# wdykas/LDDL

Hardware: AMD Instinct MI355X
Metric: WordPiece+MLM tokens/sec (1/2/4/8 MI355X) and % of HBM roofline (higher is better)
Workload: dtype uint16

## Files before the change

### include/lddl_amd.h

```cpp
#ifndef LDDL_AMD_H_
#define LDDL_AMD_H_

#include <stddef.h>
#include <stdint.h>

#ifdef __cplusplus
extern "C" {
#endif

typedef struct lddl_ctx lddl_ctx;

const char* lddl_last_error(void);
int lddl_version(void);
const char* lddl_build_id(void);

int64_t lddl_synth_corpus(uint64_t seed, int64_t doc_begin, int64_t target_bytes,
                          double nonascii_frac, uint8_t* text, int64_t text_cap,
                          int64_t* sent_off, int64_t sent_cap, int64_t* doc_sent_off,
                          int64_t doc_cap, int64_t* n_sent_out, int64_t* n_doc_out,
                          int n_threads);
int64_t lddl_synth_doc_text(uint64_t seed, int64_t doc_begin, int64_t target_bytes,
                            double nonascii_frac, uint8_t* text, int64_t text_cap, int64_t* doc_off,
                            int64_t doc_cap, int64_t* n_doc_out, int n_threads);

typedef struct lddl_reader lddl_reader;
int lddl_read_groups(int64_t n_blocks, const char* const* paths, const int64_t* starts,
                     const int64_t* ends, const uint32_t* mt_states, double ratio, int64_t n_groups,
                     const int64_t* group_off, const uint64_t* group_seed_abs, int n_threads,
                     lddl_reader** out, int64_t* n_docs, int64_t* n_text, int64_t* bad);
int lddl_read_fill(lddl_reader* reader, uint8_t* text, int64_t* doc_off, int64_t* block_ndocs);
int lddl_read_counts(const lddl_reader* reader, int64_t* block_ndocs, int64_t* doc_len);
int lddl_read_fill_range(lddl_reader* reader, int64_t d0, int64_t d1, uint8_t* text,
                         int64_t* doc_off);
int lddl_read_free(lddl_reader* reader);
int lddl_random_state_data(int64_t n, uint64_t seed_abs, uint32_t* out);

int lddl_ctx_create(int device, const uint8_t* norm_table, int64_t table_len, const char* vocab,
                    int64_t vocab_len, lddl_ctx** out);
int lddl_ctx_destroy(lddl_ctx* ctx);
int lddl_ctx_info(const lddl_ctx* ctx, int32_t* vocab_size, int32_t* special_ids,
                  int32_t* max_piece_bytes);
int lddl_ctx_id_bytes(const lddl_ctx* ctx);
int lddl_ctx_render_table(const lddl_ctx* ctx, const uint8_t** d_bytes, const int64_t** d_off);

typedef void* (*lddl_alloc_fn)(size_t bytes, void* stream, void* user);
typedef void (*lddl_free_fn)(void* p, void* stream, void* user);
int lddl_ctx_set_allocator(lddl_ctx* ctx, lddl_alloc_fn alloc_fn, lddl_free_fn free_fn,
                           void* user);

int lddl_tokenize(lddl_ctx* ctx, void* stream, const uint8_t* d_text, int64_t n_bytes,
                  const int64_t* d_sent_off, int64_t n_sent, int32_t max_pieces, int32_t* d_ids,
                  int32_t* d_sent_len);

int lddl_utf8_check(void* stream, const uint8_t* d_text, int64_t n_bytes, int64_t* d_first_bad);

int lddl_punkt_set_params(lddl_ctx* ctx, const uint8_t* table, int64_t table_bytes,
                          const uint8_t* records, int64_t records_bytes);
int lddl_segment_count(lddl_ctx* ctx, void* stream, const uint8_t* d_text, int64_t n_bytes,
                       const int64_t* d_doc_off, int64_t n_doc, int64_t* n_sent);
int lddl_segment_fill(lddl_ctx* ctx, void* stream, int64_t* d_sent_off, int64_t* d_doc_sent_off);

int lddl_bart_count(lddl_ctx* ctx, void* stream, const uint8_t* d_text, int64_t n_bytes,
                    const int64_t* d_sent_off, int64_t n_sent, const int64_t* d_doc_sent_off,
                    int64_t n_doc, int32_t target_words, int64_t* n_chunks, int64_t* n_out_bytes);
int lddl_bart_fill(lddl_ctx* ctx, void* stream, uint8_t* d_out, int64_t* d_chunk_off,
                   int32_t* d_num_tokens, int64_t* d_doc_chunk_off);

typedef struct lddl_pairs lddl_pairs;
enum { LDDL_RNG_REPLAY = 0, LDDL_RNG_NATIVE = 1 };
typedef struct {
  int32_t seq;
  int32_t dup;
  int32_t masking;
  int32_t rng;
  double short_seq_prob;
  double masked_lm_ratio;
  uint64_t native_seed;
} lddl_pair_params;
int lddl_pairs_plan(lddl_ctx* ctx, void* stream, const lddl_pair_params* params,
                    const int64_t* d_sent_off, const int32_t* d_ids, const int32_t* d_sent_len,
                    int64_t n_sent, const int64_t* d_doc_sent_off, int64_t n_doc,
                    const int64_t* d_part_doc_off, const int64_t* d_part_seed, int64_t n_part,
                    lddl_pairs** out, int64_t* counts);
int lddl_pairs_emit(lddl_pairs* plan, void* stream, void* d_tokens, int64_t* d_tok_off,
                    int32_t* d_len_a, uint8_t* d_is_rn, uint16_t* d_pos, void* d_lab,
                    int64_t* d_pos_off);
int lddl_pairs_destroy(lddl_pairs* plan, void* stream);
int lddl_pairs_part_offsets(lddl_pairs* plan, void* stream, int64_t* d_part_pair_off);
int lddl_pairs_plan_ms(const lddl_pairs* plan, float* ms);

int lddl_bin_partitions(lddl_ctx* ctx, void* stream, const int32_t* d_num_tokens,
                        const int64_t* d_tok_off, int64_t n_rows, const int64_t* d_part_off,
                        int64_t n_part, int32_t bin_size, int32_t nbins, int64_t* d_perm,
                        int64_t* d_bin_id, int64_t* d_counts);

int lddl_bin_stable(lddl_ctx* ctx, void* stream, const int32_t* d_num_tokens,
                    const int64_t* d_tok_off, int64_t n_rows, int32_t bin_size, int32_t nbins,
                    int64_t* d_perm, int64_t* d_bin_id, int64_t* d_counts);

int lddl_render_lengths(lddl_ctx* ctx, void* stream, const void* d_tokens,
                        const int64_t* d_tok_off, const int32_t* d_len_a, const void* d_lab,
                        const int64_t* d_pos_off, const int64_t* d_rows, int64_t n_rows,
                        int64_t* d_a_len, int64_t* d_b_len, int64_t* d_l_len, int64_t* d_npy_len,
                        const uint8_t* d_is_rn, uint16_t* d_num_tokens_out, uint8_t* d_is_rn_out);
int lddl_render_write(lddl_ctx* ctx, void* stream, const void* d_tokens,
                      const int64_t* d_tok_off, const int32_t* d_len_a, const uint16_t* d_pos,
                      const void* d_lab, const int64_t* d_pos_off, const int64_t* d_rows,
                      int64_t n_rows, const int64_t* d_a_off, const int64_t* d_b_off,
                      const int64_t* d_l_off, const int64_t* d_npy_off, uint8_t* d_a_bytes,
                      uint8_t* d_b_bytes, uint8_t* d_l_bytes, uint8_t* d_npy_bytes);

int lddl_gather_ragged(void* stream, const void* d_src_a, const int64_t* d_off_a, int64_t n_a,
                       const void* d_src_b, const int64_t* d_off_b, int32_t elem_bytes,
                       const int64_t* d_rows, int64_t n_rows, const int64_t* d_dst_off, void* d_dst);
int lddl_take(void* stream, const void* d_a, int64_t n_a, const void* d_b, int32_t elem_bytes,
              const int64_t* d_rows, int64_t n_rows, void* d_dst);
int lddl_ragged_offsets(lddl_ctx* ctx, void* stream, const int64_t* d_off_a, int64_t n_a,
                        const int64_t* d_off_b, const int64_t* d_rows, int64_t n_rows,
                        int64_t* d_out);
int lddl_expand_segments(void* stream, const int64_t* d_src, const int64_t* d_seg,
                         const int64_t* d_seg_off, int64_t n_seg, int64_t total, int64_t* d_out);
int lddl_pairs_meta_pack(void* stream, const int64_t* d_tok_off, const int32_t* d_len_a,
                         const uint8_t* d_is_rn, const int64_t* d_pos_off, const int64_t* d_rows,
                         int64_t n, int32_t* d_meta);
int lddl_pairs_meta_unpack(void* stream, const int32_t* d_meta, int64_t n, int64_t* d_ntok,
                           int32_t* d_len_a, uint8_t* d_is_rn, int64_t* d_nmask);

int lddl_scan_i64(lddl_ctx* ctx, void* stream, const int64_t* d_in, int64_t n, int64_t* d_out);

int lddl_collate_encode(lddl_ctx* ctx, void* stream, const uint8_t* d_bytes, const int64_t* d_a_off,
                        const int64_t* d_b_off, const int32_t* d_na, const int32_t* d_nb,
                        int32_t batch, int32_t seq_len, int64_t* d_input_ids,
                        int64_t* d_token_type_ids, int64_t* d_attention_mask,
                        int64_t* d_special_tokens_mask, const uint8_t* d_lab_bytes,
                        const int64_t* d_lab_off, const uint16_t* d_pos, const int64_t* d_pos_off,
                        int64_t* d_labels, int64_t ignore_index);

int lddl_collate_encode_mp(lddl_ctx* ctx, void* stream, const uint8_t* d_bytes,
                           const int64_t* d_a_off, const int64_t* d_b_off, const int32_t* d_na,
                           const int32_t* d_nb, int32_t batch, int32_t seq_len,
                           int64_t* d_input_ids, int64_t* d_token_type_ids,
                           int64_t* d_attention_mask, int64_t* d_special_tokens_mask,
                           const uint8_t* d_lab_bytes, const int64_t* d_lab_off,
                           const uint16_t* d_pos, const int64_t* d_pos_off, int64_t* d_labels,
                           int64_t ignore_index, int64_t* d_loss_mask);

int lddl_collate_encode_masked(lddl_ctx* ctx, void* stream, const uint8_t* d_bytes,
                               const int64_t* d_a_off, const int64_t* d_b_off, const int32_t* d_na,
                               const int32_t* d_nb, int32_t batch, int32_t seq_len,
                               int64_t* d_input_ids, int64_t* d_token_type_ids,
                               int64_t* d_attention_mask, int64_t* d_labels, float mlm_probability,
                               int64_t ignore_index, int64_t vocab_len, uint64_t seed,
                               uint64_t counter);

int lddl_mask_dynamic(lddl_ctx* ctx, void* stream, int64_t* d_input_ids, int64_t* d_labels,
                      const int64_t* d_special_tokens_mask, const int32_t* d_na, const int32_t* d_nb,
                      int64_t batch, int64_t seq_len, float mlm_probability, int64_t ignore_index,
                      int64_t vocab_len, uint64_t seed, uint64_t counter,
                      const uint8_t* d_r_masked, const uint8_t* d_r_replaced,
                      const uint8_t* d_r_random, const int64_t* d_r_words);

int lddl_mask_dynamic_ww(lddl_ctx* ctx, void* stream, int64_t* d_input_ids, int64_t* d_labels,
                         const int64_t* d_special_tokens_mask, const int32_t* d_na,
                         const int32_t* d_nb, int64_t batch, int64_t seq_len,
                         float mlm_probability, int64_t ignore_index, int64_t vocab_len,
                         uint64_t seed, uint64_t counter);

int lddl_collate_encode_masked_ww(lddl_ctx* ctx, void* stream, const uint8_t* d_bytes,
                                  const int64_t* d_a_off, const int64_t* d_b_off,
                                  const int32_t* d_na, const int32_t* d_nb, int32_t batch,
                                  int32_t seq_len, int64_t* d_input_ids, int64_t* d_token_type_ids,
                                  int64_t* d_attention_mask, int64_t* d_labels,
                                  float mlm_probability, int64_t ignore_index, int64_t vocab_len,
                                  uint64_t seed, uint64_t counter);

#ifdef __cplusplus
}
#endif

#endif
```

### lddl_amd/_native.py

```python
import ctypes
import os

import torch

_HERE = os.path.dirname(os.path.abspath(__file__))
LIB_PATH = os.environ.get('LDDL_AMD_LIB') or os.path.join(_HERE, '_lib', 'liblddl_amd.so')

c_i64, c_u64, c_i32, c_u32, c_dbl, c_vp = (ctypes.c_int64, ctypes.c_uint64, ctypes.c_int32,
                                           ctypes.c_uint32, ctypes.c_double, ctypes.c_void_p)
c_i64p = ctypes.POINTER(ctypes.c_int64)

SIGNATURES = {
    'lddl_last_error': (ctypes.c_char_p, []),
    'lddl_build_id': (ctypes.c_char_p, []),
    'lddl_version': (ctypes.c_int, []),
    'lddl_synth_corpus': (c_i64, [c_u64, c_i64, c_i64, c_dbl, c_vp, c_i64, c_vp, c_i64, c_vp, c_i64,
                                  c_i64p, c_i64p, ctypes.c_int]),
    'lddl_read_groups': (ctypes.c_int, [c_i64, c_vp, c_vp, c_vp, c_vp, c_dbl, c_i64, c_vp, c_vp,
                                        ctypes.c_int, ctypes.POINTER(c_vp), c_i64p, c_i64p, c_vp]),
    'lddl_read_fill': (ctypes.c_int, [c_vp, c_vp, c_vp, c_vp]),
    'lddl_read_free': (ctypes.c_int, [c_vp]),
    'lddl_read_counts': (ctypes.c_int, [c_vp, c_vp, c_vp]),
    'lddl_read_fill_range': (ctypes.c_int, [c_vp, c_i64, c_i64, c_vp, c_vp]),
    'lddl_random_state_data': (ctypes.c_int, [c_i64, c_u64, c_vp]),
    'lddl_ctx_create': (ctypes.c_int, [ctypes.c_int, c_vp, c_i64, c_vp, c_i64,
                                       ctypes.POINTER(c_vp)]),
    'lddl_ctx_destroy': (ctypes.c_int, [c_vp]),
    'lddl_ctx_info': (ctypes.c_int, [c_vp, c_vp, c_vp, c_vp]),
    'lddl_ctx_id_bytes': (ctypes.c_int, [c_vp]),
    'lddl_ctx_render_table': (ctypes.c_int, [c_vp, ctypes.POINTER(c_vp), ctypes.POINTER(c_vp)]),
    'lddl_synth_doc_text': (c_i64, [c_u64, c_i64, c_i64, c_dbl, c_vp, c_i64, c_vp, c_i64, c_vp,
                                    ctypes.c_int]),
    'lddl_punkt_set_params': (ctypes.c_int, [c_vp, c_vp, c_i64, c_vp, c_i64]),
    'lddl_segment_count': (ctypes.c_int, [c_vp, c_vp, c_vp, c_i64, c_vp, c_i64,
                                          ctypes.POINTER(c_i64)]),
    'lddl_segment_fill': (ctypes.c_int, [c_vp, c_vp, c_vp, c_vp]),
    'lddl_bart_count': (ctypes.c_int, [c_vp, c_vp, c_vp, c_i64, c_vp, c_i64, c_vp, c_i64, c_i32,
                                       ctypes.POINTER(c_i64), ctypes.POINTER(c_i64)]),
    'lddl_bart_fill': (ctypes.c_int, [c_vp, c_vp, c_vp, c_vp, c_vp, c_vp]),
    'lddl_tokenize': (ctypes.c_int, [c_vp, c_vp, c_vp, c_i64, c_vp, c_i64, c_i32, c_vp, c_vp]),
    'lddl_pairs_plan': (ctypes.c_int, [c_vp, c_vp, c_vp, c_vp, c_vp, c_vp, c_i64, c_vp, c_i64, c_vp,
                                       c_vp, c_i64, ctypes.POINTER(c_vp), c_vp]),
    'lddl_pairs_emit': (ctypes.c_int, [c_vp, c_vp, c_vp, c_vp, c_vp, c_vp, c_vp, c_vp, c_vp]),
    'lddl_pairs_destroy': (ctypes.c_int, [c_vp, c_vp]),
    'lddl_pairs_part_offsets': (ctypes.c_int, [c_vp, c_vp, c_vp]),
    'lddl_pairs_plan_ms': (ctypes.c_int, [c_vp, ctypes.POINTER(ctypes.c_float)]),
    'lddl_bin_partitions': (ctypes.c_int, [c_vp, c_vp, c_vp, c_vp, c_i64, c_vp, c_i64, c_i32, c_i32,
                                           c_vp, c_vp, c_vp]),
    'lddl_bin_stable': (ctypes.c_int, [c_vp, c_vp, c_vp, c_vp, c_i64, c_i32, c_i32, c_vp, c_vp,
                                       c_vp]),
    'lddl_render_lengths': (ctypes.c_int, [c_vp, c_vp, c_vp, c_vp, c_vp, c_vp, c_vp, c_vp, c_i64,
                                           c_vp, c_vp, c_vp, c_vp, c_vp, c_vp, c_vp]),
    'lddl_render_write': (ctypes.c_int, [c_vp, c_vp, c_vp, c_vp, c_vp, c_vp, c_vp, c_vp, c_vp,
                                         c_i64, c_vp, c_vp, c_vp, c_vp, c_vp, c_vp, c_vp, c_vp]),
    'lddl_scan_i64': (ctypes.c_int, [c_vp, c_vp, c_vp, c_i64, c_vp]),
    'lddl_gather_ragged': (ctypes.c_int, [c_vp, c_vp, c_vp, c_i64, c_vp, c_vp, c_i32, c_vp, c_i64,
                                          c_vp, c_vp]),
    'lddl_take': (ctypes.c_int, [c_vp, c_vp, c_i64, c_vp, c_i32, c_vp, c_i64, c_vp]),
    'lddl_ragged_offsets': (ctypes.c_int, [c_vp, c_vp, c_vp, c_i64, c_vp, c_vp, c_i64, c_vp]),
    'lddl_expand_segments': (ctypes.c_int, [c_vp, c_vp, c_vp, c_vp, c_i64, c_i64, c_vp]),
    'lddl_pairs_meta_pack': (ctypes.c_int, [c_vp, c_vp, c_vp, c_vp, c_vp, c_vp, c_i64, c_vp]),
    'lddl_pairs_meta_unpack': (ctypes.c_int, [c_vp, c_vp, c_i64, c_vp, c_vp, c_vp, c_vp]),
    'lddl_ctx_set_allocator': (ctypes.c_int, [c_vp, c_vp, c_vp, c_vp]),
    'lddl_collate_encode': (ctypes.c_int, [c_vp, c_vp, c_vp, c_vp, c_vp, c_vp, c_vp, c_i32, c_i32,
                                           c_vp, c_vp, c_vp, c_vp, c_vp, c_vp, c_vp, c_vp, c_vp,
                                           c_i64]),
    'lddl_collate_encode_mp': (ctypes.c_int, [c_vp, c_vp, c_vp, c_vp, c_vp, c_vp, c_vp, c_i32,
                                              c_i32, c_vp, c_vp, c_vp, c_vp, c_vp, c_vp, c_vp, c_vp,
                                              c_vp, c_i64, c_vp]),
    'lddl_utf8_check': (ctypes.c_int, [c_vp, c_vp, c_i64, c_vp]),
    'lddl_collate_encode_masked': (ctypes.c_int, [c_vp, c_vp, c_vp, c_vp, c_vp, c_vp, c_vp, c_i32,
                                                  c_i32, c_vp, c_vp, c_vp, c_vp, ctypes.c_float,
                                                  c_i64, c_i64, c_u64, c_u64]),
    'lddl_mask_dynamic': (ctypes.c_int, [c_vp, c_vp, c_vp, c_vp, c_vp, c_vp, c_vp, c_i64, c_i64,
                                         ctypes.c_float, c_i64, c_i64, c_u64, c_u64, c_vp, c_vp,
                                         c_vp, c_vp]),
    'lddl_mask_dynamic_ww': (ctypes.c_int, [c_vp, c_vp, c_vp, c_vp, c_vp, c_vp, c_vp, c_i64, c_i64,
                                            ctypes.c_float, c_i64, c_i64, c_u64, c_u64]),
    'lddl_collate_encode_masked_ww': (ctypes.c_int, [c_vp, c_vp, c_vp, c_vp, c_vp, c_vp, c_vp,
                                                     c_i32, c_i32, c_vp, c_vp, c_vp, c_vp,
                                                     ctypes.c_float, c_i64, c_i64, c_u64, c_u64]),
}


class PairParams(ctypes.Structure):
    _fields_ = [('seq', ctypes.c_int32), ('dup', ctypes.c_int32), ('masking', ctypes.c_int32),
                ('rng', ctypes.c_int32), ('short_seq_prob', ctypes.c_double),
                ('masked_lm_ratio', ctypes.c_double), ('native_seed', ctypes.c_uint64)]


RNG_REPLAY, RNG_NATIVE = 0, 1


class NativeError(RuntimeError):
    pass


def _load():
    if not os.path.exists(LIB_PATH):
        raise ImportError('lddl_amd native library not built: {} is missing (run `python -m '
                          'lddl_amd.build`). There is no CPU fallback.'.format(LIB_PATH))
    lib = ctypes.CDLL(LIB_PATH)
    for name, (res, args) in SIGNATURES.items():
        fn = getattr(lib, name)
        fn.restype = res
        fn.argtypes = args
    return lib


lib = _load()


def check(status):
    if status < 0:
        msg = lib.lddl_last_error()
        raise NativeError((msg or b'unknown error').decode())
    return status
```

### lddl_amd/csrc/ctx.h

```cpp
#pragma once
#include <hip/hip_runtime.h>
#include <cstdio>
#include <cstdlib>
#include <string>
#include <vector>

#include "arena.h"
#include "device.h"
struct lddl_ctx {
  int device = 0;
  lddl::Tables tab{};
  uint16_t* d_l1 = nullptr;
  uint32_t* d_pages = nullptr;
  uint8_t* d_pool = nullptr;
  lddl::VEnt* d_vhash = nullptr;
  uint8_t* d_vbytes = nullptr;
  int64_t* d_voff = nullptr;
  uint8_t* d_render = nullptr;
  int64_t* d_render_off = nullptr;
  uint32_t* d_bloom = nullptr;
  uint64_t* d_vlong = nullptr;
  uint32_t* d_cont_bits = nullptr;
  int32_t vocab_size = 0;
  int32_t id_bytes() const { return vocab_size <= 65534 ? 2 : 4; }
  size_t lds_per_block = 0;
  std::vector<std::string> tokens;
  lddl::DevArena arena;
  void* punkt = nullptr;
  void* bart = nullptr;
};
extern "C" void lddl_punkt_release(lddl_ctx* c);
extern "C" void lddl_bart_release(lddl_ctx* c);
extern "C" int lddl_punkt_tables(lddl_ctx* c, const uint16_t** l1, const uint8_t** pages);

namespace lddl {
inline hipStream_t as_stream(void* s) { return reinterpret_cast<hipStream_t>(s); }
}
```

### lddl_amd/csrc/ctx.hip

```cpp
#include <cstring>

#include "common.h"
#include "ctx.h"
#include "lddl_amd.h"

using namespace lddl;

namespace {

template <typename T>
int upload(T** dst, const void* src, size_t bytes) {
  LDDL_HIP(hipMalloc((void**)dst, bytes ? bytes : 16));
  if (bytes) LDDL_HIP(hipMemcpy(*dst, src, bytes, hipMemcpyHostToDevice));
  return 0;
}

uint64_t pack8(const uint8_t* p, int len) {
  uint64_t v = 0;
  for (int i = 0; i < len && i < 8; ++i) v |= (uint64_t)p[i] << (8 * i);
  return v;
}

}

extern "C" int lddl_ctx_create(int device, const uint8_t* norm_table, int64_t table_len,
                               const char* vocab, int64_t vocab_len, lddl_ctx** out) {
  *out = nullptr;
  if (table_len < 20 || memcmp(norm_table, "LDNT", 4) != 0)
    LDDL_FAIL(-1, "bad normaliser table blob");
  uint32_t n_pages, pool_len;
  memcpy(&n_pages, norm_table + 12, 4);
  memcpy(&pool_len, norm_table + 16, 4);
  const int64_t need = 20 + 2 * 4352 + 4 * 256 * (int64_t)n_pages + pool_len;
  if (table_len < need) LDDL_FAIL(-1, "truncated normaliser table (%lld < %lld)",
                                  (long long)table_len, (long long)need);
  LDDL_HIP(hipSetDevice(device));
  {
    hipMemPool_t pool;
    if (hipDeviceGetDefaultMemPool(&pool, device) == hipSuccess) {
      uint64_t thr = UINT64_MAX;
      (void)hipMemPoolSetAttribute(pool, hipMemPoolAttrReleaseThreshold, &thr);
    }
  }
  auto* c = new lddl_ctx();
  c->device = device;
  {
    int lds = 0;
    if (hipDeviceGetAttribute(&lds, hipDeviceAttributeMaxSharedMemoryPerBlock, device) == hipSuccess)
      c->lds_per_block = (size_t)lds;
  }

  std::string cur;
  for (int64_t i = 0; i < vocab_len; ++i) {
    char ch = vocab[i];
    if (ch == '\n') {
      if (!cur.empty() && cur.back() == '\r') cur.pop_back();
      c->tokens.push_back(cur);
      cur.clear();
    } else {
      cur.push_back(ch);
    }
  }
  if (!cur.empty()) c->tokens.push_back(cur);
  const int32_t V = (int32_t)c->tokens.size();
  if (V == 0 || V >= (1 << 21)) { delete c; LDDL_FAIL(-1, "vocab size %d unsupported", V); }
  c->vocab_size = V;

  std::vector<uint8_t> vbytes, render;
  std::vector<int64_t> voff(V + 1), roff(V + 1);
  std::vector<uint8_t> cont(V);
  int max_piece = 1;
  for (int32_t i = 0; i < V; ++i) {
    const std::string& t = c->tokens[i];
    roff[i] = (int64_t)render.size();
    render.insert(render.end(), t.begin(), t.end());
    voff[i] = (int64_t)vbytes.size();
    size_t b = 0;
    if (t.size() > 2 && t[0] == '#' && t[1] == '#') { cont[i] = 1; b = 2; }
    vbytes.insert(vbytes.end(), t.begin() + b, t.end());
    max_piece = std::max(max_piece, (int)(t.size() - b));
  }
  voff[V] = (int64_t)vbytes.size();
  roff[V] = (int64_t)render.size();
  if (max_piece > 255) { delete c; LDDL_FAIL(-1, "vocab piece longer than 255 bytes"); }

  uint32_t cap = 1;
  while (cap < 4u * (uint32_t)V + 64) cap <<= 1;
  std::vector<VEnt> tab(cap);
  memset(tab.data(), 0, sizeof(VEnt) * cap);
  for (int32_t i = 0; i < V; ++i) {
    const uint8_t* p = vbytes.data() + voff[i];
    const int len = (int)(voff[i + 1] - voff[i]);
    const uint64_t k0 = pack8(p, len);
    const uint32_t k1 = (uint32_t)pack8(p + 8, len > 8 ? std::min(len - 8, 4) : 0);
    const uint32_t meta = kMetaValid | (cont[i] ? kMetaCont : 0) | (len > 12 ? kMetaLong : 0) |
                          ((uint32_t)len << 21) | (uint32_t)i;
    uint64_t h = vhash(k0, k1, len, cont[i]);
    bool dup = false;
    uint32_t s = (uint32_t)h & (cap - 1);
    for (;; s = (s + 1) & (cap - 1)) {
      const VEnt& e = tab[s];
      if (!(e.meta & kMetaValid)) break;
      if (e.k0 == k0 && e.k1 == k1 && ((e.meta ^ meta) & ~0x1FFFFFu) == 0) {
        const int32_t j = meta_id(e.meta);
        if (len <= 12 || memcmp(vbytes.data() + voff[j], p, len) == 0) {
          tab[s].meta = meta;
          dup = true;
          break;
        }
      }
    }
    if (!dup) tab[s] = VEnt{k0, k1, meta};
  }

  std::vector<uint32_t> bloom(kBloomWords, 0u);
  for (int32_t i = 0; i < V; ++i) {
    const uint8_t* p = vbytes.data() + voff[i];
    const int len = (int)(voff[i + 1] - voff[i]);
    uint32_t h = 0;
    for (int k = 0; k < len; ++k) h = h * kBloomP + (uint32_t)p[k] + 1u;
    const uint32_t x = bloom_mix(h, (uint32_t)len, cont[i]);
    bloom[bloom_word(x)] |= bloom_bits(x);
  }
  std::vector<uint64_t> vlong(4 * (size_t)V, 0ull);
  for (int32_t i = 0; i < V; ++i) {
    const int len = (int)(voff[i + 1] - voff[i]);
    memcpy(reinterpret_cast<uint8_t*>(vlong.data() + 4 * (size_t)i), vbytes.data() + voff[i], std::min(len, 32));
  }
  std::vector<uint32_t> cont_bits(((size_t)V + 31) / 32, 0u);
  for (int32_t i = 0; i < V; ++i)
    if (cont[i]) cont_bits[i >> 5] |= 1u << (i & 31);
  const uint8_t* l1 = norm_table + 20;
  const uint8_t* pages = l1 + 2 * 4352;
  const uint8_t* pool = pages + 4 * 256 * (int64_t)n_pages;
  int rc = 0;
  if ((rc = upload(&c->d_l1, l1, 2 * 4352)) || (rc = upload(&c->d_pages, pages, 4 * 256 * (size_t)n_pages)) ||
      (rc = upload(&c->d_pool, pool, pool_len)) || (rc = upload(&c->d_vhash, tab.data(), sizeof(VEnt) * cap)) ||
      (rc = upload(&c->d_vbytes, vbytes.data(), vbytes.size())) ||
      (rc = upload(&c->d_voff, voff.data(), sizeof(int64_t) * voff.size())) ||
      (rc = upload(&c->d_render, render.data(), render.size())) ||
      (rc = upload(&c->d_render_off, roff.data(), sizeof(int64_t) * roff.size())) ||
      (rc = upload(&c->d_bloom, bloom.data(), sizeof(uint32_t) * bloom.size())) ||
      (rc = upload(&c->d_vlong, vlong.data(), sizeof(uint64_t) * vlong.size())) ||
      (rc = upload(&c->d_cont_bits, cont_bits.data(), sizeof(uint32_t) * cont_bits.size()))) {
    lddl_ctx_destroy(c);
    return rc;
  }
  Tables& T = c->tab;
  T.l1 = c->d_l1;
  T.pages = c->d_pages;
  T.pool = c->d_pool;
  T.vhash = c->d_vhash;
  T.vbytes = c->d_vbytes;
  T.voff = c->d_voff;
  T.vmask = cap - 1;
  T.bloom = c->d_bloom;
  T.vlong = c->d_vlong;
  T.max_piece_bytes = max_piece;
  static const char* kSpecial[kNumSpecial] = {"[PAD]", "[UNK]", "[CLS]", "[SEP]", "[MASK]"};
  for (int k = 0; k < kNumSpecial; ++k) {
    T.special_id[k] = -1;
    for (int32_t i = 0; i < V; ++i)
      if (c->tokens[i] == kSpecial[k]) { T.special_id[k] = i; break; }
  }
  {
    const uint16_t* l1p = reinterpret_cast<const uint16_t*>(l1);
    const uint32_t* pg = reinterpret_cast<const uint32_t*>(pages) + 256 * (size_t)l1p[0];
    bool lower_ok = true, ident_ok = true;
    for (uint32_t cp = 0; cp < 128; ++cp) {
      const uint32_t e = pg[cp];
      if ((e >> 30) != kWord && (e >> 30) != kIso) continue;
      const uint32_t outc = (e & kIdent) ? cp : (e & kMulti) ? 0xFFFFFFFFu : (e & 0x1FFFFFu);
      const uint32_t want_lower = (cp >= 'A' && cp <= 'Z') ? cp + 32 : cp;
      lower_ok &= outc == want_lower;
      ident_ok &= outc == cp;
    }
    T.ascii_mode = ident_ok ? 2 : lower_ok ? 1 : 0;
  }
  if (T.special_id[kUnk] < 0) { lddl_ctx_destroy(c); LDDL_FAIL(-1, "vocab has no [UNK]"); }
  *out = c;
  return 0;
}

extern "C" int lddl_ctx_destroy(lddl_ctx* c) {
  if (!c) return 0;
  (void)hipSetDevice(c->device);
  lddl_bart_release(c);
  lddl_punkt_release(c);
  for (void* p : {(void*)c->d_l1, (void*)c->d_pages, (void*)c->d_pool, (void*)c->d_vhash,
                  (void*)c->d_vbytes, (void*)c->d_voff, (void*)c->d_render, (void*)c->d_render_off,
                  (void*)c->d_bloom, (void*)c->d_vlong, (void*)c->d_cont_bits})
    if (p) (void)hipFree(p);
  delete c;
  return 0;
}

extern "C" int lddl_ctx_info(const lddl_ctx* c, int32_t* vocab_size, int32_t* special_ids,
                             int32_t* max_piece_bytes) {
  if (!c) LDDL_FAIL(-1, "null ctx");
  if (vocab_size) *vocab_size = c->vocab_size;
  if (special_ids)
    for (int k = 0; k < kNumSpecial; ++k) special_ids[k] = c->tab.special_id[k];
  if (max_piece_bytes) *max_piece_bytes = c->tab.max_piece_bytes;
  return 0;
}

extern "C" int lddl_ctx_id_bytes(const lddl_ctx* c) {
  if (!c) LDDL_FAIL(-1, "null ctx");
  return c->id_bytes();
}

extern "C" int lddl_ctx_render_table(const lddl_ctx* c, const uint8_t** d_bytes,
                                     const int64_t** d_off) {
  if (!c) LDDL_FAIL(-1, "null ctx");
  *d_bytes = c->d_render;
  *d_off = c->d_render_off;
  return 0;
}

extern "C" int lddl_ctx_set_allocator(lddl_ctx* c, lddl_alloc_fn alloc_fn, lddl_free_fn free_fn,
                                      void* user) {
  if (!c) LDDL_FAIL(-1, "null ctx");
  if ((alloc_fn == nullptr) != (free_fn == nullptr))
    LDDL_FAIL(-1, "set both allocator callbacks or neither");
  c->arena.set_external(alloc_fn, free_fn, user);
  return 0;
}
```

### lddl_amd/csrc/pairs.hip

```cpp
#include <algorithm>
#include <cstdio>
#include <memory>
#include <vector>

#include <cstdlib>
#include <cstring>

#include "common.h"
#include "ctx.h"
#include "device.h"
#include "lddl_amd.h"
#include "scan.h"

namespace lddl {
namespace {

struct alignas(16) PairDesc {
  int64_t a_ks;
  int64_t b_ks;
  int32_t a_front;
  int32_t na;
  int32_t b_front;
  int32_t nb_rn;
};

struct alignas(16) SlotPool {
  uint32_t moff8;
  uint32_t joff16;
  int32_t nmask;
  int32_t ncand;
};

constexpr int32_t kKeep = -1;

#ifdef LDDL_STAMPS
constexpr int kStampRegions = 8;
#define STAMP_T() __builtin_amdgcn_s_memtime()
#define STAMP_ADD(r, t0)                   \
  do {                                     \
    const uint64_t t1_ = STAMP_T();        \
    st_acc[r] += t1_ - (t0);               \
    t0 = t1_;                              \
  } while (0)
#else
#define STAMP_T() 0ull
#define STAMP_ADD(r, t0) ((void)0)
#endif

struct KeepSent {
  const int32_t* len;
  __device__ int64_t operator()(int64_t s) const { return (len[s] & kLenMask) > 0; }
};
struct SentCounts {
  const int32_t* len;
  __device__ Sum2 operator()(int64_t s) const {
    const int32_t l = len[s] & kLenMask;
    return Sum2{l > 0 ? 1 : 0, l};
  }
};
struct KeepDoc {
  const int64_t* ks_pos;
  const int64_t* doc_sent_off;
  __device__ int64_t operator()(int64_t d) const {
    return ks_pos[doc_sent_off[d + 1]] > ks_pos[doc_sent_off[d]];
  }
};

__global__ void scatter_sentences_kernel(const int64_t* sent_off, const int32_t* sent_len,
                                         int64_t n_sent, const int64_t* ks_pos, const int64_t* tok_pos,
                                         int64_t* ks_start, int32_t* ks_len, int64_t* kscan) {
  const int64_t s = (int64_t)blockIdx.x * blockDim.x + threadIdx.x;
  if (s > n_sent) return;
  if (s == n_sent) {
    kscan[ks_pos[n_sent]] = tok_pos[n_sent];
    return;
  }
  const int32_t l = sent_len[s];
  if ((l & kLenMask) == 0) return;
  const int64_t k = ks_pos[s];
  ks_start[k] = sent_off[s];
  ks_len[k] = l;
  kscan[k] = tok_pos[s];
}

__global__ void scatter_docs_kernel(const int64_t* doc_sent_off, int64_t n_doc, const int64_t* ks_pos,
                                    const int64_t* kd_pos, int64_t* kd_off) {
  const int64_t d = (int64_t)blockIdx.x * blockDim.x + threadIdx.x;
  if (d > n_doc) return;
  if (d == n_doc) { kd_off[kd_pos[n_doc]] = ks_pos[doc_sent_off[n_doc]]; return; }
  if (kd_pos[d + 1] > kd_pos[d]) kd_off[kd_pos[d]] = ks_pos[doc_sent_off[d]];
}

__global__ void part_offsets_kernel(const int64_t* part_doc_off, int64_t n_part, const int64_t* kd_pos,
                                    int64_t* kp_off, unsigned long long* max_docs) {
  const int64_t p = (int64_t)blockIdx.x * blockDim.x + threadIdx.x;
  if (p <= n_part) kp_off[p] = kd_pos[part_doc_off[p]];
  if (p < n_part)
    atomicMax(max_docs, (unsigned long long)(kd_pos[part_doc_off[p + 1]] - kd_pos[part_doc_off[p]]));
}

constexpr int kN = 624, kM = 397;
constexpr int kLook = 64;
constexpr int64_t kPoolChunk = 4096;

__device__ inline int uni(int x) { return __builtin_amdgcn_readfirstlane(x); }
__device__ inline uint32_t rdlane(uint32_t v, int idx) {
  return (uint32_t)__builtin_amdgcn_readlane((int)v, uni(idx));
}
__device__ inline uint32_t temper(uint32_t y) {
  y ^= (y >> 11);
  y ^= (y << 7) & 0x9d2c5680u;
  y ^= (y << 15) & 0xefc60000u;
  y ^= (y >> 18);
  return y;
}

struct WaveRng {
  uint32_t* mt;
  int mti;
  int wbase;
  int wend;
  uint32_t win;
#ifdef LDDL_STAMPS
  uint64_t n_pass = 0, n_win = 0;
#endif

  __device__ static uint32_t twist1(uint32_t a, uint32_t b, uint32_t c) {
    const uint32_t y = (a & 0x80000000u) | (b & 0x7fffffffu);
    return c ^ (y >> 1) ^ ((y & 1u) ? 0x9908b0dfu : 0u);
  }

  __device__ void twist() {
    const int l = threadIdx.x;
#pragma unroll
    for (int r = 0; r < 10; ++r) {
      const int i = 64 * r + l;
      const int ci = r < 3 ? i + kM : r > 3 ? i - (kN - kM) : (l < kN - kM - 192 ? i + kM : i - (kN - kM));
      const uint32_t v = twist1(mt[i], mt[i + 1], mt[ci]);
      mt[i] = v;
      __asm__ volatile("" ::: "memory");
    }
    mt[kN + l] = twist1(mt[l], mt[l + 1], mt[l + kM]);
    __asm__ volatile("" ::: "memory");
    mti -= kN;
    wbase = -1024;
    wend = 0;
  }
  __device__ void ensure() {
    if (mti >= kN) twist();
  }

  __device__ void seed_i64(int64_t seed) {
    if (threadIdx.x == 0) {
      const uint64_t a = seed < 0 ? (uint64_t)(-(seed + 1)) + 1 : (uint64_t)seed;
      const uint32_t key[2] = {(uint32_t)a, (uint32_t)(a >> 32)};
      const int klen = key[1] ? 2 : 1;
      uint32_t prev = 19650218u;
      mt[0] = prev;
      for (int i = 1; i < kN; ++i) {
        prev = 1812433253u * (prev ^ (prev >> 30)) + (uint32_t)i;
        mt[i] = prev;
      }
      int i = 1, j = 0;
      prev = mt[0];
      for (int k = kN; k; --k) {
        const uint32_t v = (mt[i] ^ ((prev ^ (prev >> 30)) * 1664525u)) + key[j] + (uint32_t)j;
        mt[i] = v;
        prev = v;
        ++i;
        ++j;
        if (i >= kN) { mt[0] = mt[kN - 1]; prev = mt[0]; i = 1; }
        if (j >= klen) j = 0;
      }
      for (int k = kN - 1; k; --k) {
        const uint32_t v = (mt[i] ^ ((prev ^ (prev >> 30)) * 1566083941u)) - (uint32_t)i;
        mt[i] = v;
        prev = v;
        ++i;
        if (i >= kN) { mt[0] = mt[kN - 1]; prev = mt[0]; i = 1; }
      }
      mt[0] = 0x80000000u;
      mt[kN] = twist1(mt[0], mt[1], mt[kM]);
    }
    __syncthreads();
    mti = kN;
    wbase = -1024;
    wend = 0;
  }

  __device__ void refill() {
    ensure();
    wbase = mti;
    wend = mti + 64;
    win = temper(mt[mti + (int)threadIdx.x]);
  }
  __device__ uint32_t u32() {
    if (mti >= wend) refill();
    const uint32_t v = rdlane(win, mti - wbase);
    mti = uni(mti + 1);
    return v;
  }
  template <typename Sink>
  __device__ void fy_draws(int32_t n, Sink sink) {
    const int lane = threadIdx.x;
    int32_t s0 = n - 1;
    while (s0 >= 1) {
      ensure();
      const uint32_t w = temper(mt[mti + lane]);
      const int32_t u1 = s0 + 1 - lane;
      int32_t R = (lane * 77) >> 8;
      uint32_t x;
      uint64_t rej;
      if (s0 >= 64) {
        auto pass = [&]() {
          const int32_t u = u1 + R;
          x = w >> __clz((uint32_t)u);
#ifdef LDDL_STAMPS
          ++n_pass;
#endif
          return ballot(x >= (uint32_t)u);
        };
        uint64_t prev = pass();
        R = (int32_t)popc_below(prev);
        rej = pass();
        while (rej != prev) {
          prev = rej;
          R = (int32_t)popc_below(rej);
          rej = pass();
        }
      } else {
        auto pass = [&]() {
          const int32_t u = u1 + R;
          x = w >> (__clz((uint32_t)u) & 31);
#ifdef LDDL_STAMPS
          ++n_pass;
#endif
          return ballot(x >= (uint32_t)u) & ballot(u > 1);
        };
        uint64_t prev = pass();
        R = (int32_t)popc_below(prev);
        rej = pass();
        while (rej != prev) {
          prev = rej;
          R = (int32_t)popc_below(rej);
          rej = pass();
        }
      }
#ifdef LDDL_STAMPS
      ++n_win;
#endif
      const int32_t i = u1 + R - 1;
      sink(x > (uint32_t)i ? 0 : max(i, 0), x);
      const uint64_t fin = ballot(i < 1);
      mti = uni(mti + (fin ? (int)__ffsll((unsigned long long)fin) - 1 : 64));
      s0 -= 64 - (int32_t)__popcll(rej);
    }
    wbase = -1024;
    wend = 0;
  }
  __device__ void trunc_draws(int32_t& na, int32_t& nb, int32_t max_num, int32_t& a_front,
                              int32_t& b_front) {
    const int32_t T = na + nb - max_num;
    if (T <= 0) return;
    const int32_t d = na - nb, ad = d < 0 ? -d : d;
    const int lane = threadIdx.x;
    for (int32_t done = 0; done < T;) {
      ensure();
      const int32_t cnt = min(T - done, 32);
      const int32_t t = done + lane;
      const uint32_t par = __popc(mt[mti + 2 * lane] & 0x89010000u) & 1u;
      const uint64_t F = ballot(par == 0) & ((1ull << cnt) - 1);
      const int32_t x = t - ad;
      const uint64_t S = ballot(t < d) | (ballot(x >= 0) & ballot((x & 1) != 0));
      a_front += __popcll(F & S);
      b_front += __popcll(F & ~S);
      mti = uni(mti + 2 * cnt);
      done += cnt;
    }
    wbase = -1024;
    wend = 0;
    const int32_t nA = (d > 0 ? min(d, T) : 0) + (T > ad ? (T - ad) / 2 : 0);
    na -= nA;
    nb -= T - nA;
  }

  __device__ int32_t mask_decisions(int cnt, uint64_t lt08, int32_t V, int32_t mask_id) {
    const int lane = threadIdx.x;
    const int kV = 32 - __clz((uint32_t)V);
    int32_t res = 0;
    int c = 0;
    while (c < cnt) {
      ensure();
      const uint32_t* wp = mt + mti + lane;
      const uint32_t w0 = temper(wp[0]);
      const uint32_t w1 = (uint32_t)wave_next((int)w0), w2 = (uint32_t)wave_next((int)w1),
                     w3 = (uint32_t)wave_next((int)w2), w4 = (uint32_t)wave_next((int)w3);
      (void)w3;
      const uint64_t N64 = ((uint64_t)(w0 >> 5) << 32) | w1;
      const bool mk = N64 < (lt08 << 6);
      const uint32_t top = w2 >> 31;
      const uint32_t r4 = w4 >> (32 - kV);
      const bool r4ok = r4 < (uint32_t)V;
      const int need = mk ? 2 : 4 + (int)top;
      int len = lane + need > kLook ? 0 : mk ? 2 : top ? (r4ok ? 5 : 0) : 4;
      int32_t tok = mk ? mask_id : top ? (int32_t)r4 : kKeep;
      if (!mk && top && !r4ok) {
        for (int j = 5; lane + j < kLook; ++j) {
          const uint32_t r = temper(wp[j]) >> (32 - kV);
          if (r < (uint32_t)V) {
            len = j + 1;
            tok = (int32_t)r;
            break;
          }
        }
      }
      int Jd[5];
      Jd[0] = len ? min(lane + len, 64) : 64;
#pragma unroll
      for (int b = 1; b < 5; ++b) {
        const int y = __shfl(Jd[b - 1], Jd[b - 1] & 63, 64);
        Jd[b] = Jd[b - 1] >= 64 ? 64 : y;
      }
      int p = 0;
#pragma unroll
      for (int b = 0; b < 5; ++b) {
        const int t = __shfl(Jd[b], p & 63, 64);
        if ((lane >> b) & 1) p = p >= 64 ? 64 : t;
      }
      const int lp = __shfl(len, p & 63, 64);
      const int32_t tp = __shfl(tok, p & 63, 64);
      const uint64_t okm = ballot(p < 64) & ballot(lp > 0) & 0xFFFFFFFFull;
      int take = __ffsll((unsigned long long)~okm) - 1;
      if (take > cnt - c) take = cnt - c;
      const int32_t tk = __shfl(tp, (lane - c) & 63, 64);
      if (lane >= c && lane < c + take) res = tk;
      if (take > 0) {
        mti = uni(mti + (int)rdlane((uint32_t)p, take - 1) + (int)rdlane((uint32_t)lp, take - 1));
        c += take;
      } else {
        wbase = -1024;
        wend = 0;
        int32_t t2;
        if (rand53() < lt08) t2 = mask_id;
        else if (below_half()) t2 = kKeep;
        else t2 = (int32_t)randint(0, V - 1);
        if (lane == c) res = t2;
        ++c;
      }
    }
    wbase = -1024;
    wend = 0;
    return res;
  }

  __device__ void u32x2(uint32_t& a, uint32_t& b) {
    if (mti + 1 < wend) {
      a = rdlane(win, mti - wbase);
      b = rdlane(win, mti + 1 - wbase);
      mti = uni(mti + 2);
    } else {
      a = u32();
      b = u32();
    }
  }
  __device__ uint64_t rand53() {
    uint32_t a, b;
    u32x2(a, b);
    return ((uint64_t)(a >> 5) << 26) | (b >> 6);
  }
  __device__ bool below_half() {
    uint32_t a, b;
    u32x2(a, b);
    return a < 0x80000000u;
  }
  __device__ uint32_t randbelow(uint32_t n) {
    const int k = 32 - __clz(n);
    uint32_t r = u32() >> (32 - k);
    while (r >= n) r = u32() >> (32 - k);
    return r;
  }
  __device__ int64_t randint(int64_t a, int64_t b) { return a + randbelow((uint32_t)(b - a + 1)); }
  __device__ int32_t randint32(int32_t a, int32_t b) { return a + (int32_t)randbelow((uint32_t)(b - a + 1)); }

};

struct IdPtr {
  void* p;
  int32_t ib;
  __device__ int32_t ld(int64_t i) const {
    return ib == 2 ? (int32_t)static_cast<const uint16_t*>(p)[i] : static_cast<const int32_t*>(p)[i];
  }
  __device__ void st(int64_t i, int32_t v) const {
    if (ib == 2) static_cast<uint16_t*>(p)[i] = (uint16_t)v;
    else static_cast<int32_t*>(p)[i] = v;
  }
};

struct PlanArgs {
  const int64_t* kscan;
  const int32_t* ks_len;
  const int64_t* kd_off;
  const int64_t* kp_off;
  const int64_t* ks_start;
  const int32_t* ids;
  IdPtr dense;
  int64_t n_kept_sent;
  int32_t n_part, n_dense_wg;
  const int64_t* part_seed;
  int32_t seq, dup, masking, vocab_size, cls_id, sep_id, mask_id, max_pred;
  double short_seq_prob, ratio;
  uint64_t k_short;
  int32_t seq_r64;
  PairDesc* desc;
  int32_t* jseq;
  SlotPool* spool;
  int32_t* mtok;
  void* jpool;
  int32_t jbytes;
  unsigned long long* pool_used;
  int64_t pool_cap, jpool_cap;
  int32_t* overflow;
  int64_t* part_npairs;
  uint64_t* stamps;
  uint64_t* tl;
};

constexpr int kDocLds = 512;
constexpr uint64_t kLt08 = 7205759403792794ull;

struct LenWin {
  const int32_t* len;
  int n, wbase;
  int32_t win, pre;
  uint64_t fl;
  __device__ void reset(const int32_t* p, int nn) { len = p; n = nn; wbase = -1024; }
  int32_t pfw;
  __device__ void prefetch(const int32_t* p, int nn) {
    const int k = (int)threadIdx.x;
    pfw = k < nn ? p[k] : 0;
  }
  __device__ void reset_prefetched(const int32_t* p, int nn) {
    len = p;
    n = nn;
    wbase = 0;
    win = pfw;
    pre = wave_incl_scan(win & kLenMask);
    fl = ballot((win & kLenHasClsSep) != 0);
  }
  __device__ bool has(int j) const { return (unsigned)(j - wbase) < 64u; }
  __device__ void load(int j) {
    wbase = j;
    const int k = j + (int)threadIdx.x;
    win = k < n ? len[k] : 0;
    pre = wave_incl_scan(win & kLenMask);
    fl = ballot((win & kLenHasClsSep) != 0);
  }
  __device__ int32_t at(int j) {
    if (!has(j)) load(j);
    return (int32_t)rdlane((uint32_t)win, j - wbase);
  }
  __device__ int64_t sum(int a, int b, int32_t& flags) {
    if (!has(a)) load(a);
    if (!has(b - 1)) {
      int64_t s = 0;
      for (int j = a; j < b; ++j) {
        const int32_t w = at(j);
        s += w & kLenMask;
        flags |= w;
      }
      return s;
    }
    const int32_t hi = (int32_t)rdlane((uint32_t)pre, b - 1 - wbase);
    const int32_t lo = a > wbase ? (int32_t)rdlane((uint32_t)pre, a - 1 - wbase) : 0;
    if (fl) {
      const int cnt = b - a;
      const uint64_t m = fl >> (a - wbase);
      if ((cnt >= 64 ? m : (m & ((1ull << cnt) - 1))) != 0) flags |= kLenHasClsSep;
    }
    return hi - lo;
  }
  __device__ int find(int a, int lim, int64_t T) {
    if (!has(a)) load(a);
    const int32_t T32 = T < -1 ? -1 : T > INT32_MAX ? INT32_MAX : (int32_t)T;
    for (int pass = 0; pass < 2; ++pass) {
      const int32_t base = a > wbase ? (int32_t)rdlane((uint32_t)pre, a - 1 - wbase) : 0;
      const int j = wbase + (int)threadIdx.x;
      const uint64_t m = ballot((uint32_t)(j - a) < (uint32_t)(lim - a)) & ballot(pre - base >= T32);
      if (m) return wbase + __ffsll((unsigned long long)m) - 1;
      if (wbase + 64 >= lim) return lim - 1;
      if (pass == 0 && wbase != a) load(a);
      else break;
    }
    int64_t s = 0;
    for (int i = a;; ++i) {
      s += at(i) & kLenMask;
      if (i == lim - 1 || s >= T) return i;
    }
  }
};

__device__ int32_t span_token(const PlanArgs& A, int64_t k0, int64_t j) {
  const int64_t x = A.kscan[k0] + j;
  int64_t k = k0;
  while (A.kscan[k + 1] <= x) ++k;
  return A.ids[A.ks_start[k] + (x - A.kscan[k])];
}

__device__ inline void densify_group(int64_t k0, const int64_t* __restrict__ ks_start,
                                     const int32_t* __restrict__ ks_len,
                                     const int64_t* __restrict__ kscan, int64_t n,
                                     const int32_t* __restrict__ ids, IdPtr dense) {
  const int lane = threadIdx.x & 63;
  const int64_t k = k0 + lane;
  const bool ok = k < n;
  const int32_t len = ok ? ks_len[k] & kLenMask : 0;
  const int64_t st = ok ? ks_start[k] : 0;
  const int32_t incl = wave_incl_scan(len);
  const int32_t total = __builtin_amdgcn_readlane(incl, 63);
  const int64_t base = kscan[k0];
  auto rl = [](int32_t v, int i) { return __builtin_amdgcn_readlane(v, i); };
  constexpr int kU = 4;
  int j = 0;
  for (int32_t c0 = 0; c0 < total; c0 += 64 * kU) {
    int64_t src[kU];
#pragma unroll
    for (int u = 0; u < kU; ++u) {
      const int32_t cu = c0 + 64 * u, x = cu + lane, hi = min(cu + 63, total - 1);
      src[u] = 0;
      if (cu < total) {
        while (rl(incl, j) <= cu) ++j;
        for (int jj = j;; ++jj) {
          const int32_t e = rl(incl, jj);
          const int32_t b = e - rl(len, jj);
          const int64_t s = ((int64_t)rl((int32_t)(st >> 32), jj) << 32) | (uint32_t)rl((int32_t)st, jj);
          if (x >= b && x < e) src[u] = s + (x - b);
          if (e > hi) break;
        }
      }
    }
    int32_t v[kU];
#pragma unroll
    for (int u = 0; u < kU; ++u) v[u] = c0 + 64 * u + lane < total ? ids[src[u]] : 0;
#pragma unroll
    for (int u = 0; u < kU; ++u)
      if (c0 + 64 * u + lane < total) dense.st(base + c0 + 64 * u + lane, v[u]);
  }
}

template <bool kDocsLds, int kJB>
__global__ void __launch_bounds__(64, 6) plan_replay_kernel(PlanArgs A) {
  extern __shared__ __attribute__((aligned(16))) uint8_t smem[];
  uint32_t* s_mt = reinterpret_cast<uint32_t*>(smem);
  int32_t* s_doc = reinterpret_cast<int32_t*>(s_mt + kN + kLook);
  const int p = blockIdx.x;
  const int lane = threadIdx.x;
  const bool leader = lane == 0;
  if (p >= A.n_part) {
    for (int64_t g = p - A.n_part; g * 64 < A.n_kept_sent; g += A.n_dense_wg)
      densify_group(g * 64, A.ks_start, A.ks_len, A.kscan, A.n_kept_sent, A.ids, A.dense);
    return;
  }
#ifdef LDDL_STAMPS
  uint64_t st_acc[kStampRegions] = {0, 0, 0, 0, 0, 0, 0, 0};
#endif
  [[maybe_unused]] uint64_t st_t = STAMP_T();
#ifdef LDDL_STAMPS
  const uint64_t rt0 = __builtin_amdgcn_s_memrealtime();
#endif
  WaveRng rng{s_mt, 0, 0, 0, 0u
#ifdef LDDL_STAMPS
              , 0, 0
#endif
  };
  rng.seed_i64(A.part_seed[p]);
  const int64_t d0 = A.kp_off[p];
  const int32_t nd = (int32_t)(A.kp_off[p + 1] - d0);
  const int64_t kbase = A.kd_off[d0];
  if (kDocsLds)
    for (int64_t d = lane; d <= nd; d += 64) s_doc[d] = (int32_t)(A.kd_off[d0 + d] - kbase);
  __syncthreads();
  auto doc_loc = [&](int32_t d) -> int32_t {
    if constexpr (kDocsLds) return uni(s_doc[d]);
    else return uni((int32_t)(A.kd_off[d0 + d] - kbase));
  };
  const int32_t* ks_len_p = A.ks_len + kbase;
  const int64_t base = (int64_t)A.dup * kbase;
  const int32_t max_num = A.seq - 3;
  int64_t pool_cur = 0, jpool_cur = 0;
  int32_t pool_left = 0, jpool_left = 0;
  bool pool_fits = true, jpool_fits = true;
  LenWin La, Lb;
  int64_t np = 0;
  constexpr int kPrioLevels = 4;
  int prio_q = -1;
  const int64_t prio_tot = (int64_t)A.dup * nd;
  int32_t prio_next = 0, prio_done = 0;
  if (nd > 0) La.prefetch(ks_len_p + doc_loc(0), doc_loc(1) - doc_loc(0));
  for (int dp = 0; dp < A.dup; ++dp) {
    for (int32_t di = 0; di < nd; ++di) {
      if (prio_done >= prio_next) {
        ++prio_q;
        prio_next = (int32_t)(((int64_t)(prio_q + 1) * prio_tot + kPrioLevels - 1) / kPrioLevels);
        const int lvl = kPrioLevels - 1 - prio_q;
        if (lvl >= 3) __builtin_amdgcn_s_setprio(3);
        else if (lvl == 2) __builtin_amdgcn_s_setprio(2);
        else if (lvl == 1) __builtin_amdgcn_s_setprio(1);
        else __builtin_amdgcn_s_setprio(0);
      }
      ++prio_done;
      const int32_t ls0 = doc_loc(di);
      const int64_t s0 = kbase + ls0;
      const int ns = doc_loc(di + 1) - ls0;
      La.reset_prefetched(ks_len_p + ls0, ns);
      {
        const int32_t dn = di + 1 < nd ? di + 1 : 0;
        const int32_t nl0 = doc_loc(dn);
        La.prefetch(ks_len_p + nl0, doc_loc(dn + 1) - nl0);
      }
      int32_t target = max_num;
      if (rng.rand53() < A.k_short) target = rng.randint32(2, max_num);
      for (int chunk0 = 0; chunk0 < ns;) {
        const int i = La.find(chunk0, ns, target);
        const int chunk_n = i - chunk0 + 1;
        const int a_end = chunk_n >= 2 ? rng.randint32(1, chunk_n - 1) : 1;
        int32_t flags = 0;
        const int64_t la = La.sum(chunk0, chunk0 + a_end, flags);
        int64_t lb = 0, b_ks;
        int32_t rn = 0;
        int next0;
        STAMP_ADD(0, st_t);
        if (chunk_n == 1 || rng.below_half()) {
          rn = 1;
          const int64_t target_b = target - la;
          int32_t rd = 0;
          for (int t = 0; t < 10; ++t) {
            rd = rng.randint32(0, nd - 1);
            if (rd != di) break;
          }
          if (rd == di) rn = 0;
          const int32_t r0l = doc_loc(rd);
          const int rns = doc_loc(rd + 1) - r0l;
          const int rstart = rng.randint32(0, rns - 1);
          b_ks = kbase + (r0l + rstart);
          Lb.reset(ks_len_p + r0l, rns);
          const int jb = Lb.find(rstart, rns, target_b);
          lb = Lb.sum(rstart, jb + 1, flags);
          next0 = chunk0 + a_end;
        } else {
          b_ks = s0 + chunk0 + a_end;
          lb = La.sum(chunk0 + a_end, i + 1, flags);
          next0 = i + 1;
        }
        STAMP_ADD(3, st_t);
        int32_t a_front = 0, b_front = 0, na = (int32_t)la, nb = (int32_t)lb;
        rng.trunc_draws(na, nb, max_num, a_front, b_front);
        STAMP_ADD(5, st_t);
        const int64_t slot = base + np;
        A.desc[slot] = PairDesc{s0 + chunk0, b_ks, a_front, na, b_front,
                                nb | (int32_t)((uint32_t)rn << 31)};
        if (A.masking) {
          int32_t nc = na + nb;
          if (flags & kLenHasClsSep) {
            int32_t c = 0;
            for (int32_t t = 0; t < na + nb; ++t) {
              const int32_t tok = uni(t < na ? span_token(A, s0 + chunk0, a_front + t)
                                             : span_token(A, b_ks, b_front + (t - na)));
              c += tok != A.cls_id && tok != A.sep_id;
            }
            nc = uni(c);
          }
          STAMP_ADD(1, st_t);
          int32_t num = uni((int32_t)__builtin_rint((double)(na + nb + 3) * A.ratio));
          if (num < 1) num = 1;
          if (num > nc) num = nc;
          if (num > pool_left) {
            const int32_t sz = num > kPoolChunk ? (num + 7) & ~7 : (int32_t)kPoolChunk;
            int64_t nb0 = 0;
            if (leader) nb0 = (int64_t)atomicAdd(&A.pool_used[0], (unsigned long long)sz);
            nb0 = ((int64_t)uni((int)(nb0 >> 32)) << 32) | (uint32_t)uni((int)(uint32_t)nb0);
            pool_cur = nb0;
            pool_left = sz;
            pool_fits = nb0 + sz <= A.pool_cap;
          }
          if (nc > jpool_left) {
            const int32_t sz = nc > kPoolChunk ? (nc + 15) & ~15 : (int32_t)kPoolChunk;
            int64_t nb0 = 0;
            if (leader) nb0 = (int64_t)atomicAdd(&A.pool_used[2], (unsigned long long)sz);
            nb0 = ((int64_t)uni((int)(nb0 >> 32)) << 32) | (uint32_t)uni((int)(uint32_t)nb0);
            jpool_cur = nb0;
            jpool_left = sz;
            jpool_fits = nb0 + sz <= A.jpool_cap;
          }
          const int64_t mb = pool_cur, jb = jpool_cur;
          pool_cur += (num + 7) & ~7;
          pool_left -= (num + 7) & ~7;
          jpool_cur += (nc + 15) & ~15;
          jpool_left -= (nc + 15) & ~15;
          const bool fits = pool_fits && jpool_fits;
          if (!fits) *A.overflow = 1;
          const int32_t ip = nc + lane;
          if constexpr (kJB == 1) {
            uint8_t* jd = static_cast<uint8_t*>(A.jpool) + jb;
            rng.fy_draws(nc, [&](int32_t i, uint32_t j) {
              if (fits) jd[i] = (uint8_t)j;
            });
            if (fits && ip < ((nc + 15) & ~15)) jd[ip] = (uint8_t)ip;
          } else {
            uint16_t* jd = static_cast<uint16_t*>(A.jpool) + jb;
            rng.fy_draws(nc, [&](int32_t i, uint32_t j) {
              if (fits) jd[i] = (uint16_t)j;
            });
            if (fits && ip < ((nc + 15) & ~15)) jd[ip] = (uint16_t)ip;
          }
          STAMP_ADD(2, st_t);
          for (int32_t c0 = 0; c0 < num; c0 += 64) {
            const int cmax = min(64, num - c0);
            const int32_t mytok = rng.mask_decisions(cmax, kLt08, A.vocab_size, A.mask_id);
            if (fits && lane < cmax) A.mtok[mb + c0 + lane] = mytok;
          }
          STAMP_ADD(4, st_t);
          A.spool[slot] = SlotPool{(uint32_t)(mb >> 3), (uint32_t)(jb >> 4), num, nc};
        }
        ++np;
        chunk0 = next0;
      }
    }
  }
  STAMP_ADD(0, st_t);
  {
    int32_t* js = A.jseq + base;
    rng.fy_draws(np, [&](int32_t i, uint32_t j) { js[i] = (int32_t)j; });
  }
  STAMP_ADD(6, st_t);
#ifdef LDDL_STAMPS
  st_acc[7] = rng.n_pass * 1000000 / (rng.n_win ? rng.n_win : 1);
  if (leader && A.stamps)
    for (int r = 0; r < kStampRegions; ++r) A.stamps[(int64_t)p * kStampRegions + r] = st_acc[r];
  if (leader && A.tl) {
    A.tl[2 * (int64_t)p] = rt0;
    A.tl[2 * (int64_t)p + 1] = __builtin_amdgcn_s_memrealtime();
  }
#endif
  if (leader) A.part_npairs[p] = np;
}

__device__ inline uint64_t mix64(uint64_t x) {
  x ^= x >> 30;
  x *= 0xBF58476D1CE4E5B9ull;
  x ^= x >> 27;
  x *= 0x94D049BB133111EBull;
  return x ^ (x >> 31);
}

__device__ inline uint64_t part_key(uint64_t native_seed, int64_t part_seed) {
  return mix64(native_seed ^ mix64((uint64_t)part_seed + 0x9E3779B97F4A7C15ull));
}

enum : uint32_t { kStreamWalk = 1, kStreamMask = 2, kStreamOrder = 3, kStreamDecide = 4 };

struct CtrRng {
  uint2 key;
  uint32_t id0, id1, blk;
  uint4 buf;
  int have;
  __device__ CtrRng(uint64_t k, int64_t index, uint32_t stream)
      : key{(uint32_t)k, (uint32_t)(k >> 32)},
        id0((uint32_t)index),
        id1((uint32_t)((uint64_t)index >> 32) << 4 | stream),
        blk(0),
        have(0) {}
  __device__ uint32_t u32() {
    if (have == 0) {
      buf = Philox::gen(make_uint4(blk++, id0, id1, 0x6C64646Cu), key);
      have = 4;
    }
    --have;
    return have == 3 ? buf.x : have == 2 ? buf.y : have == 1 ? buf.z : buf.w;
  }
  __device__ uint64_t rand53() {
    const uint32_t a = u32() >> 5, b = u32() >> 6;
    return ((uint64_t)a << 26) | b;
  }
  __device__ bool coin() { return u32() < 0x80000000u; }
  __device__ uint32_t randbelow(uint32_t n) {
    const int k = 32 - __clz(n);
    uint32_t r = u32() >> (32 - k);
    while (r >= n) r = u32() >> (32 - k);
    return r;
  }
  __device__ int64_t randint(int64_t a, int64_t b) { return a + randbelow((uint32_t)(b - a + 1)); }
  __device__ int32_t heads(int32_t n) {
    int32_t h = 0;
    for (; n >= 32; n -= 32) h += __popc(u32());
    if (n > 0) h += __popc(u32() & ((1u << n) - 1u));
    return h;
  }
};

struct NativeArgs {
  const int32_t* ks_len;
  const int64_t* kd_off;
  const int64_t* kp_off;
  const int64_t* kscan;
  IdPtr dense;
  const int64_t* part_seed;
  int64_t n_part, n_units, unit0;
  uint64_t native_seed, k_short;
  int32_t seq, dup, masking, cls_id, sep_id, mask_id, vocab_size;
  double ratio;
  int64_t* ucnt;
  const int64_t* uoff;
  const int64_t* part_base;
  PairDesc* desc;
  int32_t* nmask;
  int32_t* ncand;
  int32_t* ppart;
  const int64_t* moff;
  uint16_t* mpos;
  int32_t* mtok;
  int64_t* src;
  int64_t n_pairs;
  int32_t words;
};

__device__ inline int32_t win_token(const NativeArgs& A, int64_t k, int32_t front, int32_t t) {
  return A.dense.ld(A.kscan[k] + front + t);
}

struct WalkTab {
  const int32_t* s_pre;
  const int32_t* s_doc;
  const int64_t* g_pre;
  const int64_t* g_doc;
  int64_t sb, pre_sb;
  bool lds;
  __device__ int64_t pre(int64_t i) const { return lds ? (int64_t)s_pre[i] : g_pre[sb + i] - pre_sb; }
  __device__ int32_t doc(int64_t d) const { return lds ? s_doc[d] : (int32_t)(g_doc[d] - sb); }
};

__device__ inline int32_t first_reaching(const WalkTab& W, int32_t i, int32_t end, int64_t need) {
  int32_t a = i, b = i + 1;
  for (int32_t step = 1;; step <<= 1) {
    b = a + step;
    if (b >= end) {
      b = end;
      break;
    }
    if (W.pre(b) >= need) break;
    a = b;
  }
  if (b == end && W.pre(end) < need) return end - 1;
  while (b - a > 1) {
    const int32_t m = (a + b) >> 1;
    if (W.pre(m) >= need) b = m;
    else a = m;
  }
  return b - 1;
}

__device__ inline int32_t range_flags(const NativeArgs& A, bool has_flags, int64_t sb, int32_t x,
                                      int32_t y) {
  int32_t f = 0;
  if (has_flags)
    for (int32_t j = x; j < y; ++j) f |= A.ks_len[sb + j];
  return f & kLenHasClsSep;
}

constexpr int kNativeThreads = 256;

template <bool EMIT>
__global__ void __launch_bounds__(kNativeThreads) plan_native_kernel(NativeArgs A, const int64_t* g_pre,
                                                                     int32_t lds_words) {
  extern __shared__ int32_t s_tab[];
  __shared__ int32_t s_next;
  const int64_t p = blockIdx.x;
  const int64_t d0 = A.kp_off[p], nd = A.kp_off[p + 1] - d0;
  const int64_t sb = A.kd_off[d0], nsp = A.kd_off[d0 + nd] - sb;
  WalkTab W{s_tab, s_tab + nsp + 1, g_pre, A.kd_off + d0, sb, 0,
            nsp + nd + 2 <= (int64_t)lds_words};
  bool flag_any = false;
  if (W.lds) {
    int32_t* pre = s_tab;
    int32_t* dst = s_tab + nsp + 1;
    for (int64_t i = threadIdx.x; i < nsp; i += kNativeThreads) {
      const int32_t v = A.ks_len[sb + i];
      pre[i + 1] = v & kLenMask;
      flag_any |= (v & kLenHasClsSep) != 0;
    }
    for (int64_t d = threadIdx.x; d <= nd; d += kNativeThreads) dst[d] = (int32_t)(A.kd_off[d0 + d] - sb);
    if (threadIdx.x == 0) {
      pre[0] = 0;
      s_next = kNativeThreads;
    }
    __syncthreads();
    const int32_t per = (int32_t)((nsp + kNativeThreads - 1) / kNativeThreads);
    const int32_t x0 = 1 + (int32_t)threadIdx.x * per;
    const int32_t x1 = min(x0 + per, (int32_t)nsp + 1);
    int32_t run = 0;
    for (int32_t x = x0; x < x1; ++x) run += pre[x];
    __shared__ int32_t s_wsum[kNativeThreads / 64];
    const int32_t inc = wave_incl_scan(run);
    if ((threadIdx.x & 63) == 63) s_wsum[threadIdx.x >> 6] = inc;
    __syncthreads();
    int32_t off = inc - run;
    for (int w = 0; w < (int)(threadIdx.x >> 6); ++w) off += s_wsum[w];
    for (int32_t x = x0; x < x1; ++x) {
      off += pre[x];
      pre[x] = off;
    }
  } else {
    W.pre_sb = g_pre[sb];
    for (int64_t i = threadIdx.x; i < nsp; i += kNativeThreads)
      flag_any |= (A.ks_len[sb + i] & kLenHasClsSep) != 0;
    if (threadIdx.x == 0) s_next = kNativeThreads;
  }
  const bool has_flags = __syncthreads_or(flag_any) != 0;
  const int64_t nu = (int64_t)A.dup * nd;
  const int64_t ug0 = (int64_t)A.dup * (d0 - A.kp_off[0]);
  const uint64_t key = part_key(A.native_seed, A.part_seed[p]);
  const int32_t max_num = A.seq - 3;
  int64_t r = threadIdx.x;
  bool fresh = true;
  CtrRng rng(key, 0, kStreamWalk);
  int32_t s0 = 0, ns = 0, i = 0, target = 0, dl = 0;
  int64_t np = 0, base = 0;
  while (__builtin_amdgcn_ballot_w64(r < nu)) {
    if (r < nu) {
      if (fresh) {
        fresh = false;
        dl = (int32_t)(r % nd);
        rng = CtrRng(key, r, kStreamWalk);
        s0 = W.doc(dl);
        ns = W.doc(dl + 1) - s0;
        i = 0;
        np = 0;
        if (EMIT) base = A.uoff[ug0 + r];
        target = max_num;
        if (rng.rand53() < A.k_short) target = (int32_t)rng.randint(2, max_num);
      }
      if (i < ns) {
        const int64_t c_pre = W.pre(s0 + i);
        const int32_t e = first_reaching(W, s0 + i, s0 + ns, c_pre + target) - s0;
        const int32_t chunk0 = i, chunk_n = e - i + 1;
        const int32_t a_end = chunk_n >= 2 ? (int32_t)rng.randint(1, chunk_n - 1) : 1;
        const int64_t la = W.pre(s0 + chunk0 + a_end) - c_pre;
        int64_t lb, b_ks;
        int32_t rn = 0, flags = 0;
        if (chunk_n == 1 || rng.coin()) {
          rn = 1;
          const int64_t target_b = target - la;
          int64_t rd = 0;
          for (int t = 0; t < 10; ++t) {
            rd = rng.randint(0, nd - 1);
            if (rd != dl) break;
          }
          if (rd == dl) rn = 0;
          const int32_t r0 = W.doc(rd), rns = W.doc(rd + 1) - r0;
          const int32_t rstart = (int32_t)rng.randint(0, rns - 1);
          const int64_t b_pre = W.pre(r0 + rstart);
          const int32_t be = first_reaching(W, r0 + rstart, r0 + rns, b_pre + target_b);
          lb = W.pre(be + 1) - b_pre;
          b_ks = sb + r0 + rstart;
          if (EMIT && A.masking)
            flags = range_flags(A, has_flags, sb, s0 + chunk0, s0 + chunk0 + a_end) |
                    range_flags(A, has_flags, sb, r0 + rstart, be + 1);
          i = chunk0 + a_end;
        } else {
          lb = W.pre(s0 + e + 1) - W.pre(s0 + chunk0 + a_end);
          b_ks = sb + s0 + chunk0 + a_end;
          if (EMIT && A.masking) flags = range_flags(A, has_flags, sb, s0 + chunk0, s0 + e + 1);
          i = e + 1;
        }
        int32_t na = (int32_t)la, nb = (int32_t)lb, a_front = 0, b_front = 0;
        const int32_t T = na + nb - max_num;
        if (T > 0) {
          const int32_t dd = na - nb, ad = dd < 0 ? -dd : dd;
          const int32_t nA = (dd > 0 ? min(dd, T) : 0) + (T > ad ? (T - ad) / 2 : 0);
          a_front = rng.heads(nA);
          b_front = rng.heads(T - nA);
          na -= nA;
          nb -= T - nA;
        }
        if (EMIT) {
          const int64_t q = base + np;
          const int64_t a_ks = sb + s0 + chunk0;
          A.desc[q] = PairDesc{a_ks, b_ks, a_front, na, b_front, nb | (int32_t)((uint32_t)rn << 31)};
          A.ppart[q] = (int32_t)p;
          if (A.masking) {
            int32_t nc = na + nb;
            if (flags) {
              nc = 0;
              for (int32_t t = 0; t < na + nb; ++t) {
                const int32_t tok = t < na ? win_token(A, a_ks, a_front, t)
                                           : win_token(A, b_ks, b_front, t - na);
                nc += tok != A.cls_id && tok != A.sep_id;
              }
            }
            int32_t num = (int32_t)rint((double)(na + nb + 3) * A.ratio);
            if (num < 1) num = 1;
            if (num > nc) num = nc;
            A.nmask[q] = num;
            A.ncand[q] = nc;
          }
        }
        ++np;
      }
      if (i >= ns) {
        if (!EMIT) A.ucnt[ug0 + r] = np;
        r = atomicAdd(&s_next, 1);
        fresh = true;
      }
    }
  }
}

__global__ void native_part_need_kernel(const int64_t* kp_off, const int64_t* kd_off, int64_t n_part,
                                        unsigned long long* need_max) {
  const int64_t p = (int64_t)blockIdx.x * blockDim.x + threadIdx.x;
  if (p >= n_part) return;
  const int64_t d0 = kp_off[p], d1 = kp_off[p + 1];
  atomicMax(need_max, (unsigned long long)(kd_off[d1] - kd_off[d0] + (d1 - d0) + 2));
}

struct KeptLenOnly {
  const int32_t* v;
  __device__ int64_t operator()(int64_t i) const { return v[i] & kLenMask; }
};

__global__ void native_part_base_kernel(const int64_t* kp_off, int64_t n_part, int32_t dup,
                                        const int64_t* uoff, int64_t* part_base) {
  const int64_t p = (int64_t)blockIdx.x * blockDim.x + threadIdx.x;
  if (p <= n_part) part_base[p] = uoff[(int64_t)dup * (kp_off[p] - kp_off[0])];
}

__device__ inline uint32_t lemire_below(uint32_t x, uint32_t n, CtrRng& rng) {
  uint64_t m = (uint64_t)x * n;
  if ((uint32_t)m < n) {
    const uint32_t t = (0u - n) % n;
    while ((uint32_t)m < t) m = (uint64_t)rng.u32() * n;
  }
  return (uint32_t)(m >> 32);
}

constexpr uint32_t kNat80 = 3435973837u, kNat90 = 3865470567u;

__global__ void __launch_bounds__(256) mask_native_kernel(NativeArgs A, int32_t stage_cap) {
  extern __shared__ __attribute__((aligned(16))) uint8_t s_mn[];
  const int w = wave_id(), lane = threadIdx.x & 63, nw = blockDim.x >> 6;
  const int64_t q0 = ((int64_t)blockIdx.x * nw + w) * 64;
  if (q0 >= A.n_pairs) return;
  uint32_t* bm = reinterpret_cast<uint32_t*>(s_mn) + (size_t)w * A.words * 64 + lane;
  int32_t* stok = reinterpret_cast<int32_t*>(s_mn + (size_t)nw * A.words * 64 * 4) + (size_t)w * stage_cap;
  uint16_t* spos = reinterpret_cast<uint16_t*>(s_mn + (size_t)nw * A.words * 64 * 4 +
                                                (size_t)nw * stage_cap * 4) + (size_t)w * stage_cap;
  const int64_t q = q0 + lane;
  const bool valid = q < A.n_pairs;
  const int64_t qv = valid ? q : q0;
  const int64_t qe = q0 + 64 < A.n_pairs ? q0 + 64 : A.n_pairs;
  const int64_t m0 = A.moff[q0];
  const int32_t mend = (int32_t)(A.moff[qe] - m0);
  const int32_t num = valid ? A.nmask[qv] : 0;
  const int32_t nc = A.ncand[qv];
  const int32_t mb = (int32_t)(A.moff[qv] - m0);
  const PairDesc d = A.desc[qv];
  const int32_t na = d.na, nb = d.nb_rn & 0x7FFFFFFF;
  const int64_t p = A.ppart[qv];
  const uint64_t key = part_key(A.native_seed, A.part_seed[p]);
  const int64_t idx = qv - A.part_base[p];
  for (int i = 0; i < A.words; ++i) bm[i * 64] = 0u;
  CtrRng rng(key, idx, kStreamMask);
  for (int32_t s = 0; __builtin_amdgcn_ballot_w64(s < num); ++s) {
    const uint32_t u = rng.u32();
    if (s < num) {
      const uint32_t j = (uint32_t)(nc - num + s);
      const uint32_t t = lemire_below(u, j + 1u, rng);
      const uint32_t wt = bm[(t >> 5) * 64];
      const uint32_t pick = (wt >> (t & 31)) & 1u ? j : t;
      bm[(pick >> 5) * 64] |= 1u << (pick & 31);
    }
  }
  CtrRng drng(key, idx, kStreamDecide);
  const bool fast = nc == na + nb;
  int32_t wi = 0, tcur = 0, ccur = 0;
  uint32_t bits = num > 0 ? bm[0] : 0u;
  for (int32_t m = 0; __builtin_amdgcn_ballot_w64(m < num); ++m) {
    const uint32_t x = drng.u32(), y = drng.u32();
    if (m < num) {
      while (bits == 0u) bits = bm[++wi * 64];
      const int32_t ci = wi * 32 + __ffs(bits) - 1;
      bits &= bits - 1u;
      int32_t t = ci;
      if (!fast) {
        while (true) {
          const int32_t tok = tcur < na ? win_token(A, d.a_ks, d.a_front, tcur)
                                        : win_token(A, d.b_ks, d.b_front, tcur - na);
          if (tok != A.cls_id && tok != A.sep_id) {
            if (ccur == ci) break;
            ++ccur;
          }
          ++tcur;
        }
        t = tcur++;
        ++ccur;
      }
      const int32_t tok = x < kNat80 ? A.mask_id
                          : x < kNat90 ? kKeep
                                       : (int32_t)lemire_below(y, (uint32_t)A.vocab_size, drng);
      spos[mb + m] = (uint16_t)(t < na ? t + 1 : t + 2);
      stok[mb + m] = tok;
    }
  }
  wave_sync();
  for (int32_t i = lane; i < mend; i += 64) {
    A.mpos[m0 + i] = spos[i];
    A.mtok[m0 + i] = stok[i];
  }
}

__global__ void __launch_bounds__(256) order_native_kernel(NativeArgs A) {
  const int64_t q = (int64_t)blockIdx.x * 256 + threadIdx.x;
  if (q >= A.n_pairs) return;
  const int64_t p = A.ppart[q];
  const int64_t pb = A.part_base[p], np = A.part_base[p + 1] - pb;
  const uint64_t key = mix64(part_key(A.native_seed, A.part_seed[p]) ^ kStreamOrder);
  int bits = 1;
  while ((1ll << bits) < np) ++bits;
  const int h = (bits + 1) >> 1;
  const uint64_t hm = (1ull << h) - 1;
  uint64_t x = (uint64_t)(q - pb);
  do {
    uint64_t L = x >> h, R = x & hm;
    for (uint64_t rd = 0; rd < 4; ++rd) {
      const uint64_t f = mix64(R ^ key ^ (rd << 56)) & hm;
      const uint64_t nl = R;
      R = L ^ f;
      L = nl;
    }
    x = (L << h) | R;
  } while (x >= (uint64_t)np);
  A.src[q] = pb + (int64_t)x;
}



__global__ void __launch_bounds__(64) apply_shuffle_kernel(const int64_t* kd_off, const int64_t* kp_off,
                                                          int32_t dup, const int64_t* part_npairs,
                                                          const int32_t* jseq, int32_t* order,
                                                          int64_t min_np) {
  const int p = blockIdx.x;
  const int64_t base = (int64_t)dup * kd_off[kp_off[p]];
  const int64_t np = part_npairs[p];
  if (np <= min_np) return;
  const int32_t* js = jseq + base;
  int32_t* ord = order + base;
  for (int64_t k = threadIdx.x; k < np; k += 64) ord[k] = (int32_t)k;
  __syncthreads();
  if (threadIdx.x == 0) {
    for (int64_t i = np - 1; i > 0; --i) {
      const int32_t j = js[i];
      const int32_t t = ord[i];
      ord[i] = ord[j];
      ord[j] = t;
    }
  }
}

__device__ inline uint32_t lds_add16(uint32_t* words, uint32_t v) {
  const uint32_t sh = 16u * (v & 1u);
  return (atomicAdd(&words[v >> 1], 1u << sh) >> sh) & 0xFFFFu;
}

constexpr int kShufThreads = 1024;
struct PairMaps {
  const int64_t* part_base;
  int64_t *src, *slots, *dstq;
};

__global__ void __launch_bounds__(kShufThreads) shuffle_sort_kernel(const int64_t* kd_off, const int64_t* kp_off,
                                                          int32_t dup, const int64_t* part_npairs,
                                                          const int32_t* __restrict__ jseq,
                                                          int32_t* __restrict__ order, int32_t cap,
                                                          PairMaps M) {
  extern __shared__ __attribute__((aligned(16))) uint8_t ss_smem[];
  const int p = blockIdx.x;
  const int32_t n = (int32_t)part_npairs[p];
  if (n > cap) return;
  const int32_t capw = (cap + 2) & ~1;
  uint32_t* cntw = reinterpret_cast<uint32_t*>(ss_smem);
  uint16_t* cnt = reinterpret_cast<uint16_t*>(ss_smem);
  uint16_t* srt = reinterpret_cast<uint16_t*>(ss_smem) + capw;
  uint16_t* r = srt + capw;
  const int64_t base = (int64_t)dup * kd_off[kp_off[p]];
  const int32_t* __restrict__ js = jseq + base;
  int32_t* __restrict__ ord = order + base;
  const int tid = threadIdx.x;
  for (int32_t w = tid; w < capw / 2; w += kShufThreads) cntw[w] = 0u;
  for (int32_t i = tid; i < n; i += kShufThreads) r[i] = (uint16_t)js[i];
  __syncthreads();
  for (int32_t i = 1 + tid; i < n; i += kShufThreads) (void)lds_add16(cntw, r[i]);
  __syncthreads();
  {
    __shared__ int32_t s_w[kShufThreads / 64];
    const int32_t per = (n + kShufThreads - 1) / kShufThreads;
    const int32_t x0 = tid * per, x1 = min(x0 + per, n);
    int32_t run = 0;
    for (int32_t x = x0; x < x1; ++x) run += cnt[x];
    const int32_t inc = wave_incl_scan(run);
    if ((tid & 63) == 63) s_w[tid >> 6] = inc;
    __syncthreads();
    int32_t off = inc - run;
    for (int w = 0; w < (tid >> 6); ++w) off += s_w[w];
    for (int32_t x = x0; x < x1; ++x) {
      const int32_t c = cnt[x];
      cnt[x] = (uint16_t)off;
      off += c;
    }
  }
  __syncthreads();
  for (int32_t i = 1 + tid; i < n; i += kShufThreads) srt[lds_add16(cntw, r[i])] = (uint16_t)i;
  __syncthreads();
  for (int32_t v = tid; v < n; v += kShufThreads) {
    const int32_t lo = v ? cnt[v - 1] : 0, hi = cnt[v];
    for (int32_t m = lo + 1; m < hi; ++m) {
      const uint16_t e = srt[m];
      int32_t y = m - 1;
      while (y >= lo && srt[y] > e) {
        srt[y + 1] = srt[y];
        --y;
      }
      srt[y + 1] = e;
    }
    for (int32_t m = lo; m < hi; ++m) ord[srt[m]] = m + 1 < hi ? (int32_t)srt[m + 1] : ~v;
  }
  __syncthreads();
  for (int32_t k = tid; k < n; k += kShufThreads) {
    int32_t f = -1;
    if (k > 0) {
      if (r[k] == k) {
        f = ord[k];
      } else {
        const int32_t lo = cnt[k - 1], hi = cnt[k];
        f = lo < hi ? (int32_t)srt[lo] : -1;
      }
    }
    r[k] = (uint16_t)(f < 0 ? k : f);
  }
  __syncthreads();
  for (;;) {
    int changed = 0;
    for (int32_t k = tid; k < n; k += kShufThreads) {
      const uint16_t a = r[k], b = r[a];
      if (b != a) {
        r[k] = b;
        changed = 1;
      }
    }
    if (!__syncthreads_or(changed)) break;
  }
  const int32_t first0 = n > 1 && cnt[0] > 0 ? (int32_t)srt[0] : -1;
  const int64_t q0 = M.part_base ? M.part_base[p] : 0;
  for (int32_t k = tid; k < n; k += kShufThreads) {
    const int32_t sc = k == 0 ? first0 : ord[k];
    const int32_t v = sc >= 0 ? (int32_t)r[sc] : (k == 0 ? 0 : ~sc);
    ord[k] = v;
    if (M.src) M.src[q0 + k] = base + v;
    if (M.slots) M.slots[q0 + k] = base + k;
    if (M.dstq) M.dstq[q0 + v] = q0 + k;
  }
}

__global__ void map_pairs_kernel(const int64_t* kd_off, const int64_t* kp_off, int32_t dup,
                                 const int64_t* part_pair_base, const int32_t* order, int64_t* src,
                                 int64_t* slots, int64_t* dstq) {
  const int p = blockIdx.x;
  const int64_t base = (int64_t)dup * kd_off[kp_off[p]];
  const int64_t q0 = part_pair_base[p], n = part_pair_base[p + 1] - q0;
  for (int64_t k = threadIdx.x; k < n; k += blockDim.x) {
    if (src) src[q0 + k] = base + order[base + k];
    if (slots) slots[q0 + k] = base + k;
    if (dstq) dstq[q0 + order[base + k]] = q0 + k;
  }
}

__global__ void max_pairs_kernel(const int64_t* np, int64_t n, unsigned long long* out) {
  int64_t m = 0;
  for (int64_t i = (int64_t)blockIdx.x * blockDim.x + threadIdx.x; i < n; i += (int64_t)gridDim.x * blockDim.x)
    m = np[i] > m ? np[i] : m;
  if (m) atomicMax(out, (unsigned long long)m);
}

struct Identity {
  const int64_t* v;
  __device__ int64_t operator()(int64_t i) const { return v[i]; }
};

struct alignas(16) GatherRec {
  int64_t aoff, boff, moff;
  int32_t na, nb_rn, nm, pad;
};

__global__ void __launch_bounds__(256) pair_prep_kernel(const int64_t* __restrict__ src, int64_t n,
                                                        const PairDesc* __restrict__ desc,
                                                        const int64_t* __restrict__ kscan,
                                                        const int32_t* __restrict__ nmask,
                                                        const int64_t* __restrict__ moff,
                                                        GatherRec* __restrict__ rec,
                                                        int2* __restrict__ cnt) {
  const int64_t q = xcd_block(blockIdx.x, gridDim.x) * 256 + threadIdx.x;
  if (q >= n) return;
  const int64_t slot = src[q];
  const PairDesc d = desc[slot];
  GatherRec r;
  r.aoff = kscan[d.a_ks] + d.a_front;
  r.boff = kscan[d.b_ks] + d.b_front;
  r.moff = nmask ? moff[slot] : 0;
  r.na = d.na;
  r.nb_rn = d.nb_rn;
  r.nm = nmask ? nmask[slot] : 0;
  r.pad = 0;
  rec[q] = r;
  cnt[q] = make_int2(r.na + (r.nb_rn & 0x7FFFFFFF), r.nm);
}

struct PairTokens {
  const int2* c;
  __device__ int64_t operator()(int64_t q) const { return c[q].x; }
};
struct PairCounts {
  const int2* c;
  __device__ Sum2 operator()(int64_t q) const {
    const int2 v = c[q];
    return Sum2{v.x, v.y};
  }
};

__global__ void __launch_bounds__(256) densify_kernel(const int64_t* __restrict__ ks_start,
                                                      const int32_t* __restrict__ ks_len,
                                                      const int64_t* __restrict__ kscan, int64_t n,
                                                      const int32_t* __restrict__ ids,
                                                      IdPtr dense) {
  const int64_t k0 = ((int64_t)blockIdx.x * 4 + wave_id()) * 64;
  if (k0 >= n) return;
  densify_group(k0, ks_start, ks_len, kscan, n, ids, dense);
}


struct GatherArgs {
  const void* dense;
  const GatherRec* rec;
  const uint16_t* mpos;
  const int32_t* mtok;
  int32_t masking;
  int64_t n_pairs;
  const int64_t* tok_off;
  const int64_t* pos_off;
  void* out_tok;
  int32_t* len_a;
  uint8_t* is_rn;
  uint16_t* out_pos;
  void* out_lab;
  int64_t* out_tok_off;
  int64_t* out_pos_off;
};

constexpr int kMaxSeqGather = 4096;
constexpr int kGWaves = 4;

constexpr int32_t kNoMask = INT32_MIN;
constexpr int kStageRows = 128;
struct GatherLds {
  int32_t seqp;
  int32_t ib;
  int32_t db;
  __host__ __device__ size_t per_pair() const {
    return (size_t)db * seqp + (size_t)(kStageRows + 32) * (size_t)(2 + ib);
  }
};
constexpr uint16_t kNoMask16 = 0xFFFFu, kKeep16 = 0xFFFEu;

struct ResolveArgs {
  const int64_t* src;
  int64_t n_pairs;
  const PairDesc* desc;
  const SlotPool* spool;
  const void* jpool;
  uint16_t* mpos;
  const int64_t* kscan;
  IdPtr dense;
  int32_t cls_id, sep_id;
  const int64_t* dstq;
  GatherRec* rec;
  int2* cnt;
  int32_t col_rows;
};

template <typename T, int LW>
struct LaneCol;
template <int LW>
struct LaneCol<uint16_t, LW> {
  uint16_t* base;
  int lane;
  __device__ uint32_t get(int k) const { return base[k * LW + lane]; }
  __device__ void set(int k, uint32_t v) { base[k * LW + lane] = (uint16_t)v; }
  __device__ void iota(int n) {
    for (int k = 0; k < n; ++k) set(k, (uint32_t)k);
  }
};
template <int LW>
struct LaneCol<uint8_t, LW> {
  uint8_t* base;
  int lane;
  __device__ int at(int k) const { return ((k >> 2) * (4 * LW)) | (lane << 2) | (k & 3); }
  __device__ uint32_t get(int k) const { return base[at(k)]; }
  __device__ void set(int k, uint32_t v) { base[at(k)] = (uint8_t)v; }
  __device__ void iota(int n) {
    uint32_t* w = reinterpret_cast<uint32_t*>(base);
    for (int k = 0; k < n; k += 4)
      w[(k >> 2) * LW + lane] = (uint32_t)k | (uint32_t)(k + 1) << 8 | (uint32_t)(k + 2) << 16 |
                                (uint32_t)(k + 3) << 24;
  }
};

template <typename T, typename D, int NG, int LW = 64, bool kBF = false, int kRA = 0, int kPf = 4>
__global__ void __launch_bounds__(64) fy_resolve_kernel(ResolveArgs R) {
  extern __shared__ __attribute__((aligned(16))) uint8_t s_xb[];
  constexpr int kPerVec = 16 / (int)sizeof(D);
  const int lane = threadIdx.x;
  LaneCol<T, LW> x{reinterpret_cast<T*>(s_xb), lane};
  const int64_t q = xcd_block(blockIdx.x, gridDim.x) * LW + lane;
  constexpr bool kCoopIota = kBF && sizeof(T) == 2 && LW == 16;
  if constexpr (kCoopIota) {
    const int rows = (int)(R.col_rows);
    uint4* base = reinterpret_cast<uint4*>(s_xb);
    for (int k0 = 0; k0 < rows; k0 += 8) {
      const uint32_t k = (uint32_t)(k0 + (lane >> 1)), kk = k | k << 16;
      base[2 * k + (lane & 1)] = make_uint4(kk, kk, kk, kk);
    }
    __syncthreads();
  }
  if (q >= R.n_pairs) return;
  const int64_t slot = R.src[q];
  const int64_t oq = R.dstq ? R.dstq[q] : 0;
  const uint4 spv = *reinterpret_cast<const uint4*>(R.spool + slot);
  const PairDesc d = R.desc[slot];
  const SlotPool sp{spv.x, spv.y, (int32_t)spv.z, (int32_t)spv.w};
  const int32_t num = sp.nmask;
  const int32_t nc = num > 0 ? sp.ncand : 0;
  const int64_t jb = (int64_t)sp.joff16 << 4, mb = (int64_t)sp.moff8 << 3;
  const int32_t na = d.na, nb = d.nb_rn & 0x7FFFFFFF;
  const bool fast = nc == na + nb;
  const int64_t ao = R.kscan[d.a_ks] + d.a_front, bo = R.kscan[d.b_ks] + d.b_front;
  const uint4* jp = reinterpret_cast<const uint4*>(static_cast<const D*>(R.jpool) + jb);
  uint4* mp = reinterpret_cast<uint4*>(R.mpos + mb);
  uint4 acc = make_uint4(0u, 0u, 0u, 0u);
  auto group = [&](int h, const uint32_t* w) {
#pragma unroll
    for (int u = 7; u >= 0; --u) {
      const int i = 8 * h + u;
      if (i >= nc) continue;
      const int j = sizeof(D) == 1 ? (int)((w[u >> 2] >> (8 * (u & 3))) & 0xFFu)
                                   : (int)((w[u >> 1] >> (16 * (u & 1))) & 0xFFFFu);
      const uint32_t xi = x.get(i);
      if (i >= num) {
        if (i >= 1) x.set(j, xi);
      } else {
        const int y = i >= 1 ? (int)x.get(j) : (int)xi;
        if (i >= 1) x.set(j, xi);
        const uint32_t pos = (uint32_t)(fast ? (y < na ? y + 1 : y + 2) : y);
        acc = make_uint4((acc.x << 16) | pos, (acc.y << 16) | (acc.x >> 16),
                         (acc.z << 16) | (acc.y >> 16), (acc.w << 16) | (acc.z >> 16));
      }
    }
    if (8 * h < num) mp[h] = acc;
  };
  const int32_t padd = fast ? 1 : 0, thr = fast ? na : INT32_MAX;
  auto draw = [&](int h, const uint32_t* w, int u) -> int {
    const int j = sizeof(D) == 1 ? (int)((w[u >> 2] >> (8 * (u & 3))) & 0xFFu)
                                 : (int)((w[u >> 1] >> (16 * (u & 1))) & 0xFFFFu);
    return u == 0 && h == 0 ? 0 : j;
  };
  auto group_bf = [&](int h, const uint32_t* w) {
    if (__any(8 * h < num)) {
      uint32_t pos[8];
#pragma unroll
      for (int u = 7; u >= 0; --u) {
        const int i = 8 * h + u;
        const int j = draw(h, w, u);
        const uint32_t xi = x.get(i);
        const int y = (int)x.get(j);
        x.set(j, xi);
        pos[u] = i < num ? (uint32_t)(y + padd + (y >= thr ? 1 : 0)) : 0u;
      }
      if (8 * h < num)
        mp[h] = make_uint4(pos[0] | pos[1] << 16, pos[2] | pos[3] << 16, pos[4] | pos[5] << 16,
                           pos[6] | pos[7] << 16);
    } else if (kRA == 0) {
#pragma unroll
      for (int u = 7; u >= 0; --u) x.set(draw(h, w, u), x.get(8 * h + u));
    } else {
      int jr[8];
      uint32_t r[8], v[8];
#pragma unroll
      for (int u = 0; u < 8; ++u) jr[u] = draw(h, w, u) - 8 * h;
#pragma unroll
      for (int u = 7; u >= 8 - kRA; --u) r[u] = x.get(8 * h + u);
#pragma unroll
      for (int u = 7; u >= 0; --u) {
        if (u - kRA >= 0) r[u - kRA] = x.get(8 * h + u - kRA);
        uint32_t val = r[u];
#pragma unroll
        for (int t = kRA; t >= 1; --t)
          if (u + t <= 7) val = jr[u + t] == u ? v[u + t] : val;
        v[u] = val;
        x.set(jr[u] + 8 * h, val);
      }
    }
  };
  auto vec = [&](int g, const uint4& v) {
    const uint32_t w[4] = {v.x, v.y, v.z, v.w};
    if (kBF) {
      if (sizeof(D) == 1) group_bf(2 * g + 1, w + 2);
      group_bf(sizeof(D) == 1 ? 2 * g : g, w);
    } else if (sizeof(D) == 1) {
      if (16 * g + 8 < nc) group(2 * g + 1, w + 2);
      group(2 * g, w);
    } else {
      group(g, w);
    }
  };
  const int nvec = (nc + kPerVec - 1) / kPerVec;
  if (NG > 0) {
    uint4 jv[NG > 0 ? NG : 1];
#pragma unroll
    for (int g = 0; g < NG; ++g)
      if (g < nvec) jv[g] = jp[g];
    if (!kCoopIota) x.iota(nc);
#pragma unroll
    for (int g = NG - 1; g >= 0; --g)
      if (g < nvec) vec(g, jv[g]);
  } else if (nvec > 0) {
    auto ld = [&](int g) { return jp[g < 0 ? 0 : g]; };
    const int top = nvec - 1;
    uint4 rv[kPf];
#pragma unroll
    for (int u = 0; u < kPf; ++u) rv[u] = ld(top - u);
    if (!kCoopIota) x.iota(nc);
    for (int g = top; g >= 0; g -= kPf) {
#pragma unroll
      for (int u = 0; u < kPf; ++u) {
        if (g >= u) vec(g - u, rv[u]);
        rv[u] = ld(g - u - kPf);
      }
    }
  }
  if (R.rec) {
    GatherRec r;
    r.aoff = ao;
    r.boff = bo;
    r.moff = mb;
    r.na = na;
    r.nb_rn = d.nb_rn;
    r.nm = num;
    r.pad = 0;
    R.rec[oq] = r;
    R.cnt[oq] = make_int2(na + nb, num);
  }
  if (!fast && num > 0) {
    int k = 0;
    for (int t = 0; t < na + nb; ++t) {
      const int32_t tok = t < na ? R.dense.ld(ao + t) : R.dense.ld(bo + (t - na));
      if (tok != R.cls_id && tok != R.sep_id) x.set(k++, (uint32_t)(t < na ? t + 1 : t + 2));
    }
    uint16_t* m16 = R.mpos + mb;
    for (int c = 0; c < num; ++c) m16[c] = (uint16_t)x.get(m16[c]);
  }
}

template <typename IdT>
struct Tok4;
template <>
struct Tok4<int32_t> {
  typedef int32_t type __attribute__((ext_vector_type(4), aligned(4)));
};
template <>
struct Tok4<uint16_t> {
  typedef uint16_t type __attribute__((ext_vector_type(4), aligned(2)));
};
__device__ inline uint2 blend4(uint2 a, uint2 b, int32_t ra) {
  const int32_t bits = ra <= 0 ? 0 : ra >= 4 ? 64 : 16 * ra;
  const uint32_t mlo = bits >= 32 ? ~0u : (1u << bits) - 1u;
  const uint32_t mhi = bits >= 64 ? ~0u : bits <= 32 ? 0u : (1u << (bits - 32)) - 1u;
  return make_uint2((a.x & mlo) | (b.x & ~mlo), (a.y & mhi) | (b.y & ~mhi));
}
__device__ inline int4 blend4(int4 a, int4 b, int32_t ra) {
  return make_int4(0 < ra ? a.x : b.x, 1 < ra ? a.y : b.y, 2 < ra ? a.z : b.z, 3 < ra ? a.w : b.w);
}
template <typename IdT>
using Raw4 = std::conditional_t<sizeof(IdT) == 2, uint2, int4>;

template <int K, typename IdT>
__global__ void __launch_bounds__(64 * kGWaves, 1) gather_kernel(GatherArgs G, GatherLds Lg) {
  static_assert(K == 1 || K == 2, "masked counts of K pairs are packed 16 bits apart");
  using tok4_t = typename Tok4<IdT>::type;
  const IdT* __restrict__ dense = static_cast<const IdT*>(G.dense);
  extern __shared__ __attribute__((aligned(16))) uint8_t g_smem[];
  const int w = wave_id(), lane = threadIdx.x & 63, h = lane >> 5, sl = lane & 31;
  const int64_t wg = xcd_block((int64_t)blockIdx.y * gridDim.x + blockIdx.x, (int64_t)gridDim.x * gridDim.y);
  const int64_t q0 = (wg * kGWaves + w) * 2 * K;

  int64_t tof[K], aoff[K], boff[K], po[K], mb[K];
  int32_t na[K], nb[K], rk[K], nm[K];
  int32_t* dec[K];
  uint16_t* spos[K];
  IdT* slab[K];
  GatherRec rc[K];
#pragma unroll
  for (int k = 0; k < K; ++k) {
    const int64_t q = q0 + 2 * k + h;
    const bool act = q < G.n_pairs;
    rc[k] = act ? G.rec[q] : GatherRec{0, 0, 0, 0, 0, 0, 0};
    tof[k] = act ? G.tok_off[q] : 0;
    po[k] = (G.masking && act) ? G.pos_off[q] : 0;
  }
#pragma unroll
  for (int k = 0; k < K; ++k) {
    const int64_t q = q0 + 2 * k + h;
    const GatherRec& r = rc[k];
    na[k] = r.na;
    nb[k] = r.nb_rn & 0x7FFFFFFF;
    aoff[k] = r.aoff;
    boff[k] = r.boff;
    mb[k] = r.moff;
    nm[k] = G.masking ? r.nm : 0;
    rk[k] = 0;
    uint8_t* pb = g_smem + (((size_t)w * K + k) * 2 + h) * Lg.per_pair();
    dec[k] = reinterpret_cast<int32_t*>(pb);
    spos[k] = reinterpret_cast<uint16_t*>(pb + 4 * (size_t)Lg.seqp);
    slab[k] = reinterpret_cast<IdT*>(pb + 4 * (size_t)Lg.seqp + 2 * (kStageRows + 32));
    if (sl == 0 && q < G.n_pairs) {
      G.len_a[q] = na[k];
      G.is_rn[q] = (uint8_t)((uint32_t)r.nb_rn >> 31);
      if (G.out_tok_off) {
        G.out_tok_off[q] = tof[k];
        if (q + 1 == G.n_pairs) G.out_tok_off[q + 1] = tof[k] + na[k] + nb[k];
      }
      if (G.out_pos_off && G.masking) {
        G.out_pos_off[q] = po[k];
        if (q + 1 == G.n_pairs) G.out_pos_off[q + 1] = po[k] + nm[k];
      }
    }
  }
  using raw_t = Raw4<IdT>;
  raw_t ta[K], tb[K];
  auto issue_tokens = [&](int32_t x) {
#pragma unroll
    for (int k = 0; k < K; ++k) {
      const int32_t n = na[k] + nb[k], bx = x - na[k];
      ta[k] = *reinterpret_cast<const raw_t*>(dense + aoff[k] + (x < na[k] ? x : 0));
      tb[k] = *reinterpret_cast<const raw_t*>(dense + boff[k] + (bx >= -3 && x < n ? bx : 0));
    }
  };
  auto finish_tokens = [&](int32_t x, tok4_t* v) {
#pragma unroll
    for (int k = 0; k < K; ++k) v[k] = __builtin_bit_cast(tok4_t, blend4(ta[k], tb[k], na[k] - x));
  };
  tok4_t v[K];
  issue_tokens(4 * sl);
  if (G.masking) {
#pragma unroll
    for (int k = 0; k < K; ++k)
      for (int i = 4 * sl; i < Lg.seqp; i += 128)
        *reinterpret_cast<int4*>(dec[k] + i) = make_int4(kNoMask, kNoMask, kNoMask, kNoMask);
    wave_sync();
#pragma unroll
    for (int k = 0; k < K; ++k)
      for (int j = sl; j < nm[k]; j += 32) {
        const int p = G.mpos[mb[k] + j];
        dec[k][p <= na[k] ? p - 1 : p - 2] = G.mtok[mb[k] + j];
      }
    wave_sync();
  }
  for (int32_t cb = 0;; cb += 128) {
    const int32_t x = cb + 4 * sl;
    if (cb > 0) issue_tokens(x);
    finish_tokens(x, v);
    bool more = false;
    if (G.masking) {
      int4 d4[K];
      uint32_t m4[K], packed = 0;
#pragma unroll
      for (int k = 0; k < K; ++k) {
        d4[k] = *reinterpret_cast<const int4*>(dec[k] + x);
        m4[k] = (d4[k].x != kNoMask ? 1u : 0u) | (d4[k].y != kNoMask ? 2u : 0u) |
                (d4[k].z != kNoMask ? 4u : 0u) | (d4[k].w != kNoMask ? 8u : 0u);
        packed |= (uint32_t)__popc(m4[k]) << (16 * k);
      }
      const uint32_t inc = wave_incl_scan(packed);
      const uint32_t lo_tot = (uint32_t)__builtin_amdgcn_readlane((int)inc, 31);
      const uint32_t all_tot = (uint32_t)__builtin_amdgcn_readlane((int)inc, 63);
      const uint32_t excl = inc - packed - (h ? lo_tot : 0u);
      const uint32_t tots = h ? all_tot - lo_tot : lo_tot;
#pragma unroll
      for (int k = 0; k < K; ++k) {
        int32_t r = (int32_t)((excl >> (16 * k)) & 0xFFFFu);
        const int32_t dd[4] = {d4[k].x, d4[k].y, d4[k].z, d4[k].w};
#pragma unroll
        for (int e = 0; e < 4; ++e) {
          const bool mk = (m4[k] >> e) & 1u;
          const int32_t xe = x + e, at = mk ? r : kStageRows + sl;
          spos[k][at] = (uint16_t)(xe < na[k] ? xe + 1 : xe + 2);
          slab[k][at] = v[k][e];
          v[k][e] = mk && dd[e] != kKeep ? (IdT)dd[e] : v[k][e];
          r += mk ? 1 : 0;
        }
      }
      wave_sync();
#pragma unroll
      for (int k = 0; k < K; ++k) {
        const int32_t tot = (int32_t)((tots >> (16 * k)) & 0xFFFFu);
        for (int32_t i = sl; i < tot; i += 32) {
          G.out_pos[po[k] + rk[k] + i] = spos[k][i];
          static_cast<IdT*>(G.out_lab)[po[k] + rk[k] + i] = slab[k][i];
        }
        rk[k] += tot;
      }
      wave_sync();
    }
#pragma unroll
    for (int k = 0; k < K; ++k) {
      const int32_t n = na[k] + nb[k];
      IdT* out = static_cast<IdT*>(G.out_tok) + tof[k];
      if (x + 3 < n) {
        __builtin_nontemporal_store(v[k], reinterpret_cast<tok4_t*>(out + x));
      } else {
#pragma unroll
        for (int e = 0; e < 4; ++e)
          if (x + e < n) __builtin_nontemporal_store(v[k][e], out + x + e);
      }
      more |= n > cb + 128;
    }
    if (!ballot(more)) break;
  }
}

typedef uint16_t Tok8 __attribute__((ext_vector_type(8), aligned(2)));
__device__ inline uint4 blend8(uint4 a, uint4 b, int32_t ra) {
  const int32_t bits = ra <= 0 ? 0 : ra >= 8 ? 128 : 16 * ra;
  auto m = [&](int d) -> uint32_t {
    const int32_t t = bits - 32 * d;
    return t >= 32 ? ~0u : t <= 0 ? 0u : (1u << t) - 1u;
  };
  const uint32_t m0 = m(0), m1 = m(1), m2 = m(2), m3 = m(3);
  return make_uint4((a.x & m0) | (b.x & ~m0), (a.y & m1) | (b.y & ~m1), (a.z & m2) | (b.z & ~m2),
                    (a.w & m3) | (b.w & ~m3));
}

template <int LP>
struct G16 {
  static constexpr int kNT = 128 / LP;
  static constexpr int kNV = kNT / 8;
};

template <int LP>
__device__ inline uint32_t seg_scan(uint32_t v, int lane, uint32_t* tot) {
  uint32_t inc = v;
  inc = scan_step<0x111, 0xF, true>(inc);
  inc = scan_step<0x112, 0xF, true>(inc);
  inc = scan_step<0x114, 0xF, true>(inc);
  inc = scan_step<0x118, 0xF, true>(inc);
  const uint32_t r15 = (uint32_t)__builtin_amdgcn_update_dpp(0, (int)inc, 0x15F, 0xF, 0xF, false);
  if (LP == 16) {
    *tot = r15;
    return inc;
  }
  const uint32_t r7 = (uint32_t)__builtin_amdgcn_update_dpp(0, (int)inc, 0x157, 0xF, 0xF, false);
  const bool hi = (lane & 8) != 0;
  *tot = hi ? r15 - r7 : r7;
  return hi ? inc - r7 : inc;
}

template <int LP>
__global__ void __launch_bounds__(64 * kGWaves, 1) gather16_kernel(GatherArgs G, GatherLds Lg) {
  constexpr int NT = G16<LP>::kNT, NV = G16<LP>::kNV, PW = 64 / LP;
  const uint16_t* __restrict__ dense = static_cast<const uint16_t*>(G.dense);
  uint16_t* __restrict__ out_tok = static_cast<uint16_t*>(G.out_tok);
  uint16_t* __restrict__ out_lab = static_cast<uint16_t*>(G.out_lab);
  extern __shared__ __attribute__((aligned(16))) uint8_t g_smem[];
  const int w = wave_id(), lane = threadIdx.x & 63, qw = lane / LP, ql = lane % LP;
  const int64_t wg = xcd_block((int64_t)blockIdx.y * gridDim.x + blockIdx.x, (int64_t)gridDim.x * gridDim.y);
  const int64_t q = (wg * kGWaves + w) * PW + qw;
  const bool act = q < G.n_pairs;
  const GatherRec r = act ? G.rec[q] : GatherRec{0, 0, 0, 0, 0, 0, 0};
  const int64_t tof = act ? G.tok_off[q] : 0;
  const int64_t po = (G.masking && act) ? G.pos_off[q] : 0;
  const int32_t na = r.na, nb = r.nb_rn & 0x7FFFFFFF, n = na + nb;
  const int32_t nm = G.masking ? r.nm : 0;
  const int64_t mb = r.moff;
  uint8_t* pb = g_smem + ((size_t)w * PW + qw) * Lg.per_pair();
  uint16_t* dec = reinterpret_cast<uint16_t*>(pb);
  uint16_t* spos = reinterpret_cast<uint16_t*>(pb + 2 * (size_t)Lg.seqp);
  uint16_t* slab = reinterpret_cast<uint16_t*>(pb + 2 * (size_t)Lg.seqp + 2 * (kStageRows + 32));
  if (ql == 0 && act) {
    G.len_a[q] = na;
    G.is_rn[q] = (uint8_t)((uint32_t)r.nb_rn >> 31);
    if (G.out_tok_off) {
      G.out_tok_off[q] = tof;
      if (q + 1 == G.n_pairs) G.out_tok_off[q + 1] = tof + n;
    }
    if (G.out_pos_off && G.masking) {
      G.out_pos_off[q] = po;
      if (q + 1 == G.n_pairs) G.out_pos_off[q + 1] = po + nm;
    }
  }
  uint4 ta[NV], tb[NV];
  auto issue = [&](int32_t x) {
#pragma unroll
    for (int k = 0; k < NV; ++k) {
      const int32_t xk = x + 8 * k, bx = xk - na;
      ta[k] = *reinterpret_cast<const uint4*>(dense + r.aoff + (xk < na ? xk : 0));
      tb[k] = *reinterpret_cast<const uint4*>(dense + r.boff + (bx >= -7 && xk < n ? bx : 0));
    }
  };
  issue(NT * ql);
  int32_t rk = 0;
  if (G.masking) {
    for (int i = 8 * ql; i < Lg.seqp; i += 8 * LP)
      *reinterpret_cast<uint4*>(dec + i) = make_uint4(~0u, ~0u, ~0u, ~0u);
    wave_sync();
    for (int j = ql; j < nm; j += LP) {
      const int p = G.mpos[mb + j];
      const int32_t t = G.mtok[mb + j];
      dec[p <= na ? p - 1 : p - 2] = t == kKeep ? kKeep16 : (uint16_t)t;
    }
    wave_sync();
  }
  for (int32_t cb = 0;; cb += 128) {
    const int32_t x = cb + NT * ql;
    if (cb > 0) issue(x);
    Tok8 v[NV];
#pragma unroll
    for (int k = 0; k < NV; ++k) v[k] = __builtin_bit_cast(Tok8, blend8(ta[k], tb[k], na - x - 8 * k));
    if (G.masking) {
      uint32_t dd[NT];
#pragma unroll
      for (int k = 0; k < NT / 8; ++k) {
        const uint4 d = *reinterpret_cast<const uint4*>(dec + x + 8 * k);
        const uint32_t dw[4] = {d.x, d.y, d.z, d.w};
#pragma unroll
        for (int e = 0; e < 8; ++e) dd[8 * k + e] = (dw[e >> 1] >> (16 * (e & 1))) & 0xFFFFu;
      }
      uint32_t mk = 0;
#pragma unroll
      for (int e = 0; e < NT; ++e) mk |= dd[e] != kNoMask16 ? 1u << e : 0u;
      const uint32_t c = (uint32_t)__popc(mk);
      uint32_t tot;
      const uint32_t inc = seg_scan<LP>(c, lane, &tot);
      int32_t rr = (int32_t)(inc - c);
#pragma unroll
      for (int e = 0; e < NT; ++e) {
        const bool m = (mk >> e) & 1u;
        const int32_t xe = x + e;
        if (m) {
          spos[rr] = (uint16_t)(xe < na ? xe + 1 : xe + 2);
          slab[rr] = v[e >> 3][e & 7];
        }
        v[e >> 3][e & 7] = m && dd[e] != kKeep16 ? (uint16_t)dd[e] : v[e >> 3][e & 7];
        rr += m ? 1 : 0;
      }
      wave_sync();
      for (int32_t i = ql; i < (int32_t)tot; i += LP) {
        G.out_pos[po + rk + i] = spos[i];
        out_lab[po + rk + i] = slab[i];
      }
      rk += (int32_t)tot;
      wave_sync();
    }
    uint16_t* out = out_tok + tof;
#pragma unroll
    for (int k = 0; k < NV; ++k) {
      const int32_t xk = x + 8 * k;
      if (xk + 7 < n) {
        __builtin_nontemporal_store(v[k], reinterpret_cast<Tok8*>(out + xk));
      } else {
#pragma unroll
        for (int e = 0; e < 8; ++e)
          if (xk + e < n) __builtin_nontemporal_store(v[k][e], out + xk + e);
      }
    }
    if (!ballot(n > cb + 128)) break;
  }
}

}
}

using namespace lddl;

struct lddl_pairs {
  int32_t masking = 0, max_pred = 0, seq = 0, cls_id = -1, sep_id = -1;
  int64_t n_part = 0, n_pairs = 0, n_tokens = 0, n_masked = 0, n_kept_sent = 0, n_kept_doc = 0;
  ArenaScope mem;
  int64_t *ks_start = nullptr, *kd_off = nullptr, *kp_off = nullptr, *kscan = nullptr;
  int32_t* ks_len = nullptr;
  IdPtr dense{nullptr, 4};
  PairDesc* desc = nullptr;
  int32_t *order = nullptr, *nmask = nullptr, *mtok = nullptr;
  uint16_t* mpos = nullptr;
  int64_t* moff = nullptr;
  int64_t *src = nullptr, *tok_off = nullptr, *pos_off = nullptr;
  GatherRec* rec = nullptr;
  int64_t* part_base = nullptr;
  hipEvent_t ev[2] = {nullptr, nullptr};

  lddl_pairs(DevArena* arena, hipStream_t st) : mem(arena, st) {}
  ~lddl_pairs() {
    for (hipEvent_t e : ev)
      if (e) (void)hipEventDestroy(e);
  }
};

struct FyKnobs {
  int mode, lw, ra, pf;
};

static int env_int(const char* name, int dflt) {
  const char* e = getenv(name);
  return e ? atoi(e) : dflt;
}

static int read_fy_knobs(FyKnobs* k) {
  *k = FyKnobs{env_int("LDDL_FY_MODE", -1), env_int("LDDL_FY_LW", 16), env_int("LDDL_FY_RA", 1),
               env_int("LDDL_FY_PF", 4)};
  if (k->mode < -1 || k->mode > 1) LDDL_FAIL(-1, "LDDL_FY_MODE must be -1 (auto), 0 or 1");
  if (k->lw != 16 && k->lw != 32) LDDL_FAIL(-1, "LDDL_FY_LW must be 16 or 32");
  if (k->ra < 0 || k->ra > 3) LDDL_FAIL(-1, "LDDL_FY_RA must be 0 .. 3");
  if (k->pf != 2 && k->pf != 4 && k->pf != 8) LDDL_FAIL(-1, "LDDL_FY_PF must be 2, 4 or 8");
  if (k->pf != 4 && k->ra != 1) LDDL_FAIL(-1, "LDDL_FY_PF applies with LDDL_FY_RA=1 only");
  if ((k->ra != 1 || k->pf != 4) && (k->mode == 0 || k->lw == 32))
    LDDL_FAIL(-1, "LDDL_FY_RA / PF select 16-lane branch-free variants (not with LDDL_FY_MODE=0 "
                  "or LDDL_FY_LW=32)");
  return 0;
}

static int check_plan_args(const lddl_ctx* c, const lddl_pair_params* prm, FyKnobs* fy) {
  if (!c || !prm) LDDL_FAIL(-1, "null argument");
  if (prm->seq < 5 || prm->seq > 65535) LDDL_FAIL(-1, "target_seq_length %d out of range", prm->seq);
  if (prm->dup < 1) LDDL_FAIL(-1, "duplicate_factor must be >= 1");
  if (prm->rng != LDDL_RNG_REPLAY && prm->rng != LDDL_RNG_NATIVE)
    LDDL_FAIL(-1, "unknown rng mode %d", prm->rng);
  if (prm->masking && prm->seq > kMaxSeqGather)
    LDDL_FAIL(-1, "static masking supports target_seq_length <= %d", kMaxSeqGather);
  if (prm->masking && (c->tab.special_id[kCls] < 0 || c->tab.special_id[kSep] < 0 ||
                       c->tab.special_id[kMask] < 0))
    LDDL_FAIL(-1, "static masking needs [CLS] [SEP] [MASK] in the vocab");
  return read_fy_knobs(fy);
}

struct PlanWork {
  lddl_ctx* c;
  const lddl_pair_params* prm;
  const int32_t* d_ids;
  const int64_t* d_part_seed;
  int64_t n_sent, n_part;
  hipStream_t st;
  ArenaScope& tmp;
  FyKnobs fy;
  int64_t* scratch = nullptr;
  int64_t n_kept_tok = 0;
  unsigned long long max_docs = 0;
  int32_t* jseq = nullptr;
  int64_t* part_npairs = nullptr;
  SlotPool* spool = nullptr;
  void* jpool = nullptr;
  int64_t max_np = 1;
  PairMaps M{nullptr, nullptr, nullptr, nullptr};
  int2* pcnt = nullptr;
  int64_t* scr2 = nullptr;
#ifdef LDDL_STAMPS
  uint64_t *d_stamps = nullptr, *d_tl = nullptr;
#endif
};

static bool dense_in_plan(const PlanWork& W) { return W.prm->rng == LDDL_RNG_REPLAY && W.n_part > 0; }

static uint64_t short_threshold(double p) {
  if (!(p > 0)) return 0;
  if (p >= 1) return 1ull << 53;
  return (uint64_t)ceil(ldexp(p, 53));
}

struct I32 {
  const int32_t* v;
  __device__ int64_t operator()(int64_t i) const { return v[i]; }
};

static int compact_inputs(lddl_pairs* P, PlanWork& W, const int64_t* d_sent_off,
                          const int32_t* d_sent_len, const int64_t* d_doc_sent_off, int64_t n_doc,
                          const int64_t* d_part_doc_off) {
  const int64_t n_sent = W.n_sent, n_part = W.n_part;
  hipStream_t st = W.st;
  int rc;
  int64_t *ks_pos, *tok_pos, *kd_pos;
  const int64_t nscr = 2 * scan_scratch_elems(std::max(n_sent, n_doc) + n_part + 1);
  if ((rc = W.tmp.take(&W.scratch, nscr)) || (rc = W.tmp.take(&ks_pos, n_sent + 1)) ||
      (rc = W.tmp.take(&tok_pos, n_sent + 1)))
    return rc;
  LDDL_HIP(scan_exclusive2(SentCounts{d_sent_len}, n_sent, ks_pos, tok_pos, W.scratch, st));
  if ((rc = W.tmp.take(&kd_pos, n_doc + 1))) return rc;
  LDDL_HIP(scan_exclusive(KeepDoc{ks_pos, d_doc_sent_off}, n_doc, kd_pos, W.scratch, st));
  int64_t h_counts[3];
  LDDL_HIP(hipMemcpyAsync(&h_counts[0], ks_pos + n_sent, 8, hipMemcpyDeviceToHost, st));
  LDDL_HIP(hipMemcpyAsync(&h_counts[1], kd_pos + n_doc, 8, hipMemcpyDeviceToHost, st));
  LDDL_HIP(hipMemcpyAsync(&h_counts[2], tok_pos + n_sent, 8, hipMemcpyDeviceToHost, st));
  LDDL_HIP(hipStreamSynchronize(st));
  P->n_kept_sent = h_counts[0];
  P->n_kept_doc = h_counts[1];
  W.n_kept_tok = h_counts[2];
  unsigned long long* d_max_docs;
  if ((rc = P->mem.take(&P->ks_start, P->n_kept_sent)) || (rc = P->mem.take(&P->ks_len, P->n_kept_sent)) ||
      (rc = P->mem.take(&P->kscan, P->n_kept_sent + 1)) || (rc = P->mem.take(&P->kd_off, P->n_kept_doc + 1)) ||
      (rc = P->mem.take(&P->kp_off, n_part + 1)) || (rc = W.tmp.take(&d_max_docs, 1)))
    return rc;
  hipLaunchKernelGGL(scatter_sentences_kernel, dim3((unsigned)((n_sent + 256) / 256)), dim3(256), 0,
                     st, d_sent_off, d_sent_len, n_sent, ks_pos, tok_pos, P->ks_start, P->ks_len,
                     P->kscan);
  hipLaunchKernelGGL(scatter_docs_kernel, dim3((unsigned)((n_doc + 256) / 256)), dim3(256), 0, st,
                     d_doc_sent_off, n_doc, ks_pos, kd_pos, P->kd_off);
  LDDL_HIP(hipMemsetAsync(d_max_docs, 0, 8, st));
  hipLaunchKernelGGL(part_offsets_kernel, dim3((unsigned)((n_part + 256) / 256)), dim3(256), 0, st,
                     d_part_doc_off, n_part, kd_pos, P->kp_off, d_max_docs);
  LDDL_HIP(hipGetLastError());
  LDDL_HIP(hipMemcpyAsync(&W.max_docs, d_max_docs, 8, hipMemcpyDeviceToHost, st));
  LDDL_HIP(hipStreamSynchronize(st));
  const int32_t ib = W.c->id_bytes();
  uint8_t* raw;
  if ((rc = P->mem.take(&raw, (W.n_kept_tok + 16) * ib))) return rc;
  P->dense = IdPtr{raw + 8 * ib, ib};
  if (P->n_kept_sent && !dense_in_plan(W))
    hipLaunchKernelGGL(densify_kernel, dim3((unsigned)((P->n_kept_sent + 255) / 256)), dim3(256), 0,
                       st, P->ks_start, P->ks_len, P->kscan, P->n_kept_sent, W.d_ids, P->dense);
  LDDL_HIP(hipGetLastError());
  return 0;
}

static int layout_alloc(lddl_pairs* P, PlanWork& W) {
  const int64_t npairs = P->n_pairs;
  int rc;
  if ((rc = P->mem.take(&P->tok_off, npairs + 1)) || (rc = P->mem.take(&P->rec, npairs)) ||
      (rc = W.tmp.take(&W.pcnt, npairs)) || (rc = W.tmp.take(&W.scr2, 2 * scan_scratch_elems(npairs))))
    return rc;
  if (P->masking && (rc = P->mem.take(&P->pos_off, npairs + 1))) return rc;
  return 0;
}

static int layout_scan(lddl_pairs* P, PlanWork& W) {
  if (P->masking)
    LDDL_HIP(scan_exclusive2(PairCounts{W.pcnt}, P->n_pairs, P->tok_off, P->pos_off, W.scr2, W.st));
  else
    LDDL_HIP(scan_exclusive(PairTokens{W.pcnt}, P->n_pairs, P->tok_off, W.scr2, W.st));
  return 0;
}

static int layout_pairs(lddl_pairs* P, PlanWork& W) {
  int rc;
  if ((rc = layout_alloc(P, W))) return rc;
  const int64_t npairs = P->n_pairs;
  if (npairs)
    hipLaunchKernelGGL(pair_prep_kernel, dim3((unsigned)((npairs + 255) / 256)), dim3(256), 0, W.st,
                       P->src, npairs, P->desc, P->kscan, P->masking ? P->nmask : nullptr,
                       P->moff, P->rec, W.pcnt);
  LDDL_HIP(hipGetLastError());
  return layout_scan(P, W);
}

template <typename Args>
static void fill_plan_args(Args& A, const lddl_pairs* P, const PlanWork& W) {
  A.kscan = P->kscan;
  A.ks_len = P->ks_len;
  A.kd_off = P->kd_off;
  A.kp_off = P->kp_off;
  A.dense = P->dense;
  A.part_seed = W.d_part_seed;
  A.n_part = (decltype(A.n_part))W.n_part;
  A.seq = W.prm->seq;
  A.dup = W.prm->dup;
  A.masking = W.prm->masking;
  A.vocab_size = W.c->vocab_size;
  A.cls_id = P->cls_id;
  A.sep_id = P->sep_id;
  A.mask_id = W.c->tab.special_id[kMask];
  A.ratio = W.prm->masked_lm_ratio;
  A.k_short = short_threshold(W.prm->short_seq_prob);
}

static int plan_native(lddl_pairs* P, PlanWork& W) {
  const lddl_pair_params* prm = W.prm;
  const int64_t n_part = W.n_part;
  hipStream_t st = W.st;
  NativeArgs A{};
  fill_plan_args(A, P, W);
  int64_t kp_ends[2] = {0, 0};
  unsigned long long need_max = 0, *d_need;
  int rc;
  if ((rc = W.tmp.take(&d_need, 1))) return rc;
  LDDL_HIP(hipMemsetAsync(d_need, 0, 8, st));
  if (n_part)
    hipLaunchKernelGGL(native_part_need_kernel, dim3((unsigned)((n_part + 255) / 256)), dim3(256), 0, st,
                       P->kp_off, P->kd_off, n_part, d_need);
  LDDL_HIP(hipMemcpyAsync(&kp_ends[0], P->kp_off, 8, hipMemcpyDeviceToHost, st));
  LDDL_HIP(hipMemcpyAsync(&kp_ends[1], P->kp_off + n_part, 8, hipMemcpyDeviceToHost, st));
  LDDL_HIP(hipMemcpyAsync(&need_max, d_need, 8, hipMemcpyDeviceToHost, st));
  LDDL_HIP(hipStreamSynchronize(st));
  A.unit0 = (int64_t)prm->dup * kp_ends[0];
  A.n_units = (int64_t)prm->dup * (kp_ends[1] - kp_ends[0]);
  A.native_seed = prm->native_seed;
  const int64_t nu = A.n_units;
  int64_t kLdsWordsCap = 24576;
  if (const char* e = getenv("LDDL_NATIVE_LDS_WORDS")) kLdsWordsCap = atoll(e);
  const int32_t lds_words = (int32_t)std::max<int64_t>(
      1, std::min<int64_t>((int64_t)need_max, kLdsWordsCap));
  int64_t *uoff, *scr, *g_pre = nullptr;
  if ((rc = W.tmp.take(&A.ucnt, nu)) || (rc = W.tmp.take(&uoff, nu + 1)) ||
      (rc = W.tmp.take(&scr, scan_scratch_elems(std::max(nu, P->n_kept_sent) + 1))))
    return rc;
  if ((int64_t)need_max > kLdsWordsCap) {
    if ((rc = W.tmp.take(&g_pre, P->n_kept_sent + 1))) return rc;
    LDDL_HIP(scan_exclusive(KeptLenOnly{P->ks_len}, P->n_kept_sent, g_pre, scr, st));
  }
  LDDL_HIP(hipEventRecord(P->ev[0], st));
  const size_t lds_bytes = (size_t)4 * lds_words;
  if (n_part && nu)
    hipLaunchKernelGGL(plan_native_kernel<false>, dim3((unsigned)n_part), dim3(kNativeThreads), lds_bytes,
                       st, A, g_pre, lds_words);
  LDDL_HIP(hipGetLastError());
  LDDL_HIP(scan_exclusive(Identity{A.ucnt}, nu, uoff, scr, st));
  LDDL_HIP(hipMemcpyAsync(&P->n_pairs, uoff + nu, 8, hipMemcpyDeviceToHost, st));
  LDDL_HIP(hipStreamSynchronize(st));
  const int64_t n = P->n_pairs;
  A.uoff = uoff;
  A.n_pairs = n;
  if ((rc = P->mem.take(&P->part_base, n_part + 1)) || (rc = P->mem.take(&P->desc, n)) ||
      (rc = W.tmp.take(&A.ppart, n)) || (rc = P->mem.take(&P->src, n)))
    return rc;
  if (prm->masking &&
      ((rc = P->mem.take(&P->nmask, n)) || (rc = W.tmp.take(&A.ncand, n)) ||
       (rc = P->mem.take(&P->moff, n + 1)) || (rc = W.tmp.take(&scr, scan_scratch_elems(n + 1)))))
    return rc;
  hipLaunchKernelGGL(native_part_base_kernel, dim3((unsigned)((n_part + 256) / 256)), dim3(256), 0,
                     st, P->kp_off, n_part, prm->dup, uoff, P->part_base);
  A.part_base = P->part_base;
  A.desc = P->desc;
  A.nmask = P->nmask;
  if (n_part && nu)
    hipLaunchKernelGGL(plan_native_kernel<true>, dim3((unsigned)n_part), dim3(kNativeThreads), lds_bytes,
                       st, A, g_pre, lds_words);
  LDDL_HIP(hipGetLastError());
  const unsigned gp = (unsigned)((n + 255) / 256);
  if (prm->masking) {
    LDDL_HIP(scan_exclusive(I32{P->nmask}, n, P->moff, scr, st));
    LDDL_HIP(hipMemcpyAsync(&P->n_masked, P->moff + n, 8, hipMemcpyDeviceToHost, st));
    LDDL_HIP(hipStreamSynchronize(st));
    if ((rc = P->mem.take(&P->mpos, P->n_masked)) || (rc = P->mem.take(&P->mtok, P->n_masked)))
      return rc;
    A.moff = P->moff;
    A.mpos = P->mpos;
    A.mtok = P->mtok;
    A.words = (prm->seq + 31) / 32;
    const int32_t stage_cap = 64 * std::max(P->max_pred, 1);
    const size_t per_wave = (size_t)A.words * 64 * 4 + (size_t)stage_cap * 6;
    const int nwv = (int)std::max<size_t>(1, std::min<size_t>(4, 65536 / per_wave));
    if (n)
      hipLaunchKernelGGL(mask_native_kernel, dim3((unsigned)((n + 64 * nwv - 1) / (64 * nwv))),
                         dim3(64 * nwv), per_wave * nwv, st, A, stage_cap);
    LDDL_HIP(hipGetLastError());
  }
  A.src = P->src;
  if (n) hipLaunchKernelGGL(order_native_kernel, dim3(gp), dim3(256), 0, st, A);
  LDDL_HIP(hipGetLastError());
  LDDL_HIP(hipEventRecord(P->ev[1], st));
  return layout_pairs(P, W);
}

static int plan_replay(lddl_pairs* P, PlanWork& W) {
  const lddl_pair_params* prm = W.prm;
  const int64_t n_part = W.n_part;
  hipStream_t st = W.st;
  if (prm->seq > 512) LDDL_FAIL(-1, "replay planner supports target_seq_length <= 512");
  const int64_t slots = (int64_t)prm->dup * P->n_kept_sent;
  int rc;
  if ((rc = P->mem.take(&P->desc, slots)) || (rc = P->mem.take(&P->order, slots)) ||
      (rc = W.tmp.take(&W.jseq, slots)) || (rc = W.tmp.take(&W.part_npairs, n_part + 1)))
    return rc;
  if (prm->masking && (rc = W.tmp.take(&W.spool, slots))) return rc;
  PlanArgs A{};
  fill_plan_args(A, P, W);
  A.ks_start = P->ks_start;
  A.ids = W.d_ids;
  A.n_kept_sent = dense_in_plan(W) ? P->n_kept_sent : 0;
  A.n_dense_wg = 4096;
  A.max_pred = P->max_pred;
  A.short_seq_prob = prm->short_seq_prob;
  A.seq_r64 = ((prm->seq + 63) / 64) * 64;
  A.desc = P->desc;
  A.jseq = W.jseq;
  A.spool = W.spool;
  A.part_npairs = W.part_npairs;
#ifdef LDDL_STAMPS
  if ((rc = W.tmp.take(&W.d_stamps, n_part * kStampRegions)) || (rc = W.tmp.take(&W.d_tl, n_part * 2)))
    return rc;
  LDDL_HIP(hipMemsetAsync(W.d_stamps, 0, 8 * n_part * kStampRegions, st));
  LDDL_HIP(hipMemsetAsync(W.d_tl, 0, 16 * n_part, st));
  A.stamps = W.d_stamps;
  A.tl = W.d_tl;
#endif
  const size_t lds = 4 * (kN + kLook) + 4 * (kDocLds + 4) + 16;
  unsigned long long* pool_ctl;
  if ((rc = W.tmp.take(&pool_ctl, 4)) || (rc = P->mem.take(&P->part_base, n_part + 1))) return rc;
  int64_t cap = 0, jcap = 0;
  const int jbytes = prm->seq <= 256 ? 1 : 2;
  if (prm->masking && W.n_sent) {
    cap = (int64_t)(2.0 * prm->masked_lm_ratio * prm->dup * (double)W.n_kept_tok) +
          (int64_t)prm->dup * P->n_kept_sent / 2 + kPoolChunk * (n_part + 16);
    jcap = (int64_t)(1.6 * prm->dup * (double)W.n_kept_tok) + 8 * slots +
           kPoolChunk * (n_part + 16);
    if (const char* e = getenv("LDDL_AMD_MASK_POOL")) cap = atoll(e);
  }
  if (cap / 8 >= (int64_t)UINT32_MAX || jcap / 16 >= (int64_t)UINT32_MAX)
    LDDL_FAIL(-1, "batch too large for the mask pools (split it into smaller GPU batches)");
  for (int attempt = 0; n_part; ++attempt) {
    int32_t* mtok = nullptr;
    uint8_t* jpool = nullptr;
    if (prm->masking) {
      LDDL_HIP(hipMemsetAsync(pool_ctl, 0, 32, st));
      if ((rc = P->mem.take(&mtok, cap + 4)) || (rc = W.tmp.take(&jpool, jbytes * (jcap + 16))))
        return rc;
    }
    A.mtok = mtok;
    A.jpool = jpool;
    A.jbytes = jbytes;
    A.pool_cap = cap;
    A.jpool_cap = jcap;
    A.pool_used = pool_ctl;
    A.overflow = reinterpret_cast<int32_t*>(pool_ctl + 1);
    LDDL_HIP(hipEventRecord(P->ev[0], st));
    const dim3 grid((unsigned)n_part + (A.n_kept_sent ? (unsigned)A.n_dense_wg : 0u));
    const bool docs_lds = W.max_docs + 1 <= (unsigned long long)kDocLds;
    auto kern = docs_lds ? (jbytes == 1 ? plan_replay_kernel<true, 1> : plan_replay_kernel<true, 2>)
                         : (jbytes == 1 ? plan_replay_kernel<false, 1> : plan_replay_kernel<false, 2>);
    hipLaunchKernelGGL(kern, grid, dim3(64), lds, st, A);
    LDDL_HIP(hipGetLastError());
    LDDL_HIP(hipEventRecord(P->ev[1], st));
    if (!prm->masking) LDDL_HIP(hipMemsetAsync(pool_ctl, 0, 32, st));
    LDDL_HIP(scan_exclusive(Identity{W.part_npairs}, n_part, P->part_base, W.scratch, st));
    hipLaunchKernelGGL(max_pairs_kernel, dim3(64), dim3(256), 0, st, W.part_npairs, n_part, pool_ctl + 3);
    unsigned long long ctl[4];
    LDDL_HIP(hipMemcpyAsync(ctl, pool_ctl, 32, hipMemcpyDeviceToHost, st));
    LDDL_HIP(hipMemcpyAsync(&P->n_pairs, P->part_base + n_part, 8, hipMemcpyDeviceToHost, st));
    LDDL_HIP(hipStreamSynchronize(st));
    W.max_np = std::max<int64_t>(1, (int64_t)ctl[3]);
    if (!prm->masking) break;
    if (!ctl[1]) {
      P->mtok = mtok;
      W.jpool = jpool;
      if ((rc = P->mem.take(&P->mpos, (int64_t)ctl[0]))) return rc;
      break;
    }
    P->mem.give(mtok);
    W.tmp.give(jpool);
    if (attempt > 0) LDDL_FAIL(-1, "mask pool overflow after resize");
    cap = (int64_t)ctl[0] + 1024;
    jcap = (int64_t)ctl[2] + 1024;
  }
  return 0;
}

static int shuffle_partitions(lddl_pairs* P, PlanWork& W) {
  const lddl_pair_params* prm = W.prm;
  const int64_t n_part = W.n_part;
  hipStream_t st = W.st;
  int rc;
  PairMaps& M = W.M;
  M.part_base = P->part_base;
  if (prm->masking) {
    if ((rc = W.tmp.take(&M.slots, P->n_pairs)) || (rc = W.tmp.take(&M.dstq, P->n_pairs))) return rc;
  } else {
    if ((rc = P->mem.take(&P->src, P->n_pairs))) return rc;
    M.src = P->src;
  }
  if (n_part) {
    const int64_t cap = W.max_np;
    const size_t kLdsBudget = std::min<size_t>(150 * 1024, W.c->lds_per_block > 10 * 1024
                                                               ? W.c->lds_per_block - 10 * 1024 : 0);
    const bool force_global = getenv("LDDL_SHUFFLE_GLOBAL") != nullptr;
    const int64_t cap_lds = force_global ? 0 : std::min<int64_t>({cap, 65534, (int64_t)(kLdsBudget / 6) - 2});
    if (cap_lds > 0)
      hipLaunchKernelGGL(shuffle_sort_kernel, dim3((unsigned)n_part), dim3(kShufThreads),
                         (size_t)6 * (size_t)((cap_lds + 2) & ~1), st, P->kd_off, P->kp_off,
                         prm->dup, W.part_npairs, W.jseq, P->order, (int32_t)cap_lds, M);
    if (cap > cap_lds) {
      hipLaunchKernelGGL(apply_shuffle_kernel, dim3((unsigned)n_part), dim3(64), 0, st, P->kd_off,
                         P->kp_off, prm->dup, W.part_npairs, W.jseq, P->order, cap_lds);
      hipLaunchKernelGGL(map_pairs_kernel, dim3((unsigned)n_part), dim3(256), 0, st, P->kd_off,
                         P->kp_off, prm->dup, M.part_base, (const int32_t*)P->order, M.src, M.slots,
                         M.dstq);
    }
  }
  LDDL_HIP(hipGetLastError());
  return 0;
}

#ifdef LDDL_STAMPS
static int report_plan_stamps(const PlanWork& W) {
  const int64_t n_part = W.n_part;
  hipStream_t st = W.st;
  std::vector<uint64_t> h(n_part * kStampRegions);
  LDDL_HIP(hipMemcpyAsync(h.data(), W.d_stamps, 8 * h.size(), hipMemcpyDeviceToHost, st));
  LDDL_HIP(hipStreamSynchronize(st));
  double tot[kStampRegions] = {0};
  for (int64_t q = 0; q < n_part; ++q)
    for (int r = 0; r < kStampRegions; ++r) tot[r] += (double)h[q * kStampRegions + r];
  const char* names[kStampRegions] = {"plan", "cand", "shuffle_draws", "random_next", "decisions",
                                      "trunc", "final_shuffle_draws", "fy_jacobi_passes_per_window"};
  double all = 0;
  for (int r = 0; r < kStampRegions - 1; ++r) all += tot[r];
  fprintf(stderr, "[stamps] plan_replay_kernel mean cycles per partition:");
  for (int r = 0; r < kStampRegions - 1; ++r)
    fprintf(stderr, " %s=%.3g (%.1f%%)", names[r], tot[r] / n_part, 100.0 * tot[r] / (all + 1e-9));
  fprintf(stderr, " %s=%.3f\n", names[kStampRegions - 1], tot[kStampRegions - 1] / n_part / 1e6);
  std::vector<uint64_t> t(2 * n_part);
  LDDL_HIP(hipMemcpyAsync(t.data(), W.d_tl, 16 * n_part, hipMemcpyDeviceToHost, st));
  LDDL_HIP(hipStreamSynchronize(st));
  uint64_t t0 = ~0ull, t1 = 0;
  std::vector<double> dur(n_part);
  for (int64_t q = 0; q < n_part; ++q) {
    t0 = std::min(t0, t[2 * q]);
    t1 = std::max(t1, t[2 * q + 1]);
    dur[q] = (t[2 * q + 1] - t[2 * q]) / 1e5;
  }
  std::vector<double> sd = dur;
  std::sort(sd.begin(), sd.end());
  const double span = (t1 - t0) / 1e5;
  fprintf(stderr, "[timeline] span %.2f ms, partition ms min %.2f p10 %.2f p50 %.2f p90 %.2f max %.2f\n",
          span, sd[0], sd[n_part / 10], sd[n_part / 2], sd[n_part * 9 / 10], sd[n_part - 1]);
  const int nb = 40;
  fprintf(stderr, "[timeline] active partitions per %.2f ms bin:", span / nb);
  for (int b = 0; b < nb; ++b) {
    const uint64_t a = t0 + (t1 - t0) * b / nb, e = t0 + (t1 - t0) * (b + 1) / nb;
    double act = 0;
    for (int64_t q = 0; q < n_part; ++q) {
      const uint64_t s0 = std::max(a, t[2 * q]), s1 = std::min(e, t[2 * q + 1]);
      if (s1 > s0) act += (double)(s1 - s0);
    }
    fprintf(stderr, " %.0f", act / (double)(e - a));
  }
  fprintf(stderr, "\n[timeline] start ms of partitions by index decile:");
  for (int k = 0; k <= 10; ++k) {
    const int64_t q = std::min<int64_t>(n_part - 1, n_part * k / 10);
    fprintf(stderr, " %.1f", (t[2 * q] - t0) / 1e5);
  }
  fprintf(stderr, "\n");
  return 0;
}
#endif

static int resolve_masks(lddl_pairs* P, PlanWork& W) {
  if (!P->n_pairs) return 0;
  const int32_t seq = P->seq;
  const FyKnobs& fy = W.fy;
  hipStream_t st = W.st;
  ResolveArgs RA{W.M.slots, P->n_pairs, P->desc, W.spool, W.jpool, P->mpos, P->kscan, P->dense,
                 P->cls_id, P->sep_id, W.M.dstq, P->rec, W.pcnt, 0};
  const size_t col = (size_t)((seq + 15) & ~15);
  RA.col_rows = (int32_t)col;
#define LDDL_FY_LAUNCH(T, NG, LW, BF, ...)                                                     \
  hipLaunchKernelGGL((fy_resolve_kernel<T, T, NG, LW, BF, ##__VA_ARGS__>),                     \
                     dim3((unsigned)((P->n_pairs + LW - 1) / LW)), dim3(LW),                   \
                     (size_t)LW * sizeof(T) * col, st, RA)
  if (seq <= 131) {
    if (fy.mode == 1) LDDL_FY_LAUNCH(uint8_t, 8, 64, true);
    else LDDL_FY_LAUNCH(uint8_t, 8, 64, false);
  } else if (seq <= 256) {
    if (fy.mode) LDDL_FY_LAUNCH(uint8_t, 0, 16, true);
    else LDDL_FY_LAUNCH(uint8_t, 0, 16, false);
  } else if (fy.lw == 32) {
    if (fy.mode) LDDL_FY_LAUNCH(uint16_t, 0, 32, true);
    else LDDL_FY_LAUNCH(uint16_t, 0, 32, false);
  } else {
    if (!fy.mode) LDDL_FY_LAUNCH(uint16_t, 0, 16, false);
    else if (fy.ra == 1 && fy.pf == 8) LDDL_FY_LAUNCH(uint16_t, 0, 16, true, 1, 8);
    else if (fy.ra == 1 && fy.pf == 2) LDDL_FY_LAUNCH(uint16_t, 0, 16, true, 1, 2);
    else if (fy.ra == 1) LDDL_FY_LAUNCH(uint16_t, 0, 16, true, 1);
    else if (fy.ra == 2) LDDL_FY_LAUNCH(uint16_t, 0, 16, true, 2);
    else if (fy.ra == 3) LDDL_FY_LAUNCH(uint16_t, 0, 16, true, 3);
    else LDDL_FY_LAUNCH(uint16_t, 0, 16, true);
  }
#undef LDDL_FY_LAUNCH
  return 0;
}

static int layout_replay(lddl_pairs* P, PlanWork& W) {
  if (!P->masking) return layout_pairs(P, W);
  int rc;
  if ((rc = layout_alloc(P, W)) || (rc = resolve_masks(P, W))) return rc;
  LDDL_HIP(hipGetLastError());
  return layout_scan(P, W);
}

static int32_t max_predictions(const lddl_pair_params* prm) {
  if (!prm->masking) return 0;
  const int32_t m = (int32_t)rint((double)prm->seq * prm->masked_lm_ratio);
  return std::min(std::max(m, 1), prm->seq);
}

extern "C" int lddl_pairs_plan(lddl_ctx* c, void* stream, const lddl_pair_params* prm,
                               const int64_t* d_sent_off, const int32_t* d_ids,
                               const int32_t* d_sent_len, int64_t n_sent,
                               const int64_t* d_doc_sent_off, int64_t n_doc,
                               const int64_t* d_part_doc_off, const int64_t* d_part_seed,
                               int64_t n_part, lddl_pairs** out, int64_t* counts) {
  *out = nullptr;
  FyKnobs fy;
  int rc;
  if ((rc = check_plan_args(c, prm, &fy))) return rc;
  hipStream_t st = as_stream(stream);
  std::unique_ptr<lddl_pairs> P(new lddl_pairs(&c->arena, st));
  P->n_part = n_part;
  P->masking = prm->masking;
  P->seq = prm->seq;
  P->cls_id = c->tab.special_id[kCls];
  P->sep_id = c->tab.special_id[kSep];
  P->max_pred = max_predictions(prm);
  LDDL_HIP(hipEventCreate(&P->ev[0]));
  LDDL_HIP(hipEventCreate(&P->ev[1]));
  PlanWork W{c, prm, d_ids, d_part_seed, n_sent, n_part, st, P->mem, fy};
  if ((rc = compact_inputs(P.get(), W, d_sent_off, d_sent_len, d_doc_sent_off, n_doc, d_part_doc_off)))
    return rc;
  if (prm->rng == LDDL_RNG_NATIVE) {
    if ((rc = plan_native(P.get(), W))) return rc;
  } else {
    if ((rc = plan_replay(P.get(), W)) || (rc = shuffle_partitions(P.get(), W))) return rc;
#ifdef LDDL_STAMPS
    if ((rc = report_plan_stamps(W))) return rc;
#endif
    if ((rc = layout_replay(P.get(), W))) return rc;
  }
  LDDL_HIP(hipMemcpyAsync(&P->n_tokens, P->tok_off + P->n_pairs, 8, hipMemcpyDeviceToHost, st));
  if (prm->masking)
    LDDL_HIP(hipMemcpyAsync(&P->n_masked, P->pos_off + P->n_pairs, 8, hipMemcpyDeviceToHost, st));
  LDDL_HIP(hipStreamSynchronize(st));
  if (counts) {
    counts[0] = P->n_pairs;
    counts[1] = P->n_tokens;
    counts[2] = P->n_masked;
    counts[3] = P->n_kept_sent;
    counts[4] = P->n_kept_doc;
  }
  *out = P.release();
  return 0;
}

extern "C" int lddl_pairs_emit(lddl_pairs* P, void* stream, void* d_tokens, int64_t* d_tok_off,
                               int32_t* d_len_a, uint8_t* d_is_rn, uint16_t* d_pos, void* d_lab,
                               int64_t* d_pos_off) {
  if (!P) LDDL_FAIL(-1, "null plan");
  hipStream_t st = as_stream(stream);
  if (P->n_pairs == 0) return 0;
  GatherArgs G{};
  G.dense = P->dense.p;
  G.rec = P->rec;
  G.mpos = P->mpos;
  G.mtok = P->mtok;
  G.masking = P->masking;
  G.n_pairs = P->n_pairs;
  G.tok_off = P->tok_off;
  G.pos_off = P->pos_off;
  G.out_tok = d_tokens;
  G.len_a = d_len_a;
  G.is_rn = d_is_rn;
  G.out_pos = d_pos;
  G.out_lab = d_lab;
  G.out_tok_off = d_tok_off;
  G.out_pos_off = d_pos_off;
  GatherLds Lg{(P->seq + 127) / 128 * 128, P->dense.ib, P->dense.ib == 2 && P->seq <= 600 ? 2 : 4};
  auto launch = [&](auto kern, int K) {
    const int64_t per_wg = (int64_t)2 * K * kGWaves;
    const int64_t nwg = (P->n_pairs + per_wg - 1) / per_wg;
    const int64_t gx = std::min<int64_t>(nwg, 65536);
    const size_t lds = P->masking ? (size_t)kGWaves * 2 * K * Lg.per_pair() : 0;
    hipLaunchKernelGGL(kern, dim3((unsigned)gx, (unsigned)((nwg + gx - 1) / gx)), dim3(64 * kGWaves),
                       lds, st, G, Lg);
  };
  const bool i16 = P->dense.ib == 2;
  if (P->seq <= 600) {
    if (i16) launch(gather16_kernel<16>, 2);
    else launch(gather_kernel<2, int32_t>, 2);
  } else {
    if (i16) launch(gather_kernel<1, uint16_t>, 1);
    else launch(gather_kernel<1, int32_t>, 1);
  }
  LDDL_HIP(hipGetLastError());
  return 0;
}

extern "C" int lddl_pairs_destroy(lddl_pairs* P, void* stream) {
  if (!P) return 0;
  P->mem.release(as_stream(stream));
  delete P;
  return 0;
}

extern "C" int lddl_pairs_plan_ms(const lddl_pairs* P, float* ms) {
  if (!P || !ms) LDDL_FAIL(-1, "null argument");
  *ms = 0.f;
  if (P->n_part && P->ev[0]) LDDL_HIP(hipEventElapsedTime(ms, P->ev[0], P->ev[1]));
  return 0;
}

extern "C" int lddl_pairs_part_offsets(lddl_pairs* P, void* stream, int64_t* d_part_pair_off) {
  if (!P || !d_part_pair_off) LDDL_FAIL(-1, "null argument");
  LDDL_HIP(hipMemcpyAsync(d_part_pair_off, P->part_base, 8 * (P->n_part + 1),
                          hipMemcpyDeviceToDevice, as_stream(stream)));
  return 0;
}
```

### lddl_amd/pairs.py

```python
import ctypes
from dataclasses import dataclass

import numpy as np
import torch

from ._native import lib, check, PairParams, RNG_REPLAY, RNG_NATIVE
from .context import _ptr, _stream


def _ids(t):
    a = t.cpu().numpy()
    return a.view(np.uint16) if a.dtype == np.int16 else a


@dataclass
class PairBatch:
    tokens: torch.Tensor
    tok_off: torch.Tensor
    len_a: torch.Tensor
    is_random_next: torch.Tensor
    pos: torch.Tensor = None
    labels: torch.Tensor = None
    pos_off: torch.Tensor = None
    n_kept_sentences: int = 0
    n_kept_documents: int = 0
    part_off: torch.Tensor = None
    plan_ms: float = 0.0
    n_masked: int = 0

    @property
    def n_pairs(self):
        return self.len_a.numel()

    @property
    def num_tokens(self):
        return (self.tok_off[1:] - self.tok_off[:-1]) + 3

    def to_host(self):
        out = dict(tokens=_ids(self.tokens), tok_off=self.tok_off.cpu().numpy(),
                   len_a=self.len_a.cpu().numpy(),
                   is_random_next=self.is_random_next.cpu().numpy().astype(bool))
        out['num_tokens'] = np.diff(out['tok_off']) + 3
        if self.part_off is not None:
            out['part_off'] = self.part_off.cpu().numpy()
        if self.pos is not None:
            out['pos'] = self.pos.cpu().numpy().view(np.uint16)
            out['labels'] = _ids(self.labels)
            out['pos_off'] = self.pos_off.cpu().numpy()
        return out


def make_pairs(ctx, sent_off, ids, sent_len, doc_sent_off, part_doc_off, part_seed, seq=128,
               dup=5, masking=False, short_seq_prob=0.1, masked_lm_ratio=0.15, rng='replay',
               native_seed=12345):
    dev = ctx.device
    prm = PairParams(seq, dup, int(bool(masking)), RNG_REPLAY if rng == 'replay' else RNG_NATIVE,
                     short_seq_prob, masked_lm_ratio, native_seed)
    n_sent = sent_off.numel() - 1
    n_doc = doc_sent_off.numel() - 1
    n_part = part_doc_off.numel() - 1
    h = ctypes.c_void_p()
    counts = np.zeros(5, np.int64)
    st = _stream()
    check(lib.lddl_pairs_plan(ctx.handle, st, ctypes.byref(prm), _ptr(sent_off), _ptr(ids),
                              _ptr(sent_len), n_sent, _ptr(doc_sent_off), n_doc, _ptr(part_doc_off),
                              _ptr(part_seed), n_part, ctypes.byref(h), counts.ctypes.data))
    try:
        n_pairs, n_tok, n_mask = int(counts[0]), int(counts[1]), int(counts[2])
        tokens = torch.empty(max(n_tok, 1), dtype=ctx.id_dtype, device=dev)[:n_tok]
        tok_off = torch.empty(n_pairs + 1, dtype=torch.int64, device=dev)
        len_a = torch.empty(n_pairs, dtype=torch.int32, device=dev)
        is_rn = torch.empty(n_pairs, dtype=torch.uint8, device=dev)
        pos = labels = pos_off = None
        if masking:
            pos = torch.empty(max(n_mask, 1), dtype=torch.int16, device=dev)[:n_mask]
            labels = torch.empty(max(n_mask, 1), dtype=ctx.id_dtype, device=dev)[:n_mask]
            pos_off = torch.empty(n_pairs + 1, dtype=torch.int64, device=dev)
        check(lib.lddl_pairs_emit(h, st, _ptr(tokens), _ptr(tok_off), _ptr(len_a), _ptr(is_rn),
                                  _ptr(pos), _ptr(labels), _ptr(pos_off)))
        part_off = torch.empty(n_part + 1, dtype=torch.int64, device=dev)
        check(lib.lddl_pairs_part_offsets(h, st, _ptr(part_off)))
        ms = ctypes.c_float()
        check(lib.lddl_pairs_plan_ms(h, ctypes.byref(ms)))
    finally:
        lib.lddl_pairs_destroy(h, st)
    return PairBatch(tokens, tok_off, len_a, is_rn, pos, labels, pos_off, int(counts[3]),
                     int(counts[4]), part_off, float(ms.value), n_mask)


_SIDE = {}


def _side_stream(dev):
    key = torch.device(dev).index
    if key not in _SIDE:
        _SIDE[key] = torch.cuda.Stream(device=dev)
    return _SIDE[key]


def tokenize_and_pair_chunked(ctx, text, sent_off, doc_sent_off, part_doc_off, part_seed,
                              n_chunks=2, max_pieces=512, tok_stream=None, **pair_kw):
    n_part = part_doc_off.numel() - 1
    cuts = [round(k * n_part / n_chunks) for k in range(n_chunks + 1)]
    pc = torch.tensor(cuts, dtype=torch.int64, device=part_doc_off.device)
    d_cut = part_doc_off.index_select(0, pc)
    s_cut = doc_sent_off.index_select(0, d_cut)
    b_cut = sent_off.index_select(0, s_cut)
    d_cut, s_cut, b_cut = d_cut.tolist(), s_cut.tolist(), b_cut.tolist()
    main = torch.cuda.current_stream()
    side = tok_stream or _side_stream(text.device)
    side.wait_stream(main)
    toks = []
    with torch.cuda.stream(side):
        for k in range(n_chunks):
            t = text[b_cut[k]:b_cut[k + 1]]
            so = sent_off[s_cut[k]:s_cut[k + 1] + 1] - b_cut[k]
            ids, sl = ctx.tokenize(t, so, max_pieces)
            ev = torch.cuda.Event()
            ev.record(side)
            toks.append((so, ids, sl, ev))
    out = []
    for k, (so, ids, sl, ev) in enumerate(toks):
        main.wait_event(ev)
        for x in (so, ids, sl):
            x.record_stream(main)
        pb = make_pairs(ctx, so, ids, sl, doc_sent_off[d_cut[k]:d_cut[k + 1] + 1] - s_cut[k],
                        part_doc_off[cuts[k]:cuts[k + 1] + 1] - d_cut[k],
                        part_seed[cuts[k]:cuts[k + 1]], **pair_kw)
        del ids
        out.append(pb)
    return out
```

Before: 69.19 billion.

## Split pair planning into head and tail ranges to overlap gather with tail planning

Pair planning is split at a partition boundary into a head range and a tail range. The head is planned first, and its gather/emit can start while the tail partitions are planned on a side stream. Outputs are allocated from a capacity estimate based on the head. If the estimate is too small, the head results are copied into a larger buffer, or the code falls back to a full emit. This adds extra host syncs, an extra stream, event joins and possible copies in exchange for overlapping planning with gathering.

```diff
diff --git a/include/lddl_amd.h b/include/lddl_amd.h
--- a/include/lddl_amd.h
+++ b/include/lddl_amd.h
@@ -85,6 +85,18 @@
 int lddl_pairs_emit(lddl_pairs* plan, void* stream, void* d_tokens, int64_t* d_tok_off,
                     int32_t* d_len_a, uint8_t* d_is_rn, uint16_t* d_pos, void* d_lab,
                     int64_t* d_pos_off);
+int lddl_pairs_plan_head(lddl_ctx* ctx, void* stream, const lddl_pair_params* params,
+                         const int64_t* d_sent_off, const int32_t* d_ids, const int32_t* d_sent_len,
+                         int64_t n_sent, const int64_t* d_doc_sent_off, int64_t n_doc,
+                         const int64_t* d_part_doc_off, const int64_t* d_part_seed, int64_t n_part,
+                         lddl_pairs** out, int64_t* head);
+int lddl_pairs_emit_head(lddl_pairs* plan, void* stream, void* d_tokens, int64_t* d_tok_off,
+                         int32_t* d_len_a, uint8_t* d_is_rn, uint16_t* d_pos, void* d_lab,
+                         int64_t* d_pos_off);
+int lddl_pairs_plan_tail(lddl_pairs* plan, int64_t* counts, int32_t* head_valid);
+int lddl_pairs_emit_tail(lddl_pairs* plan, void* stream, void* d_tokens, int64_t* d_tok_off,
+                         int32_t* d_len_a, uint8_t* d_is_rn, uint16_t* d_pos, void* d_lab,
+                         int64_t* d_pos_off);
 int lddl_pairs_destroy(lddl_pairs* plan, void* stream);
 int lddl_pairs_part_offsets(lddl_pairs* plan, void* stream, int64_t* d_part_pair_off);
 int lddl_pairs_plan_ms(const lddl_pairs* plan, float* ms);
diff --git a/lddl_amd/_native.py b/lddl_amd/_native.py
--- a/lddl_amd/_native.py
+++ b/lddl_amd/_native.py
@@ -42,6 +42,11 @@
     'lddl_pairs_plan': (ctypes.c_int, [c_vp, c_vp, c_vp, c_vp, c_vp, c_vp, c_i64, c_vp, c_i64, c_vp,
                                        c_vp, c_i64, ctypes.POINTER(c_vp), c_vp]),
     'lddl_pairs_emit': (ctypes.c_int, [c_vp, c_vp, c_vp, c_vp, c_vp, c_vp, c_vp, c_vp, c_vp]),
+    'lddl_pairs_plan_head': (ctypes.c_int, [c_vp, c_vp, c_vp, c_vp, c_vp, c_vp, c_i64, c_vp, c_i64,
+                                            c_vp, c_vp, c_i64, ctypes.POINTER(c_vp), c_vp]),
+    'lddl_pairs_emit_head': (ctypes.c_int, [c_vp, c_vp, c_vp, c_vp, c_vp, c_vp, c_vp, c_vp, c_vp]),
+    'lddl_pairs_plan_tail': (ctypes.c_int, [c_vp, c_vp, ctypes.POINTER(ctypes.c_int32)]),
+    'lddl_pairs_emit_tail': (ctypes.c_int, [c_vp, c_vp, c_vp, c_vp, c_vp, c_vp, c_vp, c_vp, c_vp]),
     'lddl_pairs_destroy': (ctypes.c_int, [c_vp, c_vp]),
     'lddl_pairs_part_offsets': (ctypes.c_int, [c_vp, c_vp, c_vp]),
     'lddl_pairs_plan_ms': (ctypes.c_int, [c_vp, ctypes.POINTER(ctypes.c_float)]),
diff --git a/lddl_amd/csrc/ctx.h b/lddl_amd/csrc/ctx.h
--- a/lddl_amd/csrc/ctx.h
+++ b/lddl_amd/csrc/ctx.h
@@ -28,6 +28,7 @@
   lddl::DevArena arena;
   void* punkt = nullptr;
   void* bart = nullptr;
+  hipStream_t plan_side = nullptr;
 };
 extern "C" void lddl_punkt_release(lddl_ctx* c);
 extern "C" void lddl_bart_release(lddl_ctx* c);
diff --git a/lddl_amd/csrc/ctx.hip b/lddl_amd/csrc/ctx.hip
--- a/lddl_amd/csrc/ctx.hip
+++ b/lddl_amd/csrc/ctx.hip
@@ -187,6 +187,10 @@
   (void)hipSetDevice(c->device);
   lddl_bart_release(c);
   lddl_punkt_release(c);
+  if (c->plan_side) {
+    (void)hipStreamSynchronize(c->plan_side);
+    (void)hipStreamDestroy(c->plan_side);
+  }
   for (void* p : {(void*)c->d_l1, (void*)c->d_pages, (void*)c->d_pool, (void*)c->d_vhash,
                   (void*)c->d_vbytes, (void*)c->d_voff, (void*)c->d_render, (void*)c->d_render_off,
                   (void*)c->d_bloom, (void*)c->d_vlong, (void*)c->d_cont_bits})
diff --git a/lddl_amd/csrc/pairs.hip b/lddl_amd/csrc/pairs.hip
--- a/lddl_amd/csrc/pairs.hip
+++ b/lddl_amd/csrc/pairs.hip
@@ -10,6 +10,7 @@
 #include "ctx.h"
 #include "device.h"
 #include "lddl_amd.h"
+#include "plan_split.h"
 #include "scan.h"
 
 namespace lddl {
@@ -406,6 +407,8 @@
   IdPtr dense;
   int64_t n_kept_sent;
   int32_t n_part, n_dense_wg;
+  int32_t p0;
+  const int64_t* dense_lo;
   const int64_t* part_seed;
   int32_t seq, dup, masking, vocab_size, cls_id, sep_id, mask_id, max_pred;
   double short_seq_prob, ratio;
@@ -552,14 +555,15 @@
   extern __shared__ __attribute__((aligned(16))) uint8_t smem[];
   uint32_t* s_mt = reinterpret_cast<uint32_t*>(smem);
   int32_t* s_doc = reinterpret_cast<int32_t*>(s_mt + kN + kLook);
-  const int p = blockIdx.x;
   const int lane = threadIdx.x;
   const bool leader = lane == 0;
-  if (p >= A.n_part) {
-    for (int64_t g = p - A.n_part; g * 64 < A.n_kept_sent; g += A.n_dense_wg)
-      densify_group(g * 64, A.ks_start, A.ks_len, A.kscan, A.n_kept_sent, A.ids, A.dense);
+  if ((int)blockIdx.x >= A.n_part) {
+    const int64_t k_lo = A.dense_lo ? *A.dense_lo : 0;
+    for (int64_t g = (int)blockIdx.x - A.n_part; k_lo + g * 64 < A.n_kept_sent; g += A.n_dense_wg)
+      densify_group(k_lo + g * 64, A.ks_start, A.ks_len, A.kscan, A.n_kept_sent, A.ids, A.dense);
     return;
   }
+  const int p = A.p0 + (int)blockIdx.x;
 #ifdef LDDL_STAMPS
   uint64_t st_acc[kStampRegions] = {0, 0, 0, 0, 0, 0, 0, 0};
 #endif
@@ -1344,6 +1348,31 @@
   densify_group(k0, ks_start, ks_len, kscan, n, ids, dense);
 }
 
+__global__ void split_info_kernel(const int64_t* kp_off, const int64_t* kd_off, const int64_t* kscan,
+                                  int64_t s, int64_t* info) {
+  const int64_t k = kd_off[kp_off[s]];
+  info[0] = k;
+  info[1] = kscan[k];
+}
+
+__global__ void __launch_bounds__(256) densify_head_kernel(const int64_t* __restrict__ ks_start,
+                                                           const int32_t* __restrict__ ks_len,
+                                                           const int64_t* __restrict__ kscan,
+                                                           const int64_t* __restrict__ n_ptr,
+                                                           const int32_t* __restrict__ ids,
+                                                           IdPtr dense) {
+  const int64_t n = *n_ptr;
+  const int64_t k0 = ((int64_t)blockIdx.x * 4 + wave_id()) * 64;
+  if (k0 >= n) return;
+  densify_group(k0, ks_start, ks_len, kscan, n, ids, dense);
+}
+
+__global__ void tail_part_base_kernel(const int64_t* rel, int64_t n, int64_t head_pairs,
+                                      int64_t* part_base_s) {
+  const int64_t i = (int64_t)blockIdx.x * blockDim.x + threadIdx.x;
+  if (i < n) part_base_s[1 + i] = head_pairs + rel[i + 1];
+}
+
 
 struct GatherArgs {
   const void* dense;
@@ -1354,6 +1383,7 @@
   int64_t n_pairs;
   const int64_t* tok_off;
   const int64_t* pos_off;
+  int64_t tok_base, pos_base;
   void* out_tok;
   int32_t* len_a;
   uint8_t* is_rn;
@@ -1619,8 +1649,8 @@
     const int64_t q = q0 + 2 * k + h;
     const bool act = q < G.n_pairs;
     rc[k] = act ? G.rec[q] : GatherRec{0, 0, 0, 0, 0, 0, 0};
-    tof[k] = act ? G.tok_off[q] : 0;
-    po[k] = (G.masking && act) ? G.pos_off[q] : 0;
+    tof[k] = act ? G.tok_base + G.tok_off[q] : 0;
+    po[k] = (G.masking && act) ? G.pos_base + G.pos_off[q] : 0;
   }
 #pragma unroll
   for (int k = 0; k < K; ++k) {
@@ -1791,8 +1821,8 @@
   const int64_t q = (wg * kGWaves + w) * PW + qw;
   const bool act = q < G.n_pairs;
   const GatherRec r = act ? G.rec[q] : GatherRec{0, 0, 0, 0, 0, 0, 0};
-  const int64_t tof = act ? G.tok_off[q] : 0;
-  const int64_t po = (G.masking && act) ? G.pos_off[q] : 0;
+  const int64_t tof = act ? G.tok_base + G.tok_off[q] : 0;
+  const int64_t po = (G.masking && act) ? G.pos_base + G.pos_off[q] : 0;
   const int32_t na = r.na, nb = r.nb_rn & 0x7FFFFFFF, n = na + nb;
   const int32_t nm = G.masking ? r.nm : 0;
   const int64_t mb = r.moff;
@@ -1896,6 +1926,53 @@
 
 using namespace lddl;
 
+struct FyKnobs {
+  int mode, lw, ra, pf;
+};
+
+struct PlanWork {
+  lddl_ctx* c;
+  const lddl_pair_params* prm;
+  const int32_t* d_ids;
+  const int64_t* d_part_seed;
+  int64_t n_sent, n_part;
+  hipStream_t st;
+  ArenaScope& tmp;
+  FyKnobs fy;
+  int64_t split_knob = -1;
+  int64_t* scratch = nullptr;
+  int64_t n_kept_tok = 0;
+  unsigned long long max_docs = 0;
+  int32_t* jseq = nullptr;
+  int64_t* part_npairs = nullptr;
+  SlotPool* spool = nullptr;
+  void* jpool = nullptr;
+  int64_t max_np = 1;
+  PlanArgs A{};
+  unsigned long long* pool_ctl = nullptr;
+  int64_t cap = 0, jcap = 0;
+  int32_t* mtok_try = nullptr;
+  uint8_t* jpool_try = nullptr;
+  int64_t split = 0;
+  int64_t* split_info = nullptr;
+  int64_t h_split_info[2] = {0, 0};
+  int64_t* tail_rel = nullptr;
+  PairMaps M{nullptr, nullptr, nullptr, nullptr};
+  int2* pcnt = nullptr;
+  int64_t* scr2 = nullptr;
+#ifdef LDDL_STAMPS
+  uint64_t *d_stamps = nullptr, *d_tl = nullptr;
+#endif
+};
+
+struct PairRange {
+  int64_t p0 = 0, p1 = 0;
+  int64_t n_pairs = 0, n_tokens = 0, n_masked = 0;
+  int64_t pair0 = 0, tok0 = 0, pos0 = 0;
+  GatherRec* rec = nullptr;
+  int64_t *tok_off = nullptr, *pos_off = nullptr;
+};
+
 struct lddl_pairs {
   int32_t masking = 0, max_pred = 0, seq = 0, cls_id = -1, sep_id = -1;
   int64_t n_part = 0, n_pairs = 0, n_tokens = 0, n_masked = 0, n_kept_sent = 0, n_kept_doc = 0;
@@ -1907,20 +1984,28 @@
   int32_t *order = nullptr, *nmask = nullptr, *mtok = nullptr;
   uint16_t* mpos = nullptr;
   int64_t* moff = nullptr;
-  int64_t *src = nullptr, *tok_off = nullptr, *pos_off = nullptr;
-  GatherRec* rec = nullptr;
+  int64_t* src = nullptr;
+  PairRange rg[2];
+  int n_rg = 1;
   int64_t* part_base = nullptr;
   hipEvent_t ev[2] = {nullptr, nullptr};
-
-  lddl_pairs(DevArena* arena, hipStream_t st) : mem(arena, st) {}
+  hipStream_t st;
+  hipEvent_t ev_fork = nullptr, ev_join = nullptr;
+  bool tail_pending = false;
+  bool head_valid = false;
+  lddl_pair_params prm{};
+  std::unique_ptr<PlanWork> work;
+
+  lddl_pairs(DevArena* arena, hipStream_t stream) : mem(arena, stream), st(stream) {}
+  void join(hipStream_t on) {
+    if (tail_pending) (void)hipStreamWaitEvent(on, ev_join, 0);
+    tail_pending = false;
+  }
   ~lddl_pairs() {
-    for (hipEvent_t e : ev)
+    join(st);
+    for (hipEvent_t e : {ev[0], ev[1], ev_fork, ev_join})
       if (e) (void)hipEventDestroy(e);
   }
-};
-
-struct FyKnobs {
-  int mode, lw, ra, pf;
 };
 
 static int env_int(const char* name, int dflt) {
@@ -1942,7 +2027,18 @@
   return 0;
 }
 
-static int check_plan_args(const lddl_ctx* c, const lddl_pair_params* prm, FyKnobs* fy) {
+static int read_split_knob(int64_t* k) {
+  *k = -1;
+  const char* e = getenv("LDDL_PLAN_SPLIT");
+  if (!e) return 0;
+  char* end = nullptr;
+  const long long v = strtoll(e, &end, 10);
+  if (end == e || *end || v < -1) LDDL_FAIL(-1, "LDDL_PLAN_SPLIT must be -1 (auto), 0 or a partition count");
+  *k = v;
+  return 0;
+}
+
+static int check_plan_args(const lddl_ctx* c, const lddl_pair_params* prm, FyKnobs* fy, int64_t* split_knob) {
   if (!c || !prm) LDDL_FAIL(-1, "null argument");
   if (prm->seq < 5 || prm->seq > 65535) LDDL_FAIL(-1, "target_seq_length %d out of range", prm->seq);
   if (prm->dup < 1) LDDL_FAIL(-1, "duplicate_factor must be >= 1");
@@ -1953,33 +2049,10 @@
   if (prm->masking && (c->tab.special_id[kCls] < 0 || c->tab.special_id[kSep] < 0 ||
                        c->tab.special_id[kMask] < 0))
     LDDL_FAIL(-1, "static masking needs [CLS] [SEP] [MASK] in the vocab");
+  int rc;
+  if ((rc = read_split_knob(split_knob))) return rc;
   return read_fy_knobs(fy);
 }
-
-struct PlanWork {
-  lddl_ctx* c;
-  const lddl_pair_params* prm;
-  const int32_t* d_ids;
-  const int64_t* d_part_seed;
-  int64_t n_sent, n_part;
-  hipStream_t st;
-  ArenaScope& tmp;
-  FyKnobs fy;
-  int64_t* scratch = nullptr;
-  int64_t n_kept_tok = 0;
-  unsigned long long max_docs = 0;
-  int32_t* jseq = nullptr;
-  int64_t* part_npairs = nullptr;
-  SlotPool* spool = nullptr;
-  void* jpool = nullptr;
-  int64_t max_np = 1;
-  PairMaps M{nullptr, nullptr, nullptr, nullptr};
-  int2* pcnt = nullptr;
-  int64_t* scr2 = nullptr;
-#ifdef LDDL_STAMPS
-  uint64_t *d_stamps = nullptr, *d_tl = nullptr;
-#endif
-};
 
 static bool dense_in_plan(const PlanWork& W) { return W.prm->rng == LDDL_RNG_REPLAY && W.n_part > 0; }
 
@@ -2043,34 +2116,40 @@
   return 0;
 }
 
-static int layout_alloc(lddl_pairs* P, PlanWork& W) {
-  const int64_t npairs = P->n_pairs;
+static int layout_alloc(lddl_pairs* P, PlanWork& W, PairRange& r) {
+  const int64_t npairs = r.n_pairs;
   int rc;
-  if ((rc = P->mem.take(&P->tok_off, npairs + 1)) || (rc = P->mem.take(&P->rec, npairs)) ||
+  if ((rc = P->mem.take(&r.tok_off, npairs + 1)) || (rc = P->mem.take(&r.rec, npairs)) ||
       (rc = W.tmp.take(&W.pcnt, npairs)) || (rc = W.tmp.take(&W.scr2, 2 * scan_scratch_elems(npairs))))
     return rc;
-  if (P->masking && (rc = P->mem.take(&P->pos_off, npairs + 1))) return rc;
+  if (P->masking && (rc = P->mem.take(&r.pos_off, npairs + 1))) return rc;
   return 0;
 }
 
-static int layout_scan(lddl_pairs* P, PlanWork& W) {
+static int layout_scan(lddl_pairs* P, PlanWork& W, PairRange& r) {
   if (P->masking)
-    LDDL_HIP(scan_exclusive2(PairCounts{W.pcnt}, P->n_pairs, P->tok_off, P->pos_off, W.scr2, W.st));
+    LDDL_HIP(scan_exclusive2(PairCounts{W.pcnt}, r.n_pairs, r.tok_off, r.pos_off, W.scr2, W.st));
   else
-    LDDL_HIP(scan_exclusive(PairTokens{W.pcnt}, P->n_pairs, P->tok_off, W.scr2, W.st));
+    LDDL_HIP(scan_exclusive(PairTokens{W.pcnt}, r.n_pairs, r.tok_off, W.scr2, W.st));
+  LDDL_HIP(hipMemcpyAsync(&r.n_tokens, r.tok_off + r.n_pairs, 8, hipMemcpyDeviceToHost, W.st));
+  if (P->masking)
+    LDDL_HIP(hipMemcpyAsync(&r.n_masked, r.pos_off + r.n_pairs, 8, hipMemcpyDeviceToHost, W.st));
   return 0;
 }
 
 static int layout_pairs(lddl_pairs* P, PlanWork& W) {
   int rc;
-  if ((rc = layout_alloc(P, W))) return rc;
+  PairRange& r = P->rg[0];
+  r.p1 = P->n_part;
+  r.n_pairs = P->n_pairs;
+  if ((rc = layout_alloc(P, W, r))) return rc;
   const int64_t npairs = P->n_pairs;
   if (npairs)
     hipLaunchKernelGGL(pair_prep_kernel, dim3((unsigned)((npairs + 255) / 256)), dim3(256), 0, W.st,
                        P->src, npairs, P->desc, P->kscan, P->masking ? P->nmask : nullptr,
-                       P->moff, P->rec, W.pcnt);
+                       P->moff, r.rec, W.pcnt);
   LDDL_HIP(hipGetLastError());
-  return layout_scan(P, W);
+  return layout_scan(P, W, r);
 }
 
 template <typename Args>
@@ -2181,10 +2260,9 @@
   return layout_pairs(P, W);
 }
 
-static int plan_replay(lddl_pairs* P, PlanWork& W) {
+static int plan_replay_setup(lddl_pairs* P, PlanWork& W) {
   const lddl_pair_params* prm = W.prm;
   const int64_t n_part = W.n_part;
-  hipStream_t st = W.st;
   if (prm->seq > 512) LDDL_FAIL(-1, "replay planner supports target_seq_length <= 512");
   const int64_t slots = (int64_t)prm->dup * P->n_kept_sent;
   int rc;
@@ -2192,7 +2270,7 @@
       (rc = W.tmp.take(&W.jseq, slots)) || (rc = W.tmp.take(&W.part_npairs, n_part + 1)))
     return rc;
   if (prm->masking && (rc = W.tmp.take(&W.spool, slots))) return rc;
-  PlanArgs A{};
+  PlanArgs& A = W.A;
   fill_plan_args(A, P, W);
   A.ks_start = P->ks_start;
   A.ids = W.d_ids;
@@ -2208,100 +2286,191 @@
 #ifdef LDDL_STAMPS
   if ((rc = W.tmp.take(&W.d_stamps, n_part * kStampRegions)) || (rc = W.tmp.take(&W.d_tl, n_part * 2)))
     return rc;
-  LDDL_HIP(hipMemsetAsync(W.d_stamps, 0, 8 * n_part * kStampRegions, st));
-  LDDL_HIP(hipMemsetAsync(W.d_tl, 0, 16 * n_part, st));
+  LDDL_HIP(hipMemsetAsync(W.d_stamps, 0, 8 * n_part * kStampRegions, W.st));
+  LDDL_HIP(hipMemsetAsync(W.d_tl, 0, 16 * n_part, W.st));
   A.stamps = W.d_stamps;
   A.tl = W.d_tl;
 #endif
-  const size_t lds = 4 * (kN + kLook) + 4 * (kDocLds + 4) + 16;
-  unsigned long long* pool_ctl;
-  if ((rc = W.tmp.take(&pool_ctl, 4)) || (rc = P->mem.take(&P->part_base, n_part + 1))) return rc;
-  int64_t cap = 0, jcap = 0;
-  const int jbytes = prm->seq <= 256 ? 1 : 2;
+  if ((rc = W.tmp.take(&W.pool_ctl, 4)) || (rc = P->mem.take(&P->part_base, n_part + 1))) return rc;
+  W.cap = W.jcap = 0;
+  A.jbytes = prm->seq <= 256 ? 1 : 2;
   if (prm->masking && W.n_sent) {
-    cap = (int64_t)(2.0 * prm->masked_lm_ratio * prm->dup * (double)W.n_kept_tok) +
-          (int64_t)prm->dup * P->n_kept_sent / 2 + kPoolChunk * (n_part + 16);
-    jcap = (int64_t)(1.6 * prm->dup * (double)W.n_kept_tok) + 8 * slots +
-           kPoolChunk * (n_part + 16);
-    if (const char* e = getenv("LDDL_AMD_MASK_POOL")) cap = atoll(e);
-  }
-  if (cap / 8 >= (int64_t)UINT32_MAX || jcap / 16 >= (int64_t)UINT32_MAX)
+    W.cap = (int64_t)(2.0 * prm->masked_lm_ratio * prm->dup * (double)W.n_kept_tok) +
+            (int64_t)prm->dup * P->n_kept_sent / 2 + kPoolChunk * (n_part + 16);
+    W.jcap = (int64_t)(1.6 * prm->dup * (double)W.n_kept_tok) + 8 * slots +
+             kPoolChunk * (n_part + 16);
+    if (const char* e = getenv("LDDL_AMD_MASK_POOL")) W.cap = atoll(e);
+  }
+  if (W.cap / 8 >= (int64_t)UINT32_MAX || W.jcap / 16 >= (int64_t)UINT32_MAX)
     LDDL_FAIL(-1, "batch too large for the mask pools (split it into smaller GPU batches)");
-  for (int attempt = 0; n_part; ++attempt) {
-    int32_t* mtok = nullptr;
-    uint8_t* jpool = nullptr;
-    if (prm->masking) {
-      LDDL_HIP(hipMemsetAsync(pool_ctl, 0, 32, st));
-      if ((rc = P->mem.take(&mtok, cap + 4)) || (rc = W.tmp.take(&jpool, jbytes * (jcap + 16))))
-        return rc;
-    }
-    A.mtok = mtok;
-    A.jpool = jpool;
-    A.jbytes = jbytes;
-    A.pool_cap = cap;
-    A.jpool_cap = jcap;
-    A.pool_used = pool_ctl;
-    A.overflow = reinterpret_cast<int32_t*>(pool_ctl + 1);
+  A.pool_used = W.pool_ctl;
+  A.overflow = reinterpret_cast<int32_t*>(W.pool_ctl + 1);
+  return 0;
+}
+
+typedef void (*PlanKernel)(PlanArgs);
+static PlanKernel planner_kernel(const PlanWork& W) {
+  const bool docs_lds = W.max_docs + 1 <= (unsigned long long)kDocLds;
+  return docs_lds ? (W.A.jbytes == 1 ? plan_replay_kernel<true, 1> : plan_replay_kernel<true, 2>)
+                  : (W.A.jbytes == 1 ? plan_replay_kernel<false, 1> : plan_replay_kernel<false, 2>);
+}
+constexpr size_t kPlanLds = 4 * (kN + kLook) + 4 * (kDocLds + 4) + 16;
+
+static int choose_split(const PlanWork& W, int64_t* s) {
+  *s = 0;
+  if (!W.prm->masking || W.n_part <= 0 || W.split_knob == 0) return 0;
+  int64_t capacity = 0;
+  if (W.split_knob < 0) {
+    int per_cu = 0, n_cu = 0;
+    LDDL_HIP(hipOccupancyMaxActiveBlocksPerMultiprocessor(&per_cu, planner_kernel(W), 64, kPlanLds));
+    LDDL_HIP(hipDeviceGetAttribute(&n_cu, hipDeviceAttributeMultiprocessorCount, W.c->device));
+    capacity = (int64_t)per_cu * n_cu;
+  }
+  *s = plan_split_point(W.n_part, capacity, W.split_knob);
+  return 0;
+}
+
+static int take_pools(lddl_pairs* P, PlanWork& W, bool split) {
+  W.mtok_try = nullptr;
+  W.jpool_try = nullptr;
+  int rc;
+  if (W.prm->masking) {
+    LDDL_HIP(hipMemsetAsync(W.pool_ctl, 0, 32, W.st));
+    if ((rc = P->mem.take(&W.mtok_try, W.cap + 4)) ||
+        (rc = W.tmp.take(&W.jpool_try, W.A.jbytes * (W.jcap + 16))))
+      return rc;
+    if (split && (rc = P->mem.take(&P->mpos, W.cap + 4))) return rc;
+  }
+  W.A.mtok = W.mtok_try;
+  W.A.jpool = W.jpool_try;
+  W.A.pool_cap = W.cap;
+  W.A.jpool_cap = W.jcap;
+  return 0;
+}
+
+static int launch_planner(const PlanWork& W, int64_t p0, int64_t n, hipStream_t st, bool with_dense,
+                          const int64_t* dense_lo) {
+  PlanArgs A = W.A;
+  A.p0 = (int32_t)p0;
+  A.n_part = (int32_t)n;
+  A.dense_lo = dense_lo;
+  if (!with_dense) A.n_kept_sent = 0;
+  const unsigned grid = (unsigned)n + (A.n_kept_sent ? (unsigned)A.n_dense_wg : 0u);
+  if (grid) hipLaunchKernelGGL(planner_kernel(W), dim3(grid), dim3(64), kPlanLds, st, A);
+  LDDL_HIP(hipGetLastError());
+  return 0;
+}
+
+static int plan_replay_unsplit(lddl_pairs* P, PlanWork& W, int attempt) {
+  const lddl_pair_params* prm = W.prm;
+  const int64_t n_part = W.n_part;
+  hipStream_t st = W.st;
+  int rc;
+  for (; n_part; ++attempt) {
+    if ((rc = take_pools(P, W, false))) return rc;
     LDDL_HIP(hipEventRecord(P->ev[0], st));
-    const dim3 grid((unsigned)n_part + (A.n_kept_sent ? (unsigned)A.n_dense_wg : 0u));
-    const bool docs_lds = W.max_docs + 1 <= (unsigned long long)kDocLds;
-    auto kern = docs_lds ? (jbytes == 1 ? plan_replay_kernel<true, 1> : plan_replay_kernel<true, 2>)
-                         : (jbytes == 1 ? plan_replay_kernel<false, 1> : plan_replay_kernel<false, 2>);
-    hipLaunchKernelGGL(kern, grid, dim3(64), lds, st, A);
-    LDDL_HIP(hipGetLastError());
+    if ((rc = launch_planner(W, 0, n_part, st, true, nullptr))) return rc;
     LDDL_HIP(hipEventRecord(P->ev[1], st));
-    if (!prm->masking) LDDL_HIP(hipMemsetAsync(pool_ctl, 0, 32, st));
+    if (!prm->masking) LDDL_HIP(hipMemsetAsync(W.pool_ctl, 0, 32, st));
     LDDL_HIP(scan_exclusive(Identity{W.part_npairs}, n_part, P->part_base, W.scratch, st));
-    hipLaunchKernelGGL(max_pairs_kernel, dim3(64), dim3(256), 0, st, W.part_npairs, n_part, pool_ctl + 3);
+    hipLaunchKernelGGL(max_pairs_kernel, dim3(64), dim3(256), 0, st, W.part_npairs, n_part, W.pool_ctl + 3);
     unsigned long long ctl[4];
-    LDDL_HIP(hipMemcpyAsync(ctl, pool_ctl, 32, hipMemcpyDeviceToHost, st));
+    LDDL_HIP(hipMemcpyAsync(ctl, W.pool_ctl, 32, hipMemcpyDeviceToHost, st));
     LDDL_HIP(hipMemcpyAsync(&P->n_pairs, P->part_base + n_part, 8, hipMemcpyDeviceToHost, st));
     LDDL_HIP(hipStreamSynchronize(st));
     W.max_np = std::max<int64_t>(1, (int64_t)ctl[3]);
     if (!prm->masking) break;
     if (!ctl[1]) {
-      P->mtok = mtok;
-      W.jpool = jpool;
+      P->mtok = W.mtok_try;
+      W.jpool = W.jpool_try;
       if ((rc = P->mem.take(&P->mpos, (int64_t)ctl[0]))) return rc;
       break;
     }
-    P->mem.give(mtok);
-    W.tmp.give(jpool);
+    P->mem.give(W.mtok_try);
+    W.tmp.give(W.jpool_try);
     if (attempt > 0) LDDL_FAIL(-1, "mask pool overflow after resize");
-    cap = (int64_t)ctl[0] + 1024;
-    jcap = (int64_t)ctl[2] + 1024;
+    W.cap = (int64_t)ctl[0] + 1024;
+    W.jcap = (int64_t)ctl[2] + 1024;
   }
   return 0;
 }
 
-static int shuffle_partitions(lddl_pairs* P, PlanWork& W) {
+static int plan_side_stream(lddl_ctx* c, hipStream_t* out) {
+  if (!c->plan_side) {
+    int least = 0, greatest = 0;
+    LDDL_HIP(hipDeviceGetStreamPriorityRange(&least, &greatest));
+    LDDL_HIP(hipStreamCreateWithPriority(&c->plan_side, hipStreamNonBlocking, least));
+  }
+  *out = c->plan_side;
+  return 0;
+}
+
+static int plan_replay_split_head(lddl_pairs* P, PlanWork& W, bool* usable) {
+  const int64_t n_part = W.n_part, s = W.split;
+  hipStream_t st = W.st, side;
+  int rc;
+  if ((rc = plan_side_stream(W.c, &side)) || (rc = take_pools(P, W, true)) ||
+      (rc = W.tmp.take(&W.split_info, 2)) || (rc = W.tmp.take(&W.tail_rel, n_part - s + 1)))
+    return rc;
+  LDDL_HIP(hipEventCreateWithFlags(&P->ev_fork, hipEventDisableTiming));
+  LDDL_HIP(hipEventCreateWithFlags(&P->ev_join, hipEventDisableTiming));
+  hipLaunchKernelGGL(split_info_kernel, dim3(1), dim3(1), 0, st, P->kp_off, P->kd_off, P->kscan, s,
+                     W.split_info);
+  LDDL_HIP(hipGetLastError());
+  LDDL_HIP(hipEventRecord(P->ev[0], st));
+  LDDL_HIP(hipEventRecord(P->ev_fork, st));
+  LDDL_HIP(hipStreamWaitEvent(side, P->ev_fork, 0));
+  if ((rc = launch_planner(W, 0, s, st, false, nullptr))) return rc;
+  P->tail_pending = true;
+  rc = launch_planner(W, s, n_part - s, side, true, W.split_info);
+  LDDL_HIP(hipEventRecord(P->ev_join, side));
+  if (rc) return rc;
+  if (P->n_kept_sent)
+    hipLaunchKernelGGL(densify_head_kernel, dim3((unsigned)((P->n_kept_sent + 255) / 256)), dim3(256),
+                       0, st, P->ks_start, P->ks_len, P->kscan, W.split_info, W.d_ids, P->dense);
+  LDDL_HIP(scan_exclusive(Identity{W.part_npairs}, s, P->part_base, W.scratch, st));
+  hipLaunchKernelGGL(max_pairs_kernel, dim3(64), dim3(256), 0, st, W.part_npairs, s, W.pool_ctl + 3);
+  LDDL_HIP(hipGetLastError());
+  unsigned long long ctl[4];
+  LDDL_HIP(hipMemcpyAsync(ctl, W.pool_ctl, 32, hipMemcpyDeviceToHost, st));
+  LDDL_HIP(hipMemcpyAsync(&P->rg[0].n_pairs, P->part_base + s, 8, hipMemcpyDeviceToHost, st));
+  LDDL_HIP(hipMemcpyAsync(W.h_split_info, W.split_info, 16, hipMemcpyDeviceToHost, st));
+  LDDL_HIP(hipStreamSynchronize(st));
+  W.max_np = std::max<int64_t>(1, (int64_t)ctl[3]);
+  *usable = ctl[1] == 0;
+  return 0;
+}
+
+static int shuffle_partitions(lddl_pairs* P, PlanWork& W, const PairRange& r, const int64_t* rel_base) {
   const lddl_pair_params* prm = W.prm;
-  const int64_t n_part = W.n_part;
+  const int64_t n_part = r.p1 - r.p0;
   hipStream_t st = W.st;
   int rc;
   PairMaps& M = W.M;
-  M.part_base = P->part_base;
+  M = PairMaps{rel_base, nullptr, nullptr, nullptr};
   if (prm->masking) {
-    if ((rc = W.tmp.take(&M.slots, P->n_pairs)) || (rc = W.tmp.take(&M.dstq, P->n_pairs))) return rc;
+    if ((rc = W.tmp.take(&M.slots, r.n_pairs)) || (rc = W.tmp.take(&M.dstq, r.n_pairs))) return rc;
   } else {
-    if ((rc = P->mem.take(&P->src, P->n_pairs))) return rc;
+    if ((rc = P->mem.take(&P->src, r.n_pairs))) return rc;
     M.src = P->src;
   }
   if (n_part) {
     const int64_t cap = W.max_np;
+    const int64_t* kp_off = P->kp_off + r.p0;
+    const int64_t* part_npairs = W.part_npairs + r.p0;
     const size_t kLdsBudget = std::min<size_t>(150 * 1024, W.c->lds_per_block > 10 * 1024
                                                                ? W.c->lds_per_block - 10 * 1024 : 0);
     const bool force_global = getenv("LDDL_SHUFFLE_GLOBAL") != nullptr;
     const int64_t cap_lds = force_global ? 0 : std::min<int64_t>({cap, 65534, (int64_t)(kLdsBudget / 6) - 2});
     if (cap_lds > 0)
       hipLaunchKernelGGL(shuffle_sort_kernel, dim3((unsigned)n_part), dim3(kShufThreads),
-                         (size_t)6 * (size_t)((cap_lds + 2) & ~1), st, P->kd_off, P->kp_off,
-                         prm->dup, W.part_npairs, W.jseq, P->order, (int32_t)cap_lds, M);
+                         (size_t)6 * (size_t)((cap_lds + 2) & ~1), st, P->kd_off, kp_off,
+                         prm->dup, part_npairs, W.jseq, P->order, (int32_t)cap_lds, M);
     if (cap > cap_lds) {
       hipLaunchKernelGGL(apply_shuffle_kernel, dim3((unsigned)n_part), dim3(64), 0, st, P->kd_off,
-                         P->kp_off, prm->dup, W.part_npairs, W.jseq, P->order, cap_lds);
+                         kp_off, prm->dup, part_npairs, W.jseq, P->order, cap_lds);
       hipLaunchKernelGGL(map_pairs_kernel, dim3((unsigned)n_part), dim3(256), 0, st, P->kd_off,
-                         P->kp_off, prm->dup, M.part_base, (const int32_t*)P->order, M.src, M.slots,
+                         kp_off, prm->dup, M.part_base, (const int32_t*)P->order, M.src, M.slots,
                          M.dstq);
     }
   }
@@ -2363,18 +2532,18 @@
 }
 #endif
 
-static int resolve_masks(lddl_pairs* P, PlanWork& W) {
-  if (!P->n_pairs) return 0;
+static int resolve_masks(lddl_pairs* P, PlanWork& W, const PairRange& r) {
+  if (!r.n_pairs) return 0;
   const int32_t seq = P->seq;
   const FyKnobs& fy = W.fy;
   hipStream_t st = W.st;
-  ResolveArgs RA{W.M.slots, P->n_pairs, P->desc, W.spool, W.jpool, P->mpos, P->kscan, P->dense,
-                 P->cls_id, P->sep_id, W.M.dstq, P->rec, W.pcnt, 0};
+  ResolveArgs RA{W.M.slots, r.n_pairs, P->desc, W.spool, W.jpool, P->mpos, P->kscan, P->dense,
+                 P->cls_id, P->sep_id, W.M.dstq, r.rec, W.pcnt, 0};
   const size_t col = (size_t)((seq + 15) & ~15);
   RA.col_rows = (int32_t)col;
 #define LDDL_FY_LAUNCH(T, NG, LW, BF, ...)                                                     \
   hipLaunchKernelGGL((fy_resolve_kernel<T, T, NG, LW, BF, ##__VA_ARGS__>),                     \
-                     dim3((unsigned)((P->n_pairs + LW - 1) / LW)), dim3(LW),                   \
+                     dim3((unsigned)((r.n_pairs + LW - 1) / LW)), dim3(LW),                   \
                      (size_t)LW * sizeof(T) * col, st, RA)
   if (seq <= 131) {
     if (fy.mode == 1) LDDL_FY_LAUNCH(uint8_t, 8, 64, true);
@@ -2398,12 +2567,33 @@
   return 0;
 }
 
-static int layout_replay(lddl_pairs* P, PlanWork& W) {
-  if (!P->masking) return layout_pairs(P, W);
+static int layout_replay(lddl_pairs* P, PlanWork& W, PairRange& r) {
   int rc;
-  if ((rc = layout_alloc(P, W)) || (rc = resolve_masks(P, W))) return rc;
+  if ((rc = layout_alloc(P, W, r)) || (rc = resolve_masks(P, W, r))) return rc;
   LDDL_HIP(hipGetLastError());
-  return layout_scan(P, W);
+  return layout_scan(P, W, r);
+}
+
+static int finish_unsplit(lddl_pairs* P, PlanWork& W) {
+  int rc;
+  P->n_rg = 1;
+  PairRange& r = P->rg[0];
+  r = PairRange{};
+  r.p1 = W.n_part;
+  r.n_pairs = P->n_pairs;
+  if ((rc = shuffle_partitions(P, W, r, P->part_base))) return rc;
+#ifdef LDDL_STAMPS
+  if ((rc = report_plan_stamps(W))) return rc;
+#endif
+  return P->masking ? layout_replay(P, W, r) : layout_pairs(P, W);
+}
+
+static void give_range_tmp(PlanWork& W) {
+  for (void* b : {(void*)W.M.slots, (void*)W.M.dstq, (void*)W.pcnt, (void*)W.scr2})
+    if (b) W.tmp.give(b);
+  W.M = PairMaps{nullptr, nullptr, nullptr, nullptr};
+  W.pcnt = nullptr;
+  W.scr2 = nullptr;
 }
 
 static int32_t max_predictions(const lddl_pair_params* prm) {
@@ -2412,19 +2602,126 @@
   return std::min(std::max(m, 1), prm->seq);
 }
 
-extern "C" int lddl_pairs_plan(lddl_ctx* c, void* stream, const lddl_pair_params* prm,
-                               const int64_t* d_sent_off, const int32_t* d_ids,
-                               const int32_t* d_sent_len, int64_t n_sent,
-                               const int64_t* d_doc_sent_off, int64_t n_doc,
-                               const int64_t* d_part_doc_off, const int64_t* d_part_seed,
-                               int64_t n_part, lddl_pairs** out, int64_t* counts) {
-  *out = nullptr;
+static int plan_head_stage(lddl_pairs* P, const int64_t* d_sent_off, const int32_t* d_sent_len,
+                           const int64_t* d_doc_sent_off, int64_t n_doc,
+                           const int64_t* d_part_doc_off) {
+  PlanWork& W = *P->work;
+  int rc;
+  if ((rc = compact_inputs(P, W, d_sent_off, d_sent_len, d_doc_sent_off, n_doc, d_part_doc_off)))
+    return rc;
+  if (W.prm->rng == LDDL_RNG_NATIVE) {
+    if ((rc = plan_native(P, W))) return rc;
+  } else {
+    if ((rc = plan_replay_setup(P, W)) || (rc = choose_split(W, &W.split))) return rc;
+    if (!W.split) {
+      if ((rc = plan_replay_unsplit(P, W, 0)) || (rc = finish_unsplit(P, W))) return rc;
+    } else {
+      bool usable = false;
+      if ((rc = plan_replay_split_head(P, W, &usable))) return rc;
+      PairRange& r = P->rg[0];
+      r.p1 = W.split;
+      if (usable) {
+        W.jpool = W.jpool_try;
+        P->mtok = W.mtok_try;
+        if ((rc = shuffle_partitions(P, W, r, P->part_base)) || (rc = layout_replay(P, W, r))) return rc;
+        P->head_valid = true;
+      } else {
+        r.n_pairs = 0;
+      }
+    }
+  }
+  LDDL_HIP(hipStreamSynchronize(W.st));
+  if (!W.split) {
+    P->n_tokens = P->rg[0].n_tokens;
+    P->n_masked = P->rg[0].n_masked;
+    P->work.reset();
+  }
+  return 0;
+}
+
+static int plan_tail_stage(lddl_pairs* P) {
+  if (!P->work) return 0;
+  PlanWork& W = *P->work;
+  hipStream_t st = W.st;
+  const int64_t s = W.split, n_tail = W.n_part - s;
+  int rc;
+  P->join(st);
+  LDDL_HIP(hipEventRecord(P->ev[1], st));
+  LDDL_HIP(scan_exclusive(Identity{W.part_npairs + s}, n_tail, W.tail_rel, W.scratch, st));
+  hipLaunchKernelGGL(max_pairs_kernel, dim3(64), dim3(256), 0, st, W.part_npairs + s, n_tail,
+                     W.pool_ctl + 3);
+  LDDL_HIP(hipGetLastError());
+  unsigned long long ctl[4];
+  PairRange &h = P->rg[0], &t = P->rg[1];
+  LDDL_HIP(hipMemcpyAsync(ctl, W.pool_ctl, 32, hipMemcpyDeviceToHost, st));
+  LDDL_HIP(hipMemcpyAsync(&t.n_pairs, W.tail_rel + n_tail, 8, hipMemcpyDeviceToHost, st));
+  LDDL_HIP(hipStreamSynchronize(st));
+  W.max_np = std::max<int64_t>(1, (int64_t)ctl[3]);
+  if (ctl[1]) {
+    P->head_valid = false;
+    give_range_tmp(W);
+    for (void* b : {(void*)W.mtok_try, (void*)P->mpos, (void*)h.rec, (void*)h.tok_off, (void*)h.pos_off})
+      if (b) P->mem.give(b);
+    W.tmp.give(W.jpool_try);
+    P->mtok = nullptr;
+    P->mpos = nullptr;
+    W.jpool = nullptr;
+    h = PairRange{};
+    t = PairRange{};
+    W.split = 0;
+    W.cap = (int64_t)ctl[0] + 1024;
+    W.jcap = (int64_t)ctl[2] + 1024;
+    if ((rc = plan_replay_unsplit(P, W, 1)) || (rc = finish_unsplit(P, W))) return rc;
+    LDDL_HIP(hipStreamSynchronize(st));
+    P->n_tokens = h.n_tokens;
+    P->n_masked = h.n_masked;
+  } else {
+    give_range_tmp(W);
+    if (n_tail)
+      hipLaunchKernelGGL(tail_part_base_kernel, dim3((unsigned)((n_tail + 255) / 256)), dim3(256), 0,
+                         st, W.tail_rel, n_tail, h.n_pairs, P->part_base + s);
+    LDDL_HIP(hipGetLastError());
+    t.p0 = s;
+    t.p1 = W.n_part;
+    t.pair0 = h.n_pairs;
+    t.tok0 = h.n_tokens;
+    t.pos0 = h.n_masked;
+    P->n_rg = 2;
+    if ((rc = shuffle_partitions(P, W, t, W.tail_rel)) || (rc = layout_replay(P, W, t))) return rc;
+    LDDL_HIP(hipStreamSynchronize(st));
+    P->n_pairs = h.n_pairs + t.n_pairs;
+    P->n_tokens = h.n_tokens + t.n_tokens;
+    P->n_masked = h.n_masked + t.n_masked;
+  }
+  P->work.reset();
+  return 0;
+}
+
+static void plan_counts(const lddl_pairs* P, int64_t* counts) {
+  if (!counts) return;
+  counts[0] = P->n_pairs;
+  counts[1] = P->n_tokens;
+  counts[2] = P->n_masked;
+  counts[3] = P->n_kept_sent;
+  counts[4] = P->n_kept_doc;
+}
+
+extern "C" int lddl_pairs_plan_head(lddl_ctx* c, void* stream, const lddl_pair_params* prm,
+                                    const int64_t* d_sent_off, const int32_t* d_ids,
+                                    const int32_t* d_sent_len, int64_t n_sent,
+                                    const int64_t* d_doc_sent_off, int64_t n_doc,
+                                    const int64_t* d_part_doc_off, const int64_t* d_part_seed,
+                                    int64_t n_part, lddl_pairs** out, int64_t* head) {
+  if (out) *out = nullptr;
   FyKnobs fy;
+  int64_t split_knob;
   int rc;
-  if ((rc = check_plan_args(c, prm, &fy))) return rc;
+  if (!out) LDDL_FAIL(-1, "null argument");
+  if ((rc = check_plan_args(c, prm, &fy, &split_knob))) return rc;
   hipStream_t st = as_stream(stream);
   std::unique_ptr<lddl_pairs> P(new lddl_pairs(&c->arena, st));
   P->n_part = n_part;
+  P->prm = *prm;
   P->masking = prm->masking;
   P->seq = prm->seq;
   P->cls_id = c->tab.special_id[kCls];
@@ -2432,30 +2729,100 @@
   P->max_pred = max_predictions(prm);
   LDDL_HIP(hipEventCreate(&P->ev[0]));
   LDDL_HIP(hipEventCreate(&P->ev[1]));
-  PlanWork W{c, prm, d_ids, d_part_seed, n_sent, n_part, st, P->mem, fy};
-  if ((rc = compact_inputs(P.get(), W, d_sent_off, d_sent_len, d_doc_sent_off, n_doc, d_part_doc_off)))
+  P->work.reset(new PlanWork{c, &P->prm, d_ids, d_part_seed, n_sent, n_part, st, P->mem, fy, split_knob});
+  if ((rc = plan_head_stage(P.get(), d_sent_off, d_sent_len, d_doc_sent_off, n_doc, d_part_doc_off)))
     return rc;
-  if (prm->rng == LDDL_RNG_NATIVE) {
-    if ((rc = plan_native(P.get(), W))) return rc;
-  } else {
-    if ((rc = plan_replay(P.get(), W)) || (rc = shuffle_partitions(P.get(), W))) return rc;
-#ifdef LDDL_STAMPS
-    if ((rc = report_plan_stamps(W))) return rc;
-#endif
-    if ((rc = layout_replay(P.get(), W))) return rc;
-  }
-  LDDL_HIP(hipMemcpyAsync(&P->n_tokens, P->tok_off + P->n_pairs, 8, hipMemcpyDeviceToHost, st));
-  if (prm->masking)
-    LDDL_HIP(hipMemcpyAsync(&P->n_masked, P->pos_off + P->n_pairs, 8, hipMemcpyDeviceToHost, st));
-  LDDL_HIP(hipStreamSynchronize(st));
-  if (counts) {
-    counts[0] = P->n_pairs;
-    counts[1] = P->n_tokens;
-    counts[2] = P->n_masked;
-    counts[3] = P->n_kept_sent;
-    counts[4] = P->n_kept_doc;
+  if (head) {
+    for (int i = 0; i < 8; ++i) head[i] = 0;
+    if (P->work) {
+      const PlanWork& W = *P->work;
+      const PairRange& h = P->rg[0];
+      head[0] = 1;
+      head[1] = h.n_pairs;
+      head[2] = h.n_tokens;
+      head[3] = h.n_masked;
+      head[4] = plan_suggest_capacity(h.n_pairs, W.n_kept_tok, W.h_split_info[1]);
+      head[5] = plan_suggest_capacity(h.n_tokens, W.n_kept_tok, W.h_split_info[1]);
+      head[6] = plan_suggest_capacity(h.n_masked, W.n_kept_tok, W.h_split_info[1]);
+    }
   }
   *out = P.release();
+  return 0;
+}
+
+extern "C" int lddl_pairs_plan_tail(lddl_pairs* P, int64_t* counts, int32_t* head_valid) {
+  if (!P) LDDL_FAIL(-1, "null plan");
+  int rc;
+  if ((rc = plan_tail_stage(P))) return rc;
+  plan_counts(P, counts);
+  if (head_valid) *head_valid = P->head_valid ? 1 : 0;
+  return 0;
+}
+
+extern "C" int lddl_pairs_plan(lddl_ctx* c, void* stream, const lddl_pair_params* prm,
+                               const int64_t* d_sent_off, const int32_t* d_ids,
+                               const int32_t* d_sent_len, int64_t n_sent,
+                               const int64_t* d_doc_sent_off, int64_t n_doc,
+                               const int64_t* d_part_doc_off, const int64_t* d_part_seed,
+                               int64_t n_part, lddl_pairs** out, int64_t* counts) {
+  lddl_pairs* P = nullptr;
+  int rc;
+  if (out) *out = nullptr;
+  if ((rc = lddl_pairs_plan_head(c, stream, prm, d_sent_off, d_ids, d_sent_len, n_sent, d_doc_sent_off,
+                                 n_doc, d_part_doc_off, d_part_seed, n_part, &P, nullptr)))
+    return rc;
+  if ((rc = lddl_pairs_plan_tail(P, counts, nullptr))) {
+    delete P;
+    return rc;
+  }
+  *out = P;
+  return 0;
+}
+
+static int emit_ranges(lddl_pairs* P, int r0, int r1, void* stream, void* d_tokens, int64_t* d_tok_off,
+                       int32_t* d_len_a, uint8_t* d_is_rn, uint16_t* d_pos, void* d_lab,
+                       int64_t* d_pos_off) {
+  hipStream_t st = as_stream(stream);
+  for (int ri = r0; ri < r1; ++ri) {
+    const PairRange& r = P->rg[ri];
+    if (r.n_pairs == 0) continue;
+    GatherArgs G{};
+    G.dense = P->dense.p;
+    G.rec = r.rec;
+    G.mpos = P->mpos;
+    G.mtok = P->mtok;
+    G.masking = P->masking;
+    G.n_pairs = r.n_pairs;
+    G.tok_off = r.tok_off;
+    G.pos_off = r.pos_off;
+    G.tok_base = r.tok0;
+    G.pos_base = r.pos0;
+    G.out_tok = d_tokens;
+    G.len_a = d_len_a + r.pair0;
+    G.is_rn = d_is_rn + r.pair0;
+    G.out_pos = d_pos;
+    G.out_lab = d_lab;
+    G.out_tok_off = d_tok_off ? d_tok_off + r.pair0 : nullptr;
+    G.out_pos_off = d_pos_off ? d_pos_off + r.pair0 : nullptr;
+    GatherLds Lg{(P->seq + 127) / 128 * 128, P->dense.ib, P->dense.ib == 2 && P->seq <= 600 ? 2 : 4};
+    auto launch = [&](auto kern, int K) {
+      const int64_t per_wg = (int64_t)2 * K * kGWaves;
+      const int64_t nwg = (r.n_pairs + per_wg - 1) / per_wg;
+      const int64_t gx = std::min<int64_t>(nwg, 65536);
+      const size_t lds = P->masking ? (size_t)kGWaves * 2 * K * Lg.per_pair() : 0;
+      hipLaunchKernelGGL(kern, dim3((unsigned)gx, (unsigned)((nwg + gx - 1) / gx)), dim3(64 * kGWaves),
+                         lds, st, G, Lg);
+    };
+    const bool i16 = P->dense.ib == 2;
+    if (P->seq <= 600) {
+      if (i16) launch(gather16_kernel<16>, 2);
+      else launch(gather_kernel<2, int32_t>, 2);
+    } else {
+      if (i16) launch(gather_kernel<1, uint16_t>, 1);
+      else launch(gather_kernel<1, int32_t>, 1);
+    }
+    LDDL_HIP(hipGetLastError());
+  }
   return 0;
 }
 
@@ -2463,47 +2830,32 @@
                                int32_t* d_len_a, uint8_t* d_is_rn, uint16_t* d_pos, void* d_lab,
                                int64_t* d_pos_off) {
   if (!P) LDDL_FAIL(-1, "null plan");
-  hipStream_t st = as_stream(stream);
-  if (P->n_pairs == 0) return 0;
-  GatherArgs G{};
-  G.dense = P->dense.p;
-  G.rec = P->rec;
-  G.mpos = P->mpos;
-  G.mtok = P->mtok;
-  G.masking = P->masking;
-  G.n_pairs = P->n_pairs;
-  G.tok_off = P->tok_off;
-  G.pos_off = P->pos_off;
-  G.out_tok = d_tokens;
-  G.len_a = d_len_a;
-  G.is_rn = d_is_rn;
-  G.out_pos = d_pos;
-  G.out_lab = d_lab;
-  G.out_tok_off = d_tok_off;
-  G.out_pos_off = d_pos_off;
-  GatherLds Lg{(P->seq + 127) / 128 * 128, P->dense.ib, P->dense.ib == 2 && P->seq <= 600 ? 2 : 4};
-  auto launch = [&](auto kern, int K) {
-    const int64_t per_wg = (int64_t)2 * K * kGWaves;
-    const int64_t nwg = (P->n_pairs + per_wg - 1) / per_wg;
-    const int64_t gx = std::min<int64_t>(nwg, 65536);
-    const size_t lds = P->masking ? (size_t)kGWaves * 2 * K * Lg.per_pair() : 0;
-    hipLaunchKernelGGL(kern, dim3((unsigned)gx, (unsigned)((nwg + gx - 1) / gx)), dim3(64 * kGWaves),
-                       lds, st, G, Lg);
-  };
-  const bool i16 = P->dense.ib == 2;
-  if (P->seq <= 600) {
-    if (i16) launch(gather16_kernel<16>, 2);
-    else launch(gather_kernel<2, int32_t>, 2);
-  } else {
-    if (i16) launch(gather_kernel<1, uint16_t>, 1);
-    else launch(gather_kernel<1, int32_t>, 1);
-  }
-  LDDL_HIP(hipGetLastError());
-  return 0;
+  if (P->work) LDDL_FAIL(-1, "lddl_pairs_emit before lddl_pairs_plan_tail");
+  return emit_ranges(P, 0, P->n_rg, stream, d_tokens, d_tok_off, d_len_a, d_is_rn, d_pos, d_lab,
+                     d_pos_off);
+}
+
+extern "C" int lddl_pairs_emit_head(lddl_pairs* P, void* stream, void* d_tokens, int64_t* d_tok_off,
+                                    int32_t* d_len_a, uint8_t* d_is_rn, uint16_t* d_pos, void* d_lab,
+                                    int64_t* d_pos_off) {
+  if (!P) LDDL_FAIL(-1, "null plan");
+  if (!P->work) LDDL_FAIL(-1, "lddl_pairs_emit_head: not a split plan between its head and tail calls");
+  if (!P->head_valid) return 0;
+  return emit_ranges(P, 0, 1, stream, d_tokens, d_tok_off, d_len_a, d_is_rn, d_pos, d_lab, d_pos_off);
+}
+
+extern "C" int lddl_pairs_emit_tail(lddl_pairs* P, void* stream, void* d_tokens, int64_t* d_tok_off,
+                                    int32_t* d_len_a, uint8_t* d_is_rn, uint16_t* d_pos, void* d_lab,
+                                    int64_t* d_pos_off) {
+  if (!P) LDDL_FAIL(-1, "null plan");
+  if (P->work || P->n_rg != 2 || !P->head_valid)
+    LDDL_FAIL(-1, "lddl_pairs_emit_tail: no valid head range (use lddl_pairs_emit)");
+  return emit_ranges(P, 1, 2, stream, d_tokens, d_tok_off, d_len_a, d_is_rn, d_pos, d_lab, d_pos_off);
 }
 
 extern "C" int lddl_pairs_destroy(lddl_pairs* P, void* stream) {
   if (!P) return 0;
+  P->join(as_stream(stream));
   P->mem.release(as_stream(stream));
   delete P;
   return 0;
diff --git a/lddl_amd/csrc/plan_split.h b/lddl_amd/csrc/plan_split.h
--- /dev/null
+++ b/lddl_amd/csrc/plan_split.h
@@ -0,0 +1,23 @@
+#pragma once
+#include <cstdint>
+
+namespace lddl {
+
+inline int64_t plan_split_point(int64_t n_part, int64_t capacity, int64_t knob) {
+  if (n_part <= 0 || knob == 0) return 0;
+  if (knob > 0) return knob < n_part ? knob : n_part;
+  if (capacity < 2 || n_part <= capacity) return 0;
+  return capacity / 2;
+}
+
+inline int64_t plan_suggest_capacity(int64_t head_count, int64_t tok_all, int64_t tok_head) {
+  if (head_count < 0) head_count = 0;
+  unsigned __int128 v = (unsigned __int128)(uint64_t)head_count;
+  if (tok_head > 0 && tok_all > tok_head)
+    v = (v * (unsigned __int128)(uint64_t)tok_all + (uint64_t)tok_head - 1) / (uint64_t)tok_head;
+  v += v / 64 + 1024;
+  const unsigned __int128 lim = (unsigned __int128)INT64_MAX;
+  return (int64_t)(v > lim ? lim : v);
+}
+
+}
diff --git a/lddl_amd/pairs.py b/lddl_amd/pairs.py
--- a/lddl_amd/pairs.py
+++ b/lddl_amd/pairs.py
@@ -1,4 +1,5 @@
 import ctypes
+import os
 from dataclasses import dataclass
 
 import numpy as np
@@ -50,9 +51,36 @@
         return out
 
 
+def _alloc_outputs(ctx, dev, masking, n_pairs, n_tok, n_mask):
+    out = dict(tokens=torch.empty(max(n_tok, 1), dtype=ctx.id_dtype, device=dev),
+               tok_off=torch.empty(n_pairs + 1, dtype=torch.int64, device=dev),
+               len_a=torch.empty(max(n_pairs, 1), dtype=torch.int32, device=dev),
+               is_rn=torch.empty(max(n_pairs, 1), dtype=torch.uint8, device=dev),
+               pos=None, labels=None, pos_off=None)
+    if masking:
+        out.update(pos=torch.empty(max(n_mask, 1), dtype=torch.int16, device=dev),
+                   labels=torch.empty(max(n_mask, 1), dtype=ctx.id_dtype, device=dev),
+                   pos_off=torch.empty(n_pairs + 1, dtype=torch.int64, device=dev))
+    return out
+
+
+_OUT_KEYS = ('tokens', 'tok_off', 'len_a', 'is_rn', 'pos', 'labels', 'pos_off')
+
+
+def _emit_args(o):
+    return [_ptr(o[k]) for k in _OUT_KEYS]
+
+
+def _head_gather():
+    v = os.environ.get('LDDL_PLAN_HEAD_GATHER', '1')
+    if v not in ('0', '1'):
+        raise ValueError('LDDL_PLAN_HEAD_GATHER must be 0 or 1')
+    return v == '1'
+
+
 def make_pairs(ctx, sent_off, ids, sent_len, doc_sent_off, part_doc_off, part_seed, seq=128,
                dup=5, masking=False, short_seq_prob=0.1, masked_lm_ratio=0.15, rng='replay',
-               native_seed=12345):
+               native_seed=12345, _capacity_scale=1.0, _trace=None):
     dev = ctx.device
     prm = PairParams(seq, dup, int(bool(masking)), RNG_REPLAY if rng == 'replay' else RNG_NATIVE,
                      short_seq_prob, masked_lm_ratio, native_seed)
@@ -61,29 +89,54 @@
     n_part = part_doc_off.numel() - 1
     h = ctypes.c_void_p()
     counts = np.zeros(5, np.int64)
+    head = np.zeros(8, np.int64)
+    head_valid = ctypes.c_int32(0)
     st = _stream()
-    check(lib.lddl_pairs_plan(ctx.handle, st, ctypes.byref(prm), _ptr(sent_off), _ptr(ids),
-                              _ptr(sent_len), n_sent, _ptr(doc_sent_off), n_doc, _ptr(part_doc_off),
-                              _ptr(part_seed), n_part, ctypes.byref(h), counts.ctypes.data))
+    check(lib.lddl_pairs_plan_head(ctx.handle, st, ctypes.byref(prm), _ptr(sent_off), _ptr(ids),
+                                   _ptr(sent_len), n_sent, _ptr(doc_sent_off), n_doc,
+                                   _ptr(part_doc_off), _ptr(part_seed), n_part, ctypes.byref(h),
+                                   head.ctypes.data))
     try:
+        o = None
+        caps = (0, 0, 0)
+        if head[0] and _head_gather():
+            caps = tuple(max(int(head[1 + i]), int(int(head[4 + i]) * _capacity_scale))
+                         for i in range(3))
+            o = _alloc_outputs(ctx, dev, masking, *caps)
+            check(lib.lddl_pairs_emit_head(h, st, *_emit_args(o)))
+        check(lib.lddl_pairs_plan_tail(h, counts.ctypes.data, ctypes.byref(head_valid)))
         n_pairs, n_tok, n_mask = int(counts[0]), int(counts[1]), int(counts[2])
-        tokens = torch.empty(max(n_tok, 1), dtype=ctx.id_dtype, device=dev)[:n_tok]
-        tok_off = torch.empty(n_pairs + 1, dtype=torch.int64, device=dev)
-        len_a = torch.empty(n_pairs, dtype=torch.int32, device=dev)
-        is_rn = torch.empty(n_pairs, dtype=torch.uint8, device=dev)
-        pos = labels = pos_off = None
-        if masking:
-            pos = torch.empty(max(n_mask, 1), dtype=torch.int16, device=dev)[:n_mask]
-            labels = torch.empty(max(n_mask, 1), dtype=ctx.id_dtype, device=dev)[:n_mask]
-            pos_off = torch.empty(n_pairs + 1, dtype=torch.int64, device=dev)
-        check(lib.lddl_pairs_emit(h, st, _ptr(tokens), _ptr(tok_off), _ptr(len_a), _ptr(is_rn),
-                                  _ptr(pos), _ptr(labels), _ptr(pos_off)))
+        if o is not None and head_valid.value and all(c >= n for c, n in zip(caps, counts[:3])):
+            check(lib.lddl_pairs_emit_tail(h, st, *_emit_args(o)))
+            path = 'tail'
+        elif o is not None and head_valid.value:
+            big = _alloc_outputs(ctx, dev, masking, n_pairs, n_tok, n_mask)
+            hp, ht, hm = (int(x) for x in head[1:4])
+            for k, n in (('tokens', ht), ('tok_off', hp), ('len_a', hp), ('is_rn', hp), ('pos', hm),
+                         ('labels', hm), ('pos_off', hp)):
+                if big[k] is not None and n:
+                    big[k][:n].copy_(o[k][:n])
+            o = big
+            check(lib.lddl_pairs_emit_tail(h, st, *_emit_args(o)))
+            path = 'copy'
+        else:
+            o = _alloc_outputs(ctx, dev, masking, n_pairs, n_tok, n_mask)
+            check(lib.lddl_pairs_emit(h, st, *_emit_args(o)))
+            path = 'full'
+        if _trace is not None:
+            _trace.update(split=int(head[0]), head_pairs=int(head[1]),
+                          head_valid=int(head_valid.value), path=path)
         part_off = torch.empty(n_part + 1, dtype=torch.int64, device=dev)
         check(lib.lddl_pairs_part_offsets(h, st, _ptr(part_off)))
         ms = ctypes.c_float()
         check(lib.lddl_pairs_plan_ms(h, ctypes.byref(ms)))
     finally:
         lib.lddl_pairs_destroy(h, st)
+    tokens, tok_off = o['tokens'][:n_tok], o['tok_off'][:n_pairs + 1]
+    len_a, is_rn = o['len_a'][:n_pairs], o['is_rn'][:n_pairs]
+    pos = labels = pos_off = None
+    if masking:
+        pos, labels, pos_off = o['pos'][:n_mask], o['labels'][:n_mask], o['pos_off'][:n_pairs + 1]
     return PairBatch(tokens, tok_off, len_a, is_rn, pos, labels, pos_off, int(counts[3]),
                      int(counts[4]), part_off, float(ms.value), n_mask)
 
```

Result: faster. 70.88 billion (median of 6 runs) (+2.4%).
